# vfrantc/Bayesian-Enhancement-Model

Hardware: AMD Instinct MI355X
Metric: images/sec (whole node) CG_UNet N=8 Bayesian eval @256x256 (higher is better)
Workload: dtype f32

## Files before the change

### bayesian-enhancement-model_amd/bem/archs.py

```python
from __future__ import annotations

import math
import os

import torch
import torch.nn as nn

from . import autograd as ag
from . import ops
from .modules import (Conv2dK, ConvT2x2, LayerNorm2d, PwConv2d, VSSBlock, _Cache, _need_cuda, grad_mode, make_vss_level,
                      set_module_paths)
from .native import BemNativeError

_QD_DIR = os.path.join(os.path.dirname(os.path.dirname(os.path.abspath(__file__))), "basicsr", "QD", "checkpoints")


def _trunc_normal_(t, std=0.02):
    return nn.init.trunc_normal_(t, mean=0.0, std=std, a=-2.0, b=2.0)


def _init_weights(m):
    if isinstance(m, nn.Linear):
        _trunc_normal_(m.weight, std=0.02)
        if m.bias is not None:
# ... 1 lines not shown
    elif isinstance(m, nn.LayerNorm):
        nn.init.constant_(m.weight, 1.0)
        nn.init.constant_(m.bias, 0)


def conv_down(c):
    return Conv2dK(c, c * 2, 4, 2, 1, bias=False)


class _CrossAttnParams(nn.Module):

    def __init__(self, dim):
        super().__init__()
        for n in ("q1_proj", "k2_proj", "v2_proj", "q2_proj", "k1_proj", "v1_proj", "out1", "out2"):
            setattr(self, n, nn.Conv2d(dim, dim, 1))


class Decomp(nn.Module):

    def __init__(self, model="model4", wavelet_out=True, num_filters=32):
        super().__init__()
        if model not in ("model1", "model2", "model3", "model4"):
            raise ValueError(f"Unknown decomp_model: {model}")
        self.model, self.wavelet_out = model, wavelet_out
        nf = num_filters
        self.conv_in = Conv2dK(32, nf, 3, padding=1)
        if model == "model3":
            self.down_conv = Conv2dK(nf, nf, 3, stride=2, padding=1)
            self.mid_conv = Conv2dK(nf, nf, 3, padding=1)
            self.up_conv = ConvT2x2(nf, nf)
        d = 2 if model == "model2" else 1
        self.branch_q1 = nn.Sequential(Conv2dK(nf, nf, 3, padding=1), nn.ReLU(inplace=True), Conv2dK(nf, nf, 3, padding=d, dilation=d))
        self.branch_q2 = nn.Sequential(Conv2dK(nf, nf, 3, padding=1), nn.ReLU(inplace=True), Conv2dK(nf, nf, 3, padding=d, dilation=d))
        self.cross_attn = _CrossAttnParams(nf)
        self.fuse = nn.Conv2d(nf * 2, nf, 1)
        self.conv_out = Conv2dK(nf, 32, 3, padding=1)
        self.sharpening = Conv2dK(32, 32, 3, padding=1, bias=True)
        if model == "model4" and not wavelet_out:
            self.smooth_q1 = nn.Module(); self.smooth_q1.conv = nn.Conv2d(4, 4, 3, padding=1, groups=4, bias=True)
            self.smooth_q2 = nn.Module(); self.smooth_q2.conv = nn.Conv2d(4, 4, 3, padding=1, groups=4, bias=True)
        self._cache = _Cache()

    @classmethod
    def from_shipped(cls, model, wavelet_out):
        from safetensors.torch import load_file
        m = cls(model, wavelet_out)
        sd = load_file(os.path.join(_QD_DIR, f"{model}_999.safetensors"))
        res = m.load_state_dict(sd, strict=False)
        bad = [k for k in res.unexpected_keys if not k.startswith(("smooth_q1.", "smooth_q2."))]
        if res.missing_keys or bad:
            raise RuntimeError(f"frozen decomposition weights {model}_999: missing {res.missing_keys}, unexpected {bad}")
        m.eval()
        for p in m.parameters():
            p.requires_grad = False
        return m

    def _perm(self, dev):
        if self.wavelet_out:
            idx = [b * 8 + 2 * j for b in range(4) for j in range(4)] + [b * 8 + 2 * j + 1 for b in range(4) for j in range(4)]
        else:
            idx = [b * 8 + q for b in range(4) for q in (0, 2, 4, 6, 1, 3, 5, 7)]
        return torch.tensor(idx, device=dev, dtype=torch.long)

    def _prepared(self):
        srcs = [self.conv_out.weight, self.conv_out.bias, self.sharpening.weight, self.sharpening.bias, self.fuse.weight]

        def prep():
            dev = self.conv_out.weight.device
            p = self._perm(dev)
            ca = self.cross_attn
            aw = torch.cat([torch.cat([getattr(ca, n).weight.detach().reshape(-1), getattr(ca, n).bias.detach().reshape(-1)])
                            for n in ("q1_proj", "k2_proj", "v2_proj", "q2_proj", "k1_proj", "v1_proj", "out1", "out2")]).contiguous()
            d = dict(co_w=self.conv_out.weight.detach()[p].contiguous(), co_b=self.conv_out.bias.detach()[p].contiguous(),
                     sh_w=self.sharpening.weight.detach()[p][:, p].contiguous(), sh_b=self.sharpening.bias.detach()[p].contiguous(),
                     aw=aw, fw=self.fuse.weight.detach().reshape(32, 64).contiguous(), fb=self.fuse.bias.detach().contiguous())
            if hasattr(self, "smooth_q1"):
                d["sm_w"] = torch.cat([self.smooth_q1.conv.weight.detach(), self.smooth_q2.conv.weight.detach()], 0).contiguous()
                d["sm_b"] = torch.cat([self.smooth_q1.conv.bias.detach(), self.smooth_q2.conv.bias.detach()], 0).contiguous()
            return d
        return self._cache.get("prep", srcs, prep)

    def forward(self, x, c0=0):
        _need_cuda(x)
        P = self._prepared()
        d = ops.quat_dwt(x, c0)
        feat = self.conv_in(d)
        if self.model == "model3" and not self.wavelet_out:
            if self.training and torch.is_grad_enabled():
                raise BemNativeError("Decomp model3: its attention dropout is active in train() mode (QD/model3.py:98,127); only the eval-mode "
                                     "(identity) form is on the HIP path")
            mid = self.mid_conv(self.down_conv(feat, relu=True), relu=True)
            feat = ops.add(feat, self.up_conv._forward_nograd(mid))
        dil = self.branch_q1[2].dilation[0]
        b1, b2 = self.branch_q1[2], self.branch_q2[2]
        f1 = ops.conv2d(self.branch_q1[0](feat, relu=True), b1.weight.detach(), b1.bias.detach(), pad=dil, dilation=dil, res1=feat)
        f2 = ops.conv2d(self.branch_q2[0](feat, relu=True), b2.weight.detach(), b2.bias.detach(), pad=dil, dilation=dil, res1=feat)
        Wp, bias = ops.attn_fold(f1, f2, P["aw"], P["fw"], P["fb"])
        fused = ops.pw_gemm(f1, Wp, 32, x2=f2, in_mode=2, bias=bias)
        out = ops.conv2d(fused, P["co_w"], P["co_b"], pad=1)
        out = ops.conv2d(out, P["sh_w"], P["sh_b"], pad=1, res1=out)
        if self.wavelet_out:
            return out
        q = ops.iwt(out)
        if "sm_w" in P:
            q = ops.dwconv3x3(q, P["sm_w"], P["sm_b"], mode=3)
        return q


class _Dec(nn.ModuleDict):
    pass


def _check_last_act(last_act):
    if last_act is not None:
        raise NotImplementedError("last_act: only None occurs in the shipped option files")
    return nn.Identity()


def _first_conv(cin, n_feat):
    fc = Conv2dK(cin, n_feat, 3, 1, 1, bias=True)
    nn.init.kaiming_normal_(fc.weight, mode="fan_out", nonlinearity="linear")
    nn.init.zeros_(fc.bias)
    return fc


def _hamilton(o1, o2, train):
    if train:
        return ag.HamiltonFn.apply(o1, o2)
    B, _, H, W = o1.shape
    out8 = torch.empty(B, 8, H, W, device=o1.device, dtype=o1.dtype)
    ops.copy_channels(o1, out8, 0)
    ops.copy_channels(o2, out8, 4)
    return ops.hamilton(out8)


class _Stage2(nn.Module):

    def _setup(self, stage, num_blocks, d_state, ssm_ratio, mlp_ratio, mlp_type, decomp_model, wavelet_out):
        self.stage, self.num_levels = stage, len(num_blocks)
        if isinstance(d_state, int):
            d_state = [d_state] * self.num_levels
        if decomp_model is not None:
            self.decomp = Decomp.from_shipped(decomp_model, wavelet_out=wavelet_out)
        return lambda dim, i: make_vss_level(dim, num_blocks[i], d_state[i], ssm_ratio, mlp_ratio, mlp_type)

    def _add_encoder(self, sfx, cin, n_feat, level):
        setattr(self, "first_conv" + sfx, _first_conv(cin, n_feat))
        enc, cur = nn.ModuleList(), n_feat
        for i in range(self.num_levels - 1):
            enc.append(level(cur, i))
            cur *= 2
        setattr(self, "encoders" + sfx, enc)
        return cur

    def _add_down_layers(self, sfx, n_feat):
        setattr(self, "down_layers" + sfx, nn.ModuleList([conv_down(n_feat * (2 ** i)) for i in range(self.num_levels - 1)]))

    def _add_decoder(self, sfx, cur, n_feat, out_ch, level):
        decs = nn.ModuleList()
        for i in range(self.num_levels - 2, -1, -1):
            decs.append(_Dec({"up": ConvT2x2(cur, cur // 2), "fuse": PwConv2d(cur, cur // 2, bias=False), "block": level(cur // 2, i)}))
            cur //= 2
        setattr(self, "decoders" + sfx, decs)
        pj = Conv2dK(n_feat, out_ch, 3, 1, 1, bias=True)
        nn.init.zeros_(pj.bias)
        setattr(self, "proj" + sfx, pj)

    def _encode(self, sfx, x, **first_kw):
        f = getattr(self, "first_conv" + sfx)(x, **first_kw)
        skips = []
        for enc, down in zip(getattr(self, "encoders" + sfx), getattr(self, "down_layers" + sfx)):
            f, s = ag.fork(enc(f))
            skips.append(s)
            f = down(f)
        return f, skips

    def _decode(self, sfx, f, skips):
        for dec, skip in zip(getattr(self, "decoders" + sfx), reversed(skips)):
            f = dec["block"](dec["fuse"](dec["up"](f), x2=skip, in_mode=2))
        return getattr(self, "proj" + sfx)(f)

    def _cross_fuse(self, f1, f2):
        fa, fb = ag.fork(f1)
        f2 = self.cross_fusion_12(fa, f2)
        f2a, f2b = ag.fork(f2)
        return self.cross_fusion_21(f2a, fb), f2b

    def _attn_bottleneck(self, sfx, f, train):
        f = getattr(self, "bottleneck" + sfx)(f)
        se, sa = getattr(self, "bottleneck_se" + sfx), getattr(self, "spatial_attention" + sfx)
        return sa(se(f)) if train else sa(f, chan_scale=se.gate(f))


class _DualBranch(_Stage2):
    _wavelet, _in_ch, _out_ch = False, 4, 4

    def __init__(self, in_channels=3, out_channels=3, n_feat=40, stage=1, num_blocks=[2, 2, 2], d_state=1, ssm_ratio=1,
                 mlp_ratio=4, mlp_type="gdmlp", use_pixelshuffle=False, drop_path=0.0, use_illu=False, sam=False,
                 last_act=None, decomp_model="model1"):
        super().__init__()
        level = self._setup(stage, num_blocks, d_state, ssm_ratio, mlp_ratio, mlp_type, decomp_model, self._wavelet)
        for br in ("_Q1", "_Q2"):
            cur = self._add_encoder(br, self._in_ch, n_feat, level)
            self._add_down_layers(br, n_feat)
        self.bottleneck_fuse = PwConv2d(cur * 2, cur, bias=False)
        self.bottleneck_block = level(cur, -1)
        self.bottleneck_to_Q1 = PwConv2d(cur, cur, bias=False)
        self.bottleneck_to_Q2 = PwConv2d(cur, cur, bias=False)
        for br in ("_Q1", "_Q2"):
            self._add_decoder(br, cur, n_feat, self._out_ch, level)
        self.last_act = _check_last_act(last_act)
        self.apply(_init_weights)

    def _dual_unet(self, qs):
        feats, skips = [], []
        for br, q in zip(("_Q1", "_Q2"), qs):
            f, sk = self._encode(br, q)
            feats.append(f)
            skips.append(sk)
        fused = self.bottleneck_block(self.bottleneck_fuse(feats[0], x2=feats[1], in_mode=2))
        return [self._decode(br, getattr(self, "bottleneck_to" + br)(fz), sk) for br, fz, sk in zip(("_Q1", "_Q2"), ag.fork(fused), skips)]

    def _full_res(self, qs):
        train = grad_mode(self)
        with torch.enable_grad() if train else torch.no_grad():
            return _hamilton(*self._dual_unet(qs), train)


class DecompDualBranchDDWavelet(_DualBranch):
    _wavelet, _in_ch, _out_ch = True, 32, 16

    def decompose(self, x, c0):
        return self.decomp(x, c0)

    def forward_decomposed(self, d_img, d_cond, img_index=None):
        B, _, h, w = d_cond.shape
        spi = 1 if img_index is None else int(img_index)
        if d_img.shape[0] * spi != B:
            raise ValueError("forward_decomposed: image / sample batch mismatch")

        def branch_input(bi):
            q = torch.empty(B, 32, h, w, device=d_cond.device, dtype=d_cond.dtype)
            if spi == 1:
                ops.copy_channels(d_img, q, 0, src_c0=16 * bi, C=16)
            else:
                ops.copy_channels_rep(d_img, q, 0, spi, src_c0=16 * bi, C=16)
            ops.copy_channels(d_cond, q, 16, src_c0=16 * bi, C=16)
            return q
        o1, o2 = self._dual_unet(branch_input(bi) for bi in range(2))
        if o1.requires_grad or o2.requires_grad:
            return ag.IwtHamiltonFn.apply(o1, o2)
        return ops.iwt_hamilton(o1, o2)

    def forward(self, x, mask=None):
        _need_cuda(x)
        train = grad_mode(self)
        with torch.no_grad():
            x = x.contiguous()
            if x.shape[1] != 6:
                raise ValueError("DecompDualBranchDDWavelet expects 6 input channels (image || condition)")
            d_img, d_cond = self.decomp(x, 0), self.decomp(x, 3)
        with torch.enable_grad() if train else torch.no_grad():
            out = self.forward_decomposed(d_img, d_cond)
        return [x, out]


class DecompDualBranch2DD(_DualBranch):
    _in_ch = 8

    def forward(self, x, mask=None):
        _need_cuda(x)
        with torch.no_grad():
            x = x.contiguous()
            B, _, H, W = x.shape
            qi, qc = self.decomp(x, 0), self.decomp(x, 3)
            qs = []
            for bi in range(2):
                q = torch.empty(B, 8, H, W, device=x.device, dtype=x.dtype)
                ops.copy_channels(qi, q, 0, src_c0=4 * bi, C=4)
                ops.copy_channels(qc, q, 4, src_c0=4 * bi, C=4)
                qs.append(q)
        return [x, self._full_res(qs)]


class DecompDualBranch2(_DualBranch):

    def forward(self, x, mask=None):
        _need_cuda(x)
        with torch.no_grad():
            x = x.contiguous()
            B, _, H, W = x.shape
            qi = self.decomp(x, 0)
            qs = []
            for bi in range(2):
                q = torch.empty(B, 4, H, W, device=x.device, dtype=x.dtype)
                ops.copy_channels(qi, q, 0, src_c0=4 * bi, C=4)
                ops.add_channels(x, q, 0, src_c0=3, C=3)
                qs.append(q)
        return [x[:, 0:3], self._full_res(qs)]


class CrossFusionBlock(nn.Module):

    def __init__(self, ch):
        super().__init__()
        self.transform = PwConv2d(ch, ch, bias=True)
        self.gate = nn.Parameter(torch.ones(1, ch, 1, 1))
        self._cache = _Cache()

    def forward(self, x_src, x_tgt):
        _need_cuda(x_src)
        if grad_mode(self):
            return ag.GateAddFn.apply(self.transform(x_src), self.gate, x_tgt)
        t, C = self.transform, self.transform.out_channels
        Wp, b = self._cache.get("gated", [t.weight, t.bias, self.gate], lambda: (
            ops.pack_pw_weight(ops.row_scale(t.weight.detach().reshape(C, C).contiguous(), self.gate.detach().reshape(C).contiguous())),
            ops.row_scale(t.bias.detach().contiguous(), self.gate.detach().reshape(C).contiguous())))
        return ops.pw_gemm(x_src, Wp, C, bias=b, res=x_tgt)


class SEBlock(nn.Module):

# ... 430 lines not shown
```

### bayesian-enhancement-model_amd/bem/modules.py

```python
from __future__ import annotations

import math
import os
from typing import Dict, List, Optional

import torch
import torch.nn as nn

from . import autograd as ag
from . import ops
from .native import BemNativeError


class _Cache:

    def __init__(self):
        self._d = {}

    def get(self, key, srcs, fn):
        sig = (ops.WEIGHT_EPOCH[0],) + tuple((t.data_ptr(), ops.tensor_version(t), t.device) for t in srcs)
        hit = self._d.get(key)
        if hit is not None and hit[0] == sig:
            return hit[1]
        with torch.no_grad():
# ... 47 lines not shown
class sampling:

    def __init__(self, ctx: Optional[SampleCtx]):
        self.ctx = ctx

    def __enter__(self):
        self.prev = _SAMPLE_CTX[0]
        _SAMPLE_CTX[0] = self.ctx
        return self.ctx

    def __exit__(self, *a):
        _SAMPLE_CTX[0] = self.prev


class LayerNorm2d(nn.LayerNorm):

    def forward(self, x):
        raise BemNativeError("LayerNorm2d is fused into its consumer GEMM; it has no standalone forward here")


class Linear2d(nn.Linear):

    def __init__(self, *a, **k):
        super().__init__(*a, **k)
        self._cache = _Cache()
        self.module_path = ""

    def _load_from_state_dict(self, state_dict, prefix, *args):
        if prefix + "weight" in state_dict:
            state_dict[prefix + "weight"] = state_dict[prefix + "weight"].view(self.weight.shape)
        return super()._load_from_state_dict(state_dict, prefix, *args)

    def gemm_weights(self, B):
        Wp = self._cache.get("p", [self.weight], lambda: ops.pack_pw_weight(self.weight.detach().contiguous()))
        return Wp, (self.bias.detach() if self.bias is not None else None)

    def forward(self, x, **kw):
        _need_cuda(x)
        if grad_mode(self):
            return _pw_train(self, x, kw)
        Wp, b = self.gemm_weights(x.shape[0])
        return ops.pw_gemm(x, Wp, self.out_features, bias=b, **kw)


def _pw_train(m, x, kw):
    extra = set(kw) - {"x2", "in_mode"}
    if extra or (("x2" in kw) != (kw.get("in_mode", 0) == 2)):
        raise BemNativeError(f"1x1 layer: the training path covers plain and concat-input forms only (got {sorted(kw)})")
    return ag.PwFn.apply(x, kw.get("x2"), m.weight, m.bias, m)


class PwConv2d(nn.Conv2d):

    def __init__(self, cin, cout, bias=True):
        super().__init__(cin, cout, 1, 1, 0, bias=bias)
        self._cache = _Cache()
        self.module_path = ""

    def gemm_weights(self, B):
        Wp = self._cache.get("p", [self.weight], lambda: ops.pack_pw_weight(
            self.weight.detach().reshape(self.out_channels, self.in_channels).contiguous()))
        return Wp, (self.bias.detach() if self.bias is not None else None)

    def forward(self, x, **kw):
        _need_cuda(x)
        if grad_mode(self):
            return _pw_train(self, x, kw)
        Wp, b = self.gemm_weights(x.shape[0])
        return ops.pw_gemm(x, Wp, self.out_channels, bias=b, **kw)


class DwConv2d(nn.Conv2d):

    def __init__(self, ch, bias=True):
        super().__init__(ch, ch, 3, 1, 1, groups=ch, bias=bias)
        self.module_path = ""

    def dw_weights(self, B):
        return self.weight.detach(), (self.bias.detach() if self.bias is not None else None)


class Conv2dK(nn.Conv2d):

    def forward(self, x, relu=False, res1=None, res2=None, cin_slice=None):
        _need_cuda(x)
        if grad_mode(self) and self.weight.requires_grad:
            if relu or res1 is not None or res2 is not None:
                raise BemNativeError("Conv2dK: the training path covers the plain convolution (+ bias) only")
            return ag.Conv2dFn.apply(x, self.weight, self.bias, self, cin_slice)
        return ops.conv2d(x, self.weight.detach(), None if self.bias is None else self.bias.detach(),
                          stride=self.stride[0], pad=self.padding[0], relu=relu, res1=res1, res2=res2, cin_slice=cin_slice, dilation=self.dilation[0])


class ConvT2x2(nn.ConvTranspose2d):

    def __init__(self, cin, cout):
        super().__init__(cin, cout, kernel_size=2, stride=2, padding=0, output_padding=0)
        self._cache = _Cache()

    def forward(self, x):
        _need_cuda(x)
        if grad_mode(self):
            return ag.ConvT2x2Fn.apply(x, self.weight, self.bias, self)
        return self._forward_nograd(x)

    def _forward_nograd(self, x):
        co = self.out_channels

        def prep():
            w = self.weight.detach()
            w4 = w.permute(2, 3, 1, 0).reshape(4 * co, self.in_channels).contiguous()
            return ops.pack_pw_weight(w4), self.bias.detach().repeat(4).contiguous()
        Wp, b4 = self._cache.get("p", [self.weight, self.bias], prep)
        return ops.pw_gemm(x, Wp, 4 * co, bias=b4, convT_Win=x.shape[3])


class _BayesBase(nn.Module):
    def _init_common(self, sigma_init, decay, bias):
        self.deterministic = False
        self.decay, self.sigma_init, self.step = decay, sigma_init, 0
        self.bias = bias
        self.module_path = ""
        self._cache = _Cache()

    def _rho_init(self):
        return math.log(math.expm1(abs(self.sigma_init)) + 1e-20)

    def _register_priors(self):
        for kind in ("weight", "bias") if self.bias else ("weight",):
            self.register_buffer(f"prior_mu_{kind}", getattr(self, f"mu_{kind}").detach().clone(), persistent=False)
            self.register_buffer(f"prior_rho_{kind}", getattr(self, f"rho_{kind}").detach().clone(), persistent=False)
        self._ws = self._bs = self._eps_w = self._eps_b = self._sample_owner = None

    def _train_sample(self):
        step = _TRAIN_STEP[0]
        if step is None:
            raise BemNativeError("Bayesian leaves: a training-mode forward runs under Network.forward, which scopes the weight sample")
        if self._sample_owner is step:
            return
        ctx = _SAMPLE_CTX[0]
        from .train import STEP_STATE
        st = STEP_STATE[0]
        decay = lambda: min(self.decay, (1 + self.step) / (10 + self.step))
        d, d_dev = decay(), (st.slot(decay) if st is not None else None)
        for kind in ("weight", "bias") if self.bias else ("weight",):
            mu, rho = getattr(self, f"mu_{kind}"), getattr(self, f"rho_{kind}")
            ops.bnn_prior_ema_(getattr(self, f"prior_mu_{kind}"), getattr(self, f"prior_rho_{kind}"), mu.detach(), rho.detach(), d, d_dev)
            if ctx.eps is not None:
                e = ctx.eps[f"{self.module_path}.{kind}"].reshape((1,) + tuple(mu.shape)).contiguous()
            else:
                e = ops.randn((1,) + tuple(mu.shape), mu.device, ctx.seed, ctx.next_stream(), ctx.epoch_dev)
                self.__dict__.setdefault("_draw_order", {})[kind] = ctx.counter - getattr(step, "counter0", 0)
            w = ops.bnn_sample(mu.detach(), rho.detach(), 1, e)[0]
            if kind == "weight":
                self._ws, self._eps_w = w, e
            else:
                self._bs, self._eps_b = w, e
        if st is None:
            self.step += 1
        else:
            st.on_advance(self._count_step)
        self._sample_owner = step
        step.leaves.append(self)

    def _count_step(self):
        self.step += 1

    def fold_sample_grads(self):
        for w, e, kind in ((self._ws, self._eps_w, "weight"), (self._bs, self._eps_b, "bias")):
            if w is not None and w.grad is not None:
                mu, rho = getattr(self, f"mu_{kind}"), getattr(self, f"rho_{kind}")
                ops.bnn_reparam_bwd_(w.grad, e, rho.detach(), ag.grad_of(mu), ag.grad_of(rho))
        self._ws = self._bs = self._eps_w = self._eps_b = self._sample_owner = None

# ... 471 lines not shown
```

### bayesian-enhancement-model_amd/bem/native.py

```python
from __future__ import annotations

import ctypes
import os
from ctypes import c_double, c_float, c_int, c_int64, c_uint64, c_void_p

_HERE = os.path.dirname(os.path.abspath(__file__))
LIB_PATH = os.environ.get("BEM_HIP_LIB", os.path.join(os.path.dirname(_HERE), "lib", "libbem_hip.so"))
CSRC = os.path.join(os.path.dirname(_HERE), "csrc")


class BemNativeError(RuntimeError):
    pass


class PwArgs(ctypes.Structure):
    _fields_ = [
        ("x1", c_void_p), ("x2", c_void_p), ("C1", c_int), ("C2", c_int), ("in_mode", c_int),
        ("ln_w", c_void_p), ("ln_b", c_void_p), ("ln_eps", c_float),
        ("Wp", c_void_p), ("w_bstride", c_int64),
        ("bias", c_void_p), ("bias_bstride", c_int64),
        ("res", c_void_p),
        ("prelu", c_void_p), ("act", c_int),
        ("out", c_void_p), ("out_mode", c_int), ("Win", c_int),
        ("B", c_int), ("M", c_int), ("K", c_int), ("L", c_int),
    ]


class WgradArgs(ctypes.Structure):
    _fields_ = [
        ("dy", c_void_p), ("dy_bstride", c_int64), ("M", c_int),
        ("x1", c_void_p), ("x1_bstride", c_int64), ("C1", c_int),
        ("x2", c_void_p), ("x2_bstride", c_int64), ("C2", c_int),
        ("dw", c_void_p), ("ldw", c_int64), ("blk_rows", c_int), ("perm", c_int * 4),
        ("dbias", c_void_p),
        ("B", c_int), ("L", c_int),
    ]


P, I, I64, U64, F = c_void_p, c_int, c_int64, c_uint64, c_float

SIGNATURES = {
    "bem_selective_scan_fwd_f32": [P, P, P, P, P, P, P, P, I, I, I, I, I, I, P],
    "bem_selective_scan_fwd_in16": [P, P, P, P, P, P, P, P, I, I, I, I, I, I, I, P],
    "bem_cast16_to_f32": [P, P, ctypes.c_int64, I, P],
    "bem_cast_f32_to16": [P, P, ctypes.c_int64, I, P],
    "bem_selective_scan_bwd_ws_elems": [I, I, I, I],
    "bem_selective_scan_bwd_f32": [P] * 16 + [I, I, I, I, I, I, P],
    "bem_cross_scan_f32": [P, P, I, I, I, I, P],
    "bem_cross_merge_f32": [P, P, I, I, I, I, P],
    "bem_ss2d_scan_strided_f32": [P, P, P, P, P, P, P, P, P, P, I, I, I, I, I64, I64, P],
    "bem_ss2d_scan_rm_supported": [I, I, I],
    "bem_ss2d_scan_rm_f32": [P, P, P, P, P, P, P, P, P, I, I, I, I, I, I64, I64, P],
    "bem_pack_pw_weight_f32": [P, P, I, I, I, P],
    "bem_pw_packed_elems": [I, I],
    "bem_pw_gemm_x6_f32": [ctypes.POINTER(PwArgs), P],
    "bem_pack_pw_weight_x6": [P, P, I, I, I, P],
    "bem_pack_pw_weight_x6_strided": [P, P, I, I, I, I64, I64, I64, P],
    "bem_pack_pw_weight_x6_jobs": [P, P, I, P, P],
    "bem_pw_x6_packed_elems": [I, I],
    "bem_bnn_sample_pack_x6": [P, P, P, P, I, I, I, U64, U64, P, I, P],
    "bem_store_words": [P, P, I, P],
    "bem_bnn_ebank_sample_f32": [P, P, I, P, U64, U64, P],
    "bem_bnn_bank_sample_f32": [P, P, I, P, P, P, P, P, F, P, U64, U64, P, P],
    "bem_bnn_bank_kl_f32": [P, P, I, P, P, P, P],
    "bem_bnn_bank_kl_bwd_f32": [P, P, I, P, P, P, P],
    "bem_bnn_bank_reparam_bwd_f32": [P, P, I, P, P, P],
    "bem_row_scale_f32": [P, P, P, I, I, P],
    "bem_se_gate_f32": [P, P, P, P, I, I, I, P],
    "bem_spatial_attention_f32": [P, P, P, P, P, I, I, I, I, I, P],
    "bem_hamilton_bwd_f32": [P, P, P, I, I, I, P],
    "bem_chan_scale_f32": [P, P, I64, P, P, F, P, I, I, I64, P],
    "bem_chan_dot_f32": [P, P, P, I, I, I64, I, P],
    "bem_se_gate_bwd_f32": [P, P, P, P, P, P, P, P, I, I, I, P],
    "bem_spatial_attention_bwd_f32": [P, P, P, P, P, P, P, I, I, I, I, I, P],
    "bem_bnn_prior_ema_f32": [P, P, P, P, F, P, I64, P],
    "bem_bnn_kl_f32": [P, P, P, P, I64, P, P],
    "bem_bnn_kl_bwd_f32": [P, P, P, P, I64, P, P, P, P],
    "bem_bnn_reparam_bwd_f32": [P, P, P, P, P, I64, P],
    "bem_mask_token_f32": [P, P, P, P, I, I, I, I, P],
    "bem_mask_token_bwd_f32": [P, P, P, P, I, I, I, I, P],
    "bem_depth_to_space_f32": [P, P, I, I, I, I, P],
    "bem_prelu_f32": [P, P, P, I64, P],
    "bem_prelu_bwd_f32": [P, P, P, P, P, I64, P],
    "bem_bilinear_up_bwd_f32": [P, P, I, I, I, I, I, P],
    "bem_gdmlp_x6_f32": [P, P, P, F, P, P, P, P, P, P, I, I, I, I, I, P],
    "bem_conv3x3_x6_f32": [P, I64, P, P, P, P, P, I, I, I, I, I, I, P],
    "bem_conv4x4s2_x6_f32": [P, I64, P, P, P, P, P, I, I, I, I, I, I, P],
    "bem_conv4x4s2_fast_supported": [I, I, I],
    "bem_conv3x3_rows_supported": [I, I, I],
    "bem_ss2d_front_x6_f32": [P, P, P, F, P, P, P, P, P, P, P, I, I, I, I, I, P],
    "bem_conv_taps_x6_f32": [P, I64, P, P, P, P, P, I, I, I, I, I, I, I, I, I, P],
    "bem_dwconv3x3_f32": [P, P, I64, P, I64, P, I, I, I, I, I, P],
    "bem_conv2d_f32": [P, I64, P, P, P, P, P, I, I, I, I, I, I, I, I, I, I, P],
    "bem_conv2d_mfma_f32": [P, I64, P, P, P, P, P, I, I, I, I, I, I, I, I, I, I, P],
    "bem_quat_dwt_f32": [P, I64, P, I, I, I, P],
    "bem_dwt_f32": [P, P, I, I, I, I, P],
    "bem_iwt_f32": [P, P, I, I, I, I, P],
    "bem_iwt_hamilton_f32": [P, P, P, I, I, I, P],
    "bem_hamilton_f32": [P, P, I, I, I, P],
    "bem_hamilton_full_f32": [P, P, P, I, I, I, P],
    "bem_attn_stats_f64": [P, P, P, I, I, P],
    "bem_attn_fold_f32": [P, P, P, P, P, P, I, I, P],
    "bem_transpose_planes_f32": [P, I64, P, I64, I, I, I, I, P],
    "bem_copy_channels_f32": [P, I64, P, I64, I, I, I, P],
    "bem_copy_channels_rep_f32": [P, I64, P, I64, I, I, I, I, P],
    "bem_add_channels_f32": [P, I64, P, I64, I, I, I, P],
    "bem_bilinear_up_f32": [P, I64, P, I64, I, I, I, I, I, P],
    "bem_space_to_depth_f32": [P, P, I, I, I, I, P],
    "bem_pixel_shuffle2_f32": [P, P, I, I, I, I, P],
    "bem_bnn_sample_f32": [P, P, P, P, I, I64, U64, U64, P, P],
    "bem_select_best_f32": [P, P, P, P, P, I, I, I64, P],
    "bem_ssim_f32": [P, P, P, P, I, I, I, I, P],
    "bem_select_scores_f32": [P, P, P, F, I, P, P, P, P, I, I, I64, P],
    "bem_niqe_f32": [P, P, P, P, P, I, P, P, I, P, P, I, P, P, I64, I, I, I, P],
    "bem_niqe_ws_bytes": [I, I, I],
    "bem_uiqm_uciqe_f32": [P, P, P, P, I, P, P, I, P, P, P, I64, I, I, I, I, P],
    "bem_uiqm_ws_bytes": [I, I, I, I],
    "bem_mc_mean_f32": [P, P, P, P, I, I, I, I, I, I, I, P],
    "bem_pad_reflect_f32": [P, P, I, I, I, I, I, P],
    "bem_resize_down_f32": [P, P, I, I, I, I, P],
    "bem_randn_f32": [P, I64, U64, U64, P, P],
    "bem_cond_postproc_f32": [P, P, P, P, I, I, I, I, F, P],
    "bem_plane_mean_f32": [P, P, I, I, I, I, I, P],
    "bem_candidate_finalize_f32": [P, P, P, P, P, I, I, I, I, I, I, I, P],
    "bem_l1_loss_f32": [P, P, P, P, P, I64, F, P, P],
    "bem_iwt_hamilton_bwd_f32": [P, P, P, P, P, I, I, I, P],
    "bem_pixel_unshuffle2_f32": [P, P, I, I, I, I, P],
    "bem_channel_sum_f32": [P, P, I, I, I64, P],
    "bem_add_f32": [P, P, P, I64, F, P],
    "bem_ln_bwd_f32": [P, P, P, P, P, F, P, P, P, P, P, I, I, I64, P],
    "bem_ln_fwd_f32": [P, P, P, P, F, P, I, I, I64, P],
    "bem_dwact_bwd_f32": [P, P, P, P, P, P, P, I, I, I, I, I, P],
    "bem_pw_wgrad_f32": [ctypes.POINTER(WgradArgs), P],
    "bem_pw_wgrad_x6_f32": [ctypes.POINTER(WgradArgs), P, I64, P],
    "bem_pw_wgrad_x6_ws_elems": [I, I, I, I],
    "bem_conv_wgrad_f32": [P, P, I64, P, P, I, I, I, I, I, I, I, I, I, P],
    "bem_ss2d_scan_bwd_f32": [P] * 18 + [I, I, I, I, I64, I64, P],
    "bem_ss2d_scan_n_supported": [I],
    "bem_ss2d_scan_n_f32": [P] * 10 + [I, I, I, I, I, I64, I64, P],
    "bem_ss2d_scan_n_bwd_ws_elems": [I, I, I, I],
    "bem_ss2d_scan_n_bwd_f32": [P] * 19 + [I64, I, I, I, I, I, I64, I64, P],
    "bem_fusion_head_f32": [P, I64, P, I64, P, P, P, P, P, I, I, I, I, I, I, P],
    "bem_fusion_head_bwd_ws_elems": [I, I, I],
    "bem_fusion_head_bwd_f32": [P, I64, P, I64] + [P] * 11 + [I64, I, I, I, I, I, I, P],
    "bem_grad_sumsq_f32": [P, I64, P, P],
    "bem_adamw_step_f32": [P, P, P, P, I64, F, F, F, F, F, I, F, P, P, P, P],
    "bem_last_error": [],
    "bem_abi_version": [],
}
_RESTYPE = {"bem_last_error": ctypes.c_char_p, "bem_pw_packed_elems": c_int64, "bem_pw_x6_packed_elems": c_int64, "bem_selective_scan_bwd_ws_elems": c_int64,
            "bem_pw_wgrad_x6_ws_elems": c_int64, "bem_niqe_ws_bytes": c_int64, "bem_uiqm_ws_bytes": c_int64,
            "bem_ss2d_scan_n_bwd_ws_elems": c_int64, "bem_fusion_head_bwd_ws_elems": c_int64}

_lib = None


def build(verbose: bool = False) -> str:
    import subprocess
    r = subprocess.run(["make", "-j8", "-C", CSRC], capture_output=True, text=True)
    if r.returncode != 0:
        raise BemNativeError(f"building libbem_hip.so failed:\n{r.stdout}\n{r.stderr}")
    if verbose:
        print(r.stdout)
    return LIB_PATH


def lib():
    global _lib
    if _lib is None:
        if not os.path.exists(LIB_PATH):
            raise BemNativeError(
                f"{LIB_PATH} not found: the HIP library is required (no CPU fallback). "
                f"Build it with `make -C {CSRC}` or __graft_entry__.build().")
        L = ctypes.CDLL(LIB_PATH)
        for name, argtypes in SIGNATURES.items():
            fn = getattr(L, name)
            fn.argtypes = argtypes
            fn.restype = _RESTYPE.get(name, c_int)
# ... 9 lines not shown
```

### bayesian-enhancement-model_amd/bem/ops.py

```python
from __future__ import annotations

import ctypes
import os
from typing import Optional

import torch

from . import native
from .native import PwArgs, check, lib


def _stream():
    return ctypes.c_void_p(torch.cuda.current_stream().cuda_stream)


def _p(t: Optional[torch.Tensor]):
    return ctypes.c_void_p(0 if t is None else t.data_ptr())


def _chk(t: Optional[torch.Tensor], name: str, dtype=torch.float32, optional=False):
    if t is None:
        if optional:
            return
        raise ValueError(f"{name} is required")
# ... 296 lines not shown
def gdmlp_x6_supported(C, Hd):
    return GDMLP_X6 and C <= GDMLP_X6_MAXC and Hd % 16 == 0


def dw_gate_params10(dww, dwb, Hd):
    w = dww.reshape(2, Hd, 9).permute(1, 2, 0)
    b = torch.zeros(Hd, 1, 2, device=dww.device, dtype=dww.dtype) if dwb is None else dwb.reshape(2, Hd).t().reshape(Hd, 1, 2)
    return torch.cat([w, b], 1).contiguous()


def gdmlp_x6(x, ln_w, ln_b, ln_eps, Wp_gate, bias_gate, dw10, Wp_out, bias_out, Hd):
    for n_, t in (("x", x), ("ln_w", ln_w), ("ln_b", ln_b), ("Wp_gate", Wp_gate), ("bias_gate", bias_gate), ("dw10", dw10), ("Wp_out", Wp_out)):
        _chk(t, n_)
    _chk(bias_out, "bias_out", optional=True)
    B, C, H, W = x.shape
    if not (C <= 80 and Hd % 16 == 0):
        raise ValueError(f"gdmlp_x6: C = {C} (<= 80) / Hd = {Hd} (% 16) not supported")
    if tuple(dw10.shape) != (Hd, 10, 2):
        raise ValueError("gdmlp_x6: depthwise parameters must come from dw_gate_params10")
    if ln_w.numel() != C or ln_b.numel() != C or bias_gate.numel() != 2 * Hd or (bias_out is not None and bias_out.numel() != C):
        raise ValueError("gdmlp_x6: parameter shapes")
    _chk_packed1("gdmlp_x6", (("Wp_gate", Wp_gate, 2 * Hd, C), ("Wp_out", Wp_out, C, Hd)))
    out = torch.empty_like(x)
    s = _timed("gdmlp_x6", 8.0 * x.numel(), 6.0 * 2.0 * B * H * W * (2 * Hd * C + Hd * C)) if _PROF is not None and _PROF["kernel"] == "gdmlp_x6" and _PROF["pred"](C) else None
    check(lib().bem_gdmlp_x6_f32(_p(x), _p(ln_w), _p(ln_b), float(ln_eps), _p(Wp_gate), _p(bias_gate), _p(dw10), _p(Wp_out),
                                 _p(bias_out), _p(out), B, C, Hd, H, W, _stream()), "gdmlp_x6")
    _timed_end(s)
    return out


def dwconv3x3(x, w, bias=None, mode=0):
    _chk(x, "x"); _chk(w, "w"); _chk(bias, "bias", optional=True)
    B, Cin, H, W = x.shape
    Cout = Cin // 2 if mode == 2 else Cin
    per_b = w.dim() == 5
    Cw = w.shape[1] if per_b else w.shape[0]
    if Cw != Cin or tuple(w.shape[-3:]) != (1, 3, 3) or (per_b and w.shape[0] != B):
        raise ValueError(f"dwconv3x3: weight {tuple(w.shape)} vs input channels {Cin}")
    bb = 0
    if bias is not None:
        if bias.shape[-1] != Cin:
            raise ValueError("dwconv3x3: bias shape")
        bb = Cin if (bias.dim() == 2 and bias.shape[0] == B and B > 1) else 0
        if bias.dim() == 2 and bias.shape[0] not in (1, B):
            raise ValueError("dwconv3x3: bias batch")
    out = torch.empty(B, Cout, H, W, device=x.device, dtype=x.dtype)
    check(lib().bem_dwconv3x3_f32(_p(x), _p(w), (Cin * 9 if per_b else 0), _p(bias), bb, _p(out), B, Cout, H, W, mode,
                                  _stream()), "dwconv3x3")
    return out


_CONV_PACK = {}
USE_CONV_MFMA = __import__("os").environ.get("BEM_CONV_MFMA", "1") != "0"


def _packed_conv_weight(w):
    key = (w.data_ptr(), tensor_version(w), tuple(w.shape), WEIGHT_EPOCH[0])
    hit = _CONV_PACK.get(key)
    if hit is None:
        if len(_CONV_PACK) > 256:
            _CONV_PACK.clear()
        hit = (w, pack_pw_weight(w.reshape(w.shape[0], -1).contiguous(), x6=False))
        _CONV_PACK[key] = hit
    return hit[1]


_CONV_PACK_X6 = {}
USE_CONV_X6 = __import__("os").environ.get("BEM_CONV_X6", "1") != "0"
CONV4_FAST = __import__("os").environ.get("BEM_CONV4_FAST", "1") != "0"


def _packed_conv_weight_x6(w):
    key = (w.data_ptr(), tensor_version(w), tuple(w.shape), WEIGHT_EPOCH[0])
    hit = _CONV_PACK_X6.get(key)
    if hit is None:
        if len(_CONV_PACK_X6) > 256:
            _CONV_PACK_X6.clear()
        taps = w.permute(2, 3, 0, 1).reshape(w.shape[2] * w.shape[3], w.shape[0], w.shape[1]).contiguous()
        hit = (w, pack_pw_weight(taps, x6=True))
        _CONV_PACK_X6[key] = hit
    return hit[1]


def conv2d(x, w, bias=None, stride=1, pad=1, relu=False, res1=None, res2=None, cin_slice=None, dilation=1):
    _chk(x, "x"); _chk(w, "w"); _chk(bias, "bias", optional=True)
    _chk(res1, "res1", optional=True); _chk(res2, "res2", optional=True)
    B, Ct, H, W = x.shape
    Cout, Cin, KH, KW = w.shape
    c0 = 0
    if cin_slice is not None:
        c0, cs = cin_slice
        if cs != Cin or c0 + Cin > Ct:
            raise ValueError("conv2d: channel slice out of range")
    elif Ct != Cin:
        raise ValueError(f"conv2d: input has {Ct} channels, weight expects {Cin}")
    Ho, Wo = (H + 2 * pad - dilation * (KH - 1) - 1) // stride + 1, (W + 2 * pad - dilation * (KW - 1) - 1) // stride + 1
    out = torch.empty(B, Cout, Ho, Wo, device=x.device, dtype=x.dtype)
    if dilation != 1 or (KH, KW, stride) == (3, 3, 2):
        if (KH, KW) != (3, 3) or pad != dilation or Wo % 2 or Cin % 8 or (c0 * H * W) % 2:
            raise ValueError("conv2d: dilated / strided 3x3 convolutions run in the tap form only (pad = dilation, even output width, Cin % 8 == 0)")
        for n, r in (("res1", res1), ("res2", res2)):
            if r is not None and r.shape != out.shape:
                raise ValueError(f"conv2d: {n} shape")
        xp_ = ctypes.c_void_p(x.data_ptr() + 4 * c0 * H * W)
        check(lib().bem_conv_taps_x6_f32(xp_, Ct * H * W, _p(_packed_conv_weight_x6(w)), _p(bias), _p(res1), _p(res2), _p(out), B, Cin, H, W, Cout, 3, stride,
                                         dilation, int(relu), _stream()), "conv_taps_x6")
        return out
    for n, r in (("res1", res1), ("res2", res2)):
        if r is not None and r.shape != out.shape:
            raise ValueError(f"conv2d: {n} shape")
    if bias is not None and bias.shape != (Cout,):
        raise ValueError("conv2d: bias shape")
    xp = ctypes.c_void_p(x.data_ptr() + 4 * c0 * H * W)
    if USE_CONV_X6 and (KH, KW, stride, pad) == (3, 3, 1, 1) and W % 2 == 0 and Cin % 8 == 0 and (c0 * H * W) % 2 == 0:
        check(lib().bem_conv3x3_x6_f32(xp, Ct * H * W, _p(_packed_conv_weight_x6(w)), _p(bias), _p(res1), _p(res2), _p(out), B, Cin, H, W,
                                       Cout, int(relu), _stream()), "conv3x3_x6")
        return out
    conv4_fast = CONV4_FAST and (KH, KW, stride, pad) == (4, 4, 2, 1) and res1 is None and res2 is None and (c0 * H * W) % 4 == 0 \
        and (Ct * H * W) % 4 == 0 and x.data_ptr() % 16 == 0 and lib().bem_conv4x4s2_fast_supported(Cin, H, W) == 1
    if conv4_fast:
        check(lib().bem_conv4x4s2_x6_f32(xp, Ct * H * W, _p(_packed_conv_weight_x6(w)), _p(bias), _p(res1), _p(res2), _p(out), B, Cin, H, W,
                                         Cout, int(relu), _stream()), "conv4x4s2_x6")
        return out
    if USE_CONV_MFMA and Cout <= 160 and ((KH, KW, stride) in ((3, 3, 1), (4, 4, 2))):
        check(lib().bem_conv2d_mfma_f32(xp, Ct * H * W, _p(_packed_conv_weight(w)), _p(bias), _p(res1), _p(res2), _p(out), B, Cin, H, W,
                                        Cout, KH, KW, stride, pad, int(relu), _stream()), "conv2d_mfma")
        return out
    check(lib().bem_conv2d_f32(xp, Ct * H * W, _p(w), _p(bias), _p(res1), _p(res2), _p(out), B, Cin, H, W, Cout, KH, KW,
                               stride, pad, int(relu), _stream()), "conv2d")
    return out


def quat_dwt(x, c0=0):
    _chk(x, "x")
    B, Ct, H, W = x.shape
    if c0 + 3 > Ct or H % 2 or W % 2:
        raise ValueError("quat_dwt: needs 3 channels and even H, W")
    out = torch.empty(B, 32, H // 2, W // 2, device=x.device, dtype=x.dtype)
    check(lib().bem_quat_dwt_f32(ctypes.c_void_p(x.data_ptr() + 4 * c0 * H * W), Ct * H * W, _p(out), B, H, W, _stream()), "quat_dwt")
    return out


def dwt(x):
    _chk(x, "x")
    B, C, H, W = x.shape
    if H % 2 or W % 2:
        raise ValueError("dwt: even H, W required")
    out = torch.empty(B, 4 * C, H // 2, W // 2, device=x.device, dtype=x.dtype)
    check(lib().bem_dwt_f32(_p(x), _p(out), B, C, H, W, _stream()), "dwt")
    return out


def iwt(x):
    _chk(x, "x")
    B, C4, H, W = x.shape
    if C4 % 4:
        raise ValueError("iwt: channels must be a multiple of 4")
    out = torch.empty(B, C4 // 4, 2 * H, 2 * W, device=x.device, dtype=x.dtype)
    check(lib().bem_iwt_f32(_p(x), _p(out), B, C4, H, W, _stream()), "iwt")
    return out


def iwt_hamilton(q1w, q2w):
    _chk(q1w, "q1w"); _chk(q2w, "q2w")
    B, C, h, w = q1w.shape
    if C != 16 or q2w.shape != q1w.shape:
        raise ValueError("iwt_hamilton: expects two (B,16,h,w) tensors")
    out = torch.empty(B, 3, 2 * h, 2 * w, device=q1w.device, dtype=q1w.dtype)
    check(lib().bem_iwt_hamilton_f32(_p(q1w), _p(q2w), _p(out), B, h, w, _stream()), "iwt_hamilton")
    return out


def hamilton(q):
    _chk(q, "q")
    B, C, H, W = q.shape
    if C != 8:
        raise ValueError("hamilton: expects (B,8,H,W)")
    out = torch.empty(B, 3, H, W, device=q.device, dtype=q.dtype)
    check(lib().bem_hamilton_f32(_p(q), _p(out), B, H, W, _stream()), "hamilton")
    return out


def hamilton_bwd(q8, dout):
    _chk(q8, "q8"); _chk(dout, "dout")
    B, C, H, W = q8.shape
    if C != 8 or tuple(dout.shape) != (B, 3, H, W):
        raise ValueError("hamilton_bwd: shapes")
    d = torch.empty_like(q8)
    check(lib().bem_hamilton_bwd_f32(_p(q8), _p(dout), _p(d), B, H, W, _stream()), "hamilton_bwd")
    return d


def hamilton_full(q1, q2):
    _chk(q1, "q1"); _chk(q2, "q2")
    B, C, H, W = q1.shape
    if C != 4 or q2.shape != q1.shape:
        raise ValueError("hamilton_full: expects two (B,4,H,W) tensors")
    out = torch.empty_like(q1)
    check(lib().bem_hamilton_full_f32(_p(q1), _p(q2), _p(out), B, H, W, _stream()), "hamilton_full")
    return out


def attn_fold(f1, f2, attn_w, fuse_w, fuse_b):
    for n, t in (("f1", f1), ("f2", f2), ("attn_w", attn_w), ("fuse_w", fuse_w), ("fuse_b", fuse_b)):
        _chk(t, n)
    B, C, H, W = f1.shape
    if C != 32 or f2.shape != f1.shape or attn_w.numel() != 8 * (32 * 32 + 32) or fuse_w.numel() != 32 * 64 or fuse_b.numel() != 32:
        raise ValueError("attn_fold: shapes")
    L = H * W
    stats = torch.empty(B, 32 * 32 + 64, device=f1.device, dtype=torch.float64)
    check(lib().bem_attn_stats_f64(_p(f1), _p(f2), _p(stats), B, L, _stream()), "attn_stats")
    Wn = torch.empty(B, 32, 64, device=f1.device, dtype=torch.float32)
    bias = torch.empty(B, 32, device=f1.device, dtype=torch.float32)
    check(lib().bem_attn_fold_f32(_p(stats), _p(attn_w), _p(fuse_w), _p(fuse_b), _p(Wn), _p(bias), B, L, _stream()), "attn_fold")
    return pack_pw_weight(Wn, x6=True), bias


def transpose_planes(x):
    _chk(x, "x")
    B, C, H, W = x.shape
    out = torch.empty(B, C, W, H, device=x.device, dtype=x.dtype)
    n = B * C
# ... 1089 lines not shown
```

### bayesian-enhancement-model_amd/bem/pipeline.py

```python
from __future__ import annotations

import os
from typing import Dict, List, Optional

import torch

from . import ops
from .modules import SampleCtx, sampling


class BEMPipeline:

    def __init__(self, net1, net2, scale_down: int = 16, noise_level: float = 0.1):
        self.net1, self.net2 = net1, net2
        self.scale, self.noise_level = scale_down, noise_level
        self._side = None

    @torch.no_grad()
    def candidates(self, imgs, targets, num_samples: int, gt_mean: bool, deterministic: bool = False,
                   eps: Optional[Dict[str, torch.Tensor]] = None, noise: Optional[torch.Tensor] = None,
                   img_down: Optional[torch.Tensor] = None, seed: int = 0, rank: int = 0, sample_offset: int = 0,
                   total_samples: Optional[int] = None):
        from basicsr.bayesian import set_prediction_type
        B, _, h, w = imgs.shape
        N = 1 if deterministic else num_samples
        NT = total_samples or N
        if not deterministic and (eps is not None or noise is not None) and NT != N:
            rows = (torch.arange(B)[:, None] * NT + sample_offset + torch.arange(N)[None, :]).reshape(-1).to(imgs.device)
            if eps is not None:
                eps = {k_: v.index_select(0, rows) for k_, v in eps.items()}
            if noise is not None:
                noise = noise.index_select(0, rows)
        f = 4 * self.scale
        Hp = (((h + f) // f) * f) if h % f else h
        Wp = (((w + f) // f) * f) if w % f else w
        pad = ops.pad_reflect(imgs.contiguous(), Hp, Wp)
        if img_down is None:
            img_down = ops.resize_down(pad, self.scale)
        hd, wd = img_down.shape[-2:]
        x1 = img_down[:, None].expand(B, N, 3, hd, wd).reshape(B * N, 3, hd, wd)
        hoist = hasattr(self.net2, "forward_decomposed")
        d_img, main = None, torch.cuda.current_stream()
        if hoist and os.environ.get("BEM_DECOMP_OVERLAP", "1") != "0":
            if self._side is None or self._side.device != pad.device:
                self._side = torch.cuda.Stream(device=pad.device)
            self._side.wait_stream(main)
            with torch.cuda.stream(self._side):
                d_img = self.net2.decompose(pad, 0)
            pad.record_stream(self._side)
        set_prediction_type(self.net1, deterministic)
        with sampling(None if deterministic else SampleCtx(B * N, eps, seed, rank=rank)) as ctx:
            pred = self.net1(x1)[-1]
        tmean = ops.plane_mean(targets.contiguous()) if (gt_mean and targets is not None) else None
        if noise is None and self.noise_level:
            noise = ops.randn(tuple(pred.shape), pred.device, seed, (1 << 62) | (rank << 44) | SampleCtx._epoch)
        conds = ops.cond_postproc(pred, tmean, noise if self.noise_level else None, N, self.noise_level)
        cond_up = ops.bilinear_up(conds, self.scale)
        if hoist:
            if d_img is None:
                d_img = self.net2.decompose(pad, 0)
            else:
                main.wait_stream(self._side)
                d_img.record_stream(main)
            d_cond = self.net2.decompose(cond_up, 0)
            raw = self.net2.forward_decomposed(d_img, d_cond, None if N == 1 else N)
        else:
            x2 = torch.empty(B * N, 6, Hp, Wp, device=pad.device, dtype=pad.dtype)
            ops.copy_channels(pad[:, None].expand(B, N, 3, Hp, Wp).reshape(B * N, 3, Hp, Wp).contiguous(), x2, 0)
            ops.copy_channels(cond_up, x2, 3)
            raw = self.net2(x2)[-1]
        final, psnr = ops.candidate_finalize(raw, None if targets is None else targets.contiguous(), N, h, w,
                                             bool(gt_mean and targets is not None))
        return dict(conds=conds, raw=raw, final=final, psnr=psnr, N=N)

    @staticmethod
    def select(psnr_rows: List[float]) -> int:
        m = max(psnr_rows)
        if m == 0:
            return 0
        rel = [p / m for p in psnr_rows]
        return rel.index(max(rel))

    @torch.no_grad()
    def enhance(self, imgs, targets, num_samples, gt_mean=True, deterministic=False, sync=True, scorer=None, monte_carlo=False, shard=None, **kw):
        if shard is not None and shard[1] > 1 and not deterministic:
            from . import dist as bdist
            rank, world = shard
            kw.pop("rank", None)
            lo, hi = bdist.shard_samples(num_samples, rank, world)
            B = imgs.shape[0]
            r = self.candidates(imgs, targets, max(hi - lo, 1), gt_mean, False, rank=rank, sample_offset=lo, total_samples=num_samples, **kw)
            for k_ in ("final", "psnr", "conds") + (("raw",) if monte_carlo else ()):
                t = r[k_] if hi > lo else r[k_][:0]
                r[k_] = bdist.gather_samples(t.contiguous(), B, num_samples, rank, world)
            if not monte_carlo:
                r.pop("raw")
            r["N"] = num_samples
        else:
            r = self.candidates(imgs, targets, num_samples, gt_mean, deterministic, **kw)
        N = r["N"]
        h, w = imgs.shape[-2:]
        if scorer is not None:
            sel = scorer.select(r["final"], targets, N, psnr=r["psnr"])
            best, img = sel["best"], sel["best_images"]
            bp = ops.select_scores(None, r["psnr"], N, rule="max")[1] if targets is None else _gather(r["psnr"], best, N)
            r.update(scores=sel["s1"], scores2=sel["s2"])
        else:
            best, bp, img = ops.select_best(r["final"], r["psnr"], N)
            if targets is None:
                best = torch.zeros_like(best)
                img = r["final"][::N].contiguous()
        r.update(best=best, best_images=img, best_psnr=bp)
        if monte_carlo:
            mc = ops.mc_mean(r["raw"], None if targets is None else targets.contiguous(), N, h, w, bool(gt_mean and targets is not None))
            r["mc"] = mc
            if targets is not None:
                _, r["mc_psnr"] = ops.candidate_finalize(mc, targets.contiguous(), 1, h, w, False)
                r["mc_ssim"] = ops.ssim(mc, targets.contiguous(), 1) if min(h, w) > 10 else None
        if sync:
            r["best"], r["best_psnr"] = best.cpu().tolist(), bp.cpu().tolist()
        return r


def _gather(v, best, N):
    B = best.numel()
    return v.view(B, N).gather(1, best.long().view(B, 1)).view(B)


def synthetic_pair(shape, seed=287128, device="cpu"):
    g = torch.Generator().manual_seed(seed)
    lq = 0.25 * torch.rand(shape, generator=g)
    gt = (3.5 * lq + 0.05 * torch.randn(shape, generator=g)).clamp(0, 1)
    return lq.to(device), gt.to(device)


def build_nets(n_feat=40, num_blocks=(2, 2, 2), seed=100, device="cuda", stage2="DecompDualBranchDDWavelet", decomp="model4"):
    import inspect
    from basicsr.archs import build_network
    from basicsr.bayesian import convert2bnn_selective
    from basicsr.utils.registry import ARCH_REGISTRY
    torch.manual_seed(seed)
    common = dict(n_feat=n_feat, d_state=[1, 1, 1], ssm_ratio=1, mlp_ratio=4, mlp_type="gdmlp", use_pixelshuffle=True,
                  drop_path=0.0, sam=False, stage=1, num_blocks=list(num_blocks))
    net1 = build_network(dict(type="Network", in_channels=3, out_channels=3, **common))
    convert2bnn_selective(net1, {"sigma_init": 0.05, "decay": 0.998, "pretrain": False})
    opt2 = dict(type=stage2, in_channels=6, out_channels=3, **common)
    if "decomp_model" in inspect.signature(ARCH_REGISTRY.get(stage2)).parameters:
        opt2["decomp_model"] = decomp
    net2 = build_network(opt2)
# ... 2 lines not shown
```

### bayesian-enhancement-model_amd/csrc/conv.hip

```cpp
#include "bem_common.h"
#include <cstdlib>

namespace {

constexpr int RB = 4;

__device__ __forceinline__ void dw_block(const float* __restrict__ plane, int H, int W, int y0, int x0, bool vec,
                                         const float* __restrict__ w9, float (&acc)[RB][4]) {
    float wk[9];
#pragma unroll
    for (int i = 0; i < 9; ++i) wk[i] = w9[i];
#pragma unroll
    for (int ry = -1; ry <= RB; ++ry) {
        const int yy = y0 + ry;
        if (yy < 0 || yy >= H) continue;
        const float* r = plane + (int64_t)yy * W;
        float v[6];
        v[0] = x0 > 0 ? r[x0 - 1] : 0.f;
        if (vec) {
            const float4 c = *reinterpret_cast<const float4*>(r + x0);
            v[1] = c.x; v[2] = c.y; v[3] = c.z; v[4] = c.w;
        } else {
#pragma unroll
            for (int i = 0; i < 4; ++i) v[1 + i] = (x0 + i < W) ? r[x0 + i] : 0.f;
// ... 82 lines not shown
        const int yy = min(max(y0 + ry, 0), H - 1);
        const float* r = plane + (int64_t)yy * W;
        c[ry + 1] = *reinterpret_cast<const float4*>(r + x0);
        if (!DPPHALO) {
            hl[ry + 1] = r[max(x0 - 1, 0)];
            hr[ry + 1] = r[min(x0 + 4, W - 1)];
        }
    }
    float wk[9];
#pragma unroll
    for (int i = 0; i < 9; ++i) wk[i] = w9[i];
    const float mt = y0 > 0 ? 1.f : 0.f, mb = y0 + RB < H ? 1.f : 0.f;
    const float ml = x0 > 0 ? 1.f : 0.f, mr = x0 + 4 < W ? 1.f : 0.f;
#pragma unroll
    for (int ry = -1; ry <= RB; ++ry) {
        float4 q = c[ry + 1];
        if (ry == -1) { q.x *= mt; q.y *= mt; q.z *= mt; q.w *= mt; }
        if (ry == RB) { q.x *= mb; q.y *= mb; q.z *= mb; q.w *= mb; }
        const float v[6] = {(DPPHALO ? dpp_from_prev_lane(q.w) : hl[ry + 1] * ((ry == -1) ? mt : (ry == RB) ? mb : 1.f)) * ml, q.x, q.y, q.z, q.w,
                            (DPPHALO ? dpp_from_next_lane(q.x) : hr[ry + 1] * ((ry == -1) ? mt : (ry == RB) ? mb : 1.f)) * mr};
#pragma unroll
        for (int oy = 0; oy < RB; ++oy) {
            const int dy = ry - oy;
            if (dy < -1 || dy > 1) continue;
            const float w0 = wk[(dy + 1) * 3], w1 = wk[(dy + 1) * 3 + 1], w2 = wk[(dy + 1) * 3 + 2];
#pragma unroll
            for (int j = 0; j < 4; ++j) acc[oy][j] = fmaf(w0, v[j], fmaf(w1, v[j + 1], fmaf(w2, v[j + 2], acc[oy][j])));
        }
    }
}

template <int MODE, bool DPPHALO>
__global__ __launch_bounds__(256) void dwconv3x3_fast_kernel(const float* __restrict__ x, const float* __restrict__ w,
                                                             int64_t w_bs, const float* __restrict__ bias, int64_t b_bs,
                                                             float* __restrict__ out, int Cout, int H, int W) {
    const int W4 = W >> 2, HB = H / RB;
    const int i = blockIdx.x * blockDim.x + threadIdx.x;
    if (i >= HB * W4) return;
    const int yb = i / W4, y0 = yb * RB, x0 = (i - yb * W4) * 4;
    const int c = blockIdx.y, b = blockIdx.z;
    const int Cin = (MODE == 2) ? 2 * Cout : Cout;
    const int64_t HW = (int64_t)H * W;
    const float* wb = w + (int64_t)b * w_bs;
    const float* bb = bias ? bias + (int64_t)b * b_bs : wb;
    const float bm = bias ? 1.f : 0.f;
    const float b0 = bb[bias ? c : 0] * bm;
    const float b1 = (MODE == 2) ? bb[bias ? c + Cout : 0] * bm : 0.f;
    const float* pl = x + ((int64_t)b * Cin + c) * HW;
    float a0[RB][4], a1[RB][4];
#pragma unroll
    for (int r = 0; r < RB; ++r)
#pragma unroll
        for (int j = 0; j < 4; ++j) a0[r][j] = a1[r][j] = 0.f;
    dw_block_fast<DPPHALO>(pl, H, W, y0, x0, wb + (int64_t)c * 9, a0);
    if (MODE == 2) dw_block_fast<DPPHALO>(x + ((int64_t)b * Cin + c + Cout) * HW, H, W, y0, x0, wb + (int64_t)(c + Cout) * 9, a1);
    float4 self[RB];
    if (MODE == 3) {
#pragma unroll
        for (int r = 0; r < RB; ++r) self[r] = *reinterpret_cast<const float4*>(pl + (int64_t)(y0 + r) * W + x0);
    }
#pragma unroll
    for (int r = 0; r < RB; ++r) {
        float o[4];
        const float sv[4] = {MODE == 3 ? self[r].x : 0.f, MODE == 3 ? self[r].y : 0.f, MODE == 3 ? self[r].z : 0.f, MODE == 3 ? self[r].w : 0.f};
#pragma unroll
        for (int j = 0; j < 4; ++j) {
            const float v = a0[r][j] + b0;
            if (MODE == 2) o[j] = bem_gelu_fast(v) * (a1[r][j] + b1);
            else if (MODE == 1) o[j] = bem_silu(v);
            else if (MODE == 3) o[j] = sv[j] + fmaxf(v, 0.f);
            else o[j] = v;
        }
        *reinterpret_cast<float4*>(out + ((int64_t)b * Cout + c) * HW + (int64_t)(y0 + r) * W + x0) = make_float4(o[0], o[1], o[2], o[3]);
    }
}

constexpr int TH = 8, TW = 32, COB = 16, CIB = 8;

template <int KH, int KW, int S>
__global__ __launch_bounds__(256) void conv2d_kernel(const float* __restrict__ x, int64_t x_bs,
                                                     const float* __restrict__ w, const float* __restrict__ bias,
                                                     const float* __restrict__ res1, const float* __restrict__ res2,
                                                     float* __restrict__ out, int Cin, int H, int W, int Cout,
                                                     int Ho, int Wo, int pad, int relu, int tilesX) {
    constexpr int PH = (TH - 1) * S + KH, PW = (TW - 1) * S + KW;
    constexpr int PWP = PW + 1;
    __shared__ float patch[CIB][PH][PWP];
    __shared__ __attribute__((aligned(16))) float wl[CIB][KH * KW][COB];
    const int tile = blockIdx.x;
    const int ty0 = (tile / tilesX) * TH, tx0 = (tile % tilesX) * TW;
    const int co0 = blockIdx.y * COB;
    const int b = blockIdx.z;
    const int tx = threadIdx.x & 31, ty = threadIdx.x >> 5;
    const int oy = ty0 + ty, ox = tx0 + tx;
    const int iy0 = ty0 * S - pad, ix0 = tx0 * S - pad;
    const float* xb = x + (int64_t)b * x_bs;
    float acc[COB];
#pragma unroll
    for (int i = 0; i < COB; ++i) acc[i] = 0.f;
    for (int ci0 = 0; ci0 < Cin; ci0 += CIB) {
        __syncthreads();
        for (int i = threadIdx.x; i < CIB * PH * PW; i += 256) {
            const int cc = i / (PH * PW), rem = i - cc * (PH * PW);
            const int py = rem / PW, px = rem - py * PW;
            const int ci = ci0 + cc, iy = iy0 + py, ix = ix0 + px;
            float v = 0.f;
            if (ci < Cin && iy >= 0 && iy < H && ix >= 0 && ix < W) v = xb[((int64_t)ci * H + iy) * W + ix];
            patch[cc][py][px] = v;
        }
        for (int i = threadIdx.x; i < CIB * KH * KW * COB; i += 256) {
            const int o = i % COB, t = (i / COB) % (KH * KW), cc = i / (COB * KH * KW);
            const int ci = ci0 + cc, co = co0 + o;
            wl[cc][t][o] = (ci < Cin && co < Cout) ? w[(((int64_t)co * Cin + ci) * KH * KW) + t] : 0.f;
        }
        __syncthreads();
#pragma unroll 2
        for (int cc = 0; cc < CIB; ++cc) {
#pragma unroll
            for (int ky = 0; ky < KH; ++ky) {
#pragma unroll
                for (int kx = 0; kx < KW; ++kx) {
                    const float v = patch[cc][ty * S + ky][tx * S + kx];
                    const float4* wq = reinterpret_cast<const float4*>(&wl[cc][ky * KW + kx][0]);
#pragma unroll
                    for (int q = 0; q < COB / 4; ++q) {
                        const float4 ww = wq[q];
                        acc[4 * q] = fmaf(ww.x, v, acc[4 * q]);
                        acc[4 * q + 1] = fmaf(ww.y, v, acc[4 * q + 1]);
                        acc[4 * q + 2] = fmaf(ww.z, v, acc[4 * q + 2]);
                        acc[4 * q + 3] = fmaf(ww.w, v, acc[4 * q + 3]);
                    }
                }
            }
        }
    }
    if (oy >= Ho || ox >= Wo) return;
#pragma unroll
    for (int o = 0; o < COB; ++o) {
        const int co = co0 + o;
        if (co >= Cout) break;
        float v = acc[o] + (bias ? bias[co] : 0.f);
        if (relu) v = fmaxf(v, 0.f);
        const int64_t idx = (((int64_t)b * Cout + co) * Ho + oy) * Wo + ox;
        if (res1) v += res1[idx];
        if (res2) v += res2[idx];
        out[idx] = v;
    }
}


typedef float f32x16 __attribute__((ext_vector_type(16)));

template <int KH, int KW, int PH, int PWP>
__device__ __forceinline__ constexpr int patch_off(int k) {
    return (k / (KH * KW)) * PH * PWP + ((k % (KH * KW)) / KW) * PWP + (k % (KH * KW)) % KW;
}

template <int MTW>
__device__ __forceinline__ void conv_mfma_epilogue(f32x16 (&acc)[MTW][2], const float* __restrict__ Wp, const float* __restrict__ bias,
                                                   const float* __restrict__ res1, const float* __restrict__ res2,
                                                   float* __restrict__ out, int b, int Cout, int Ho, int Wo, int ty0, int tx0,
                                                   int wave, int half, int j, int relu) {
    const int ox = tx0 + j, oxc = min(ox, Wo - 1);
    const float* bp = bias ? bias : Wp;
    const float* p1 = res1 ? res1 : Wp;
    const float* p2 = res2 ? res2 : Wp;
    const float bmk = bias ? 1.f : 0.f, m1 = res1 ? 1.f : 0.f, m2 = res2 ? 1.f : 0.f;
    const int64_t k0 = bias ? -1 : 0, k1 = res1 ? -1 : 0, k2 = res2 ? -1 : 0;
    const float lo = relu ? 0.f : -3.402823466e38f;
#pragma unroll
    for (int t = 0; t < 2; ++t) {
        const int oy = ty0 + 2 * wave + t, oyc = min(oy, Ho - 1);
        const bool pix = oy < Ho && ox < Wo;
#pragma unroll
        for (int m = 0; m < MTW; ++m) {
            constexpr int RG = 8;
#pragma unroll
            for (int r0 = 0; r0 < 16; r0 += RG) {
                float r1[RG], r2[RG], bv[RG];
#pragma unroll
                for (int q = 0; q < RG; ++q) {
                    const int r = r0 + q;
                    const int co = min(m * 32 + (r & 3) + 8 * (r >> 2) + 4 * half, Cout - 1);
                    const int64_t idx = (((int64_t)b * Cout + co) * Ho + oyc) * Wo + oxc;
                    bv[q] = bp[co & k0] * bmk;
                    r1[q] = p1[idx & k1] * m1;
                    r2[q] = p2[idx & k2] * m2;
                }
#pragma unroll
                for (int q = 0; q < RG; ++q) {
                    const int r = r0 + q;
                    const int co = m * 32 + (r & 3) + 8 * (r >> 2) + 4 * half;
                    if (pix && co < Cout)
                        out[(((int64_t)b * Cout + co) * Ho + oy) * Wo + ox] = fmaxf(acc[m][t][r] + bv[q], lo) + r1[q] + r2[q];
                }
            }
        }
    }
}

template <int KH, int KW, int S, int MTW>
__global__ __launch_bounds__(256, MTW == 1 ? 4 : MTW == 2 ? 3 : MTW == 3 ? 2 : 1) void conv2d_mfma_kernel(const float* __restrict__ x, int64_t x_bs,
                                                          const float* __restrict__ Wp, const float* __restrict__ bias,
                                                          const float* __restrict__ res1, const float* __restrict__ res2,
                                                          float* __restrict__ out, int Cin, int H, int W, int Cout,
                                                          int Ho, int Wo, int pad, int relu, int tilesX, int KS) {
    constexpr int KK = KH * KW;
    constexpr int KC = CIB * KK;
    constexpr int PH = (TH - 1) * S + KH, PW = (TW - 1) * S + KW, PWP = PW + 1;
    __shared__ float patch[CIB * PH * PWP];
    const int lane = threadIdx.x & 63, wave = threadIdx.x >> 6, half = lane >> 5, j = lane & 31;
    const int tile = blockIdx.x, b = blockIdx.y;
    const int ty0 = (tile / tilesX) * TH, tx0 = (tile % tilesX) * TW;
    const int iy0 = ty0 * S - pad, ix0 = tx0 * S - pad;
    const float* xb = x + (int64_t)b * x_bs;
    f32x16 acc[MTW][2];
#pragma unroll
    for (int m = 0; m < MTW; ++m)
#pragma unroll
        for (int t = 0; t < 2; ++t)
#pragma unroll
            for (int r = 0; r < 16; ++r) acc[m][t][r] = 0.f;
    const float* wl = Wp + lane;
    const int64_t mts = (int64_t)KS * 64;
    const int rowoff0 = (2 * wave) * S * PWP + j * S, rowoff1 = rowoff0 + S * PWP;

    for (int ci0 = 0; ci0 < Cin; ci0 += CIB) {
        __syncthreads();
        {
            constexpr int UB = 8;
            constexpr int TOT = CIB * PH * PW;
            for (int base = 0; base < TOT; base += 256 * UB) {
                float v[UB];
#pragma unroll
                for (int u = 0; u < UB; ++u) {
                    const int i = base + u * 256 + threadIdx.x;
                    const int cc = i / (PH * PW), rem = i - cc * (PH * PW);
                    const int py = rem / PW, px = rem - py * PW;
                    const int ci = ci0 + cc, iy = iy0 + py, ix = ix0 + px;
                    v[u] = 0.f;
                    if (i < TOT && ci < Cin && iy >= 0 && iy < H && ix >= 0 && ix < W) v[u] = xb[((int64_t)ci * H + iy) * W + ix];
                }
#pragma unroll
                for (int u = 0; u < UB; ++u) {
                    const int i = base + u * 256 + threadIdx.x;
                    if (i < TOT) {
                        const int cc = i / (PH * PW), rem = i - cc * (PH * PW);
                        const int py = rem / PW, px = rem - py * PW;
                        patch[cc * PH * PWP + py * PWP + px] = v[u];
                    }
                }
            }
        }
        __syncthreads();
        const int sg0 = (ci0 * KK) >> 1;
        constexpr int NS = KC / 2;
        constexpr int PB = 4;
        static_assert(NS % PB == 0, "chunk k-steps must be a multiple of the operand batch");
        float an[MTW][PB];
#pragma unroll
        for (int m = 0; m < MTW; ++m)
#pragma unroll
            for (int u = 0; u < PB; ++u)
                an[m][u] = wl[m * mts + (int64_t)min(sg0 + u, KS - 1) * 64] * ((sg0 + u < KS) ? 1.f : 0.f);
        for (int s0 = 0; s0 < NS; s0 += PB) {
            float ac[MTW][PB];
#pragma unroll
            for (int m = 0; m < MTW; ++m)
#pragma unroll
                for (int u = 0; u < PB; ++u) {
                    ac[m][u] = an[m][u];
                    const int sn = sg0 + s0 + PB + u;
                    an[m][u] = wl[m * mts + (int64_t)min(sn, KS - 1) * 64] * ((s0 + PB + u < NS && sn < KS) ? 1.f : 0.f);
                }
#pragma unroll
            for (int u = 0; u < PB; ++u) {
                const int k = 2 * (s0 + u) + half, kc = k / KK, kt = k - kc * KK;
                const int o = kc * PH * PWP + (kt / KW) * PWP + (kt % KW);
                const float v0 = patch[o + rowoff0], v1 = patch[o + rowoff1];
#pragma unroll
                for (int m = 0; m < MTW; ++m) {
                    acc[m][0] = __builtin_amdgcn_mfma_f32_32x32x2f32(ac[m][u], v0, acc[m][0], 0, 0, 0);
                    acc[m][1] = __builtin_amdgcn_mfma_f32_32x32x2f32(ac[m][u], v1, acc[m][1], 0, 0, 0);
                }
            }
        }
    }
    conv_mfma_epilogue<MTW>(acc, Wp, bias, res1, res2, out, b, Cout, Ho, Wo, ty0, tx0, wave, half, j, relu);
}

template <int KH, int KW, int S, int MTW>
__global__ __launch_bounds__(256, MTW == 1 ? 3 : 2) void conv2d_mfma_pipe_kernel(const float* __restrict__ x, int64_t x_bs,
                                                               const float* __restrict__ Wp, const float* __restrict__ bias,
                                                               const float* __restrict__ res1, const float* __restrict__ res2,
                                                               float* __restrict__ out, int Cin, int H, int W, int Cout,
                                                               int Ho, int Wo, int pad, int relu, int tilesX, int KS) {
    constexpr int KK = KH * KW;
    constexpr int KC = CIB * KK;
    constexpr int NS = KC / 2;
    constexpr int PH = (TH - 1) * S + KH, PW = (TW - 1) * S + KW, PWP = PW + 1;
    constexpr int PSZ = CIB * PH * PWP;
    constexpr int TOT = CIB * PH * PW;
    constexpr int NU = (TOT + 255) / 256;
    constexpr int WSZ = NS * 64;
    static_assert(WSZ % 256 == 0, "weight slice must split evenly over the workgroup");
    constexpr int NWU = WSZ / 256;
    __shared__ float patch[2][PSZ + 1];
    __shared__ float wsm[2][MTW][WSZ];
    const int lane = threadIdx.x & 63, wave = threadIdx.x >> 6, half = lane >> 5, j = lane & 31;
    const int tile = blockIdx.x, b = blockIdx.y;
    const int ty0 = (tile / tilesX) * TH, tx0 = (tile % tilesX) * TW;
    const int iy0 = ty0 * S - pad, ix0 = tx0 * S - pad;
    const float* xb = x + (int64_t)b * x_bs;
    const int HW = H * W;
    int goff[NU], lofc[NU];
    float gm[NU];
#pragma unroll
    for (int u = 0; u < NU; ++u) {
        const int i = u * 256 + threadIdx.x;
        const int cc = i / (PH * PW), rem = i - cc * (PH * PW);
        const int py = rem / PW, px = rem - py * PW;
        const int iy = iy0 + py, ix = ix0 + px;
        const bool in = i < TOT && iy >= 0 && iy < H && ix >= 0 && ix < W;
        goff[u] = in ? iy * W + ix : 0;
        gm[u] = in ? 1.f : 0.f;
        lofc[u] = (i < TOT ? cc * PH * PWP + py * PWP + px : PSZ) | (min(cc, CIB - 1) << 20);
    }
    f32x16 acc[MTW][2];
#pragma unroll
    for (int m = 0; m < MTW; ++m)
#pragma unroll
        for (int t = 0; t < 2; ++t)
#pragma unroll
            for (int r = 0; r < 16; ++r) acc[m][t][r] = 0.f;
    const int64_t mts = (int64_t)KS * 64;
    const int wtot = KS * 64;
    const int rowoff0 = (2 * wave) * S * PWP + j * S, rowoff1 = rowoff0 + S * PWP;
    float v[NU], wv[MTW][NWU];
    auto fetch = [&](int ci0) {
#pragma unroll
        for (int u = 0; u < NU; ++u) {
            const float* p = xb + (int64_t)min(ci0 + (lofc[u] >> 20), Cin - 1) * HW + goff[u];
            asm volatile("global_load_dword %0, %1, off" : "=v"(v[u]) : "v"(p));
        }
        const int wbase = ((ci0 * KK) >> 1) * 64;
#pragma unroll
        for (int m = 0; m < MTW; ++m)
#pragma unroll
            for (int u = 0; u < NWU; ++u) {
                const float* p = Wp + m * mts + min(wbase + u * 256 + (int)threadIdx.x, wtot - 1);
                asm volatile("global_load_dword %0, %1, off" : "=v"(wv[m][u]) : "v"(p));
            }
    };
    auto arrive = [&]() {
        static_assert(NU == 11 && NWU == 9 && MTW <= 2, "operand lists below are written for the 3x3 stride-1 chunk");
        asm volatile("s_waitcnt vmcnt(0)"
                     : "+v"(v[0]), "+v"(v[1]), "+v"(v[2]), "+v"(v[3]), "+v"(v[4]), "+v"(v[5]), "+v"(v[6]), "+v"(v[7]), "+v"(v[8]),
                       "+v"(v[9]), "+v"(v[10]));
#pragma unroll
        for (int m = 0; m < MTW; ++m)
            asm volatile("" : "+v"(wv[m][0]), "+v"(wv[m][1]), "+v"(wv[m][2]), "+v"(wv[m][3]), "+v"(wv[m][4]), "+v"(wv[m][5]),
                              "+v"(wv[m][6]), "+v"(wv[m][7]), "+v"(wv[m][8]));
    };
    auto stash = [&](int bufi, int ci0) {
        const int wbase = ((ci0 * KK) >> 1) * 64;
#pragma unroll
        for (int u = 0; u < NU; ++u) patch[bufi][lofc[u] & 0xfffff] = v[u] * (ci0 + (lofc[u] >> 20) < Cin ? gm[u] : 0.f);
#pragma unroll
        for (int m = 0; m < MTW; ++m)
#pragma unroll
            for (int u = 0; u < NWU; ++u)
                wsm[bufi][m][u * 256 + threadIdx.x] = wv[m][u] * (wbase + u * 256 + (int)threadIdx.x < wtot ? 1.f : 0.f);
    };
    fetch(0);
    arrive();
    stash(0, 0);
    __syncthreads();
    int buf = 0;
    for (int ci0 = 0; ci0 < Cin; ci0 += CIB) {
        fetch(ci0 + CIB);
        __builtin_amdgcn_sched_barrier(0);
        const float* pb = patch[buf];
#pragma unroll
        for (int s = 0; s < NS; ++s) {
            const int o = half ? patch_off<KH, KW, PH, PWP>(2 * s + 1) : patch_off<KH, KW, PH, PWP>(2 * s);
            const float v0 = pb[o + rowoff0], v1 = pb[o + rowoff1];
#pragma unroll
            for (int m = 0; m < MTW; ++m) {
                const float a = wsm[buf][m][s * 64 + lane];
                acc[m][0] = __builtin_amdgcn_mfma_f32_32x32x2f32(a, v0, acc[m][0], 0, 0, 0);
                acc[m][1] = __builtin_amdgcn_mfma_f32_32x32x2f32(a, v1, acc[m][1], 0, 0, 0);
            }
        }
        __builtin_amdgcn_sched_barrier(0);
        arrive();
        stash(buf ^ 1, ci0 + CIB);
        __syncthreads();
        buf ^= 1;
    }
    conv_mfma_epilogue<MTW>(acc, Wp, bias, res1, res2, out, b, Cout, Ho, Wo, ty0, tx0, wave, half, j, relu);
}

}

extern "C" int bem_dwconv3x3_f32(const float* x, const float* w, int64_t w_bstride, const float* bias,
                                 int64_t bias_bstride, float* out, int B, int Cout, int H, int W, int mode,
                                 void* stream) {
    BEM_REQUIRE(x && w && out, "dwconv3x3: null tensor");
    BEM_REQUIRE(B >= 0 && B <= 65535 && Cout > 0 && Cout <= 65535 && H > 0 && W > 0, "dwconv3x3: bad shape");
    BEM_REQUIRE(mode >= 0 && mode <= 3, "dwconv3x3: mode %d", mode);
    if (B == 0) return BEM_OK;
    dim3 grid(cdiv(cdiv(H, RB) * ((W + 3) / 4), 256), Cout, B);
    hipStream_t s = (hipStream_t)stream;
    const bool fast = W % 4 == 0 && H % RB == 0 && (((uintptr_t)x | (uintptr_t)out) & 15) == 0;
    const bool dpp = fast && 64 % (W / 4) == 0;
#define BEM_DW(MODE) do { if (dpp) dwconv3x3_fast_kernel<MODE, true><<<grid, 256, 0, s>>>(x, w, w_bstride, bias, bias_bstride, out, Cout, H, W); \
                          else dwconv3x3_fast_kernel<MODE, false><<<grid, 256, 0, s>>>(x, w, w_bstride, bias, bias_bstride, out, Cout, H, W); } while (0)
    if (!fast) dwconv3x3_kernel<<<grid, 256, 0, s>>>(x, w, w_bstride, bias, bias_bstride, out, Cout, H, W, mode);
    else if (mode == 0) BEM_DW(0);
    else if (mode == 1) BEM_DW(1);
    else if (mode == 2) BEM_DW(2);
    else BEM_DW(3);
#undef BEM_DW
    return bem_check_launch("dwconv3x3");
}

extern "C" int bem_conv2d_f32(const float* x, int64_t x_bstride, const float* w, const float* bias,
                              const float* res1, const float* res2, float* out, int B, int Cin, int H, int W,
                              int Cout, int KH, int KW, int stride, int pad, int relu, void* stream) {
    BEM_REQUIRE(x && w && out, "conv2d: null tensor");
    BEM_REQUIRE(B >= 0 && B <= 65535 && Cin > 0 && Cout > 0 && H > 0 && W > 0, "conv2d: bad shape");
    const int Ho = (H + 2 * pad - KH) / stride + 1, Wo = (W + 2 * pad - KW) / stride + 1;
    BEM_REQUIRE(Ho > 0 && Wo > 0, "conv2d: empty output");
    if (B == 0) return BEM_OK;
    const int tilesX = cdiv(Wo, TW), tilesY = cdiv(Ho, TH);
    dim3 grid(tilesX * tilesY, cdiv(Cout, COB), B);
    hipStream_t s = (hipStream_t)stream;
    if (KH == 3 && KW == 3 && stride == 1)
        conv2d_kernel<3, 3, 1><<<grid, 256, 0, s>>>(x, x_bstride, w, bias, res1, res2, out, Cin, H, W, Cout, Ho, Wo, pad, relu, tilesX);
    else if (KH == 4 && KW == 4 && stride == 2)
        conv2d_kernel<4, 4, 2><<<grid, 256, 0, s>>>(x, x_bstride, w, bias, res1, res2, out, Cin, H, W, Cout, Ho, Wo, pad, relu, tilesX);
    else
        BEM_REQUIRE(false, "conv2d: unsupported kernel %dx%d stride %d (have 3x3 s1, 4x4 s2)", KH, KW, stride);
    return bem_check_launch("conv2d");
}

extern "C" int bem_conv2d_mfma_f32(const float* x, int64_t x_bstride, const float* Wp, const float* bias,
                                   const float* res1, const float* res2, float* out, int B, int Cin, int H, int W,
                                   int Cout, int KH, int KW, int stride, int pad, int relu, void* stream) {
    BEM_REQUIRE(x && Wp && out, "conv2d_mfma: null tensor");
    BEM_REQUIRE(B >= 0 && B <= 65535 && Cin > 0 && Cout > 0 && Cout <= 160 && H > 0 && W > 0, "conv2d_mfma: bad shape (Cout <= 160)");
    const int Ho = (H + 2 * pad - KH) / stride + 1, Wo = (W + 2 * pad - KW) / stride + 1;
    BEM_REQUIRE(Ho > 0 && Wo > 0, "conv2d_mfma: empty output");
    if (B == 0) return BEM_OK;
    const int tilesX = cdiv(Wo, TW), tilesY = cdiv(Ho, TH);
    const int KS = cdiv(Cin * KH * KW, 2), MT = cdiv(Cout, 32);
    dim3 grid(tilesX * tilesY, B);
    hipStream_t s = (hipStream_t)stream;
#define BEM_CONV_LAUNCH(KH_, KW_, S_, MTW_) \
    conv2d_mfma_kernel<KH_, KW_, S_, MTW_><<<grid, 256, 0, s>>>(x, x_bstride, Wp, bias, res1, res2, out, Cin, H, W, Cout, Ho, Wo, pad, relu, tilesX, KS)
    if (KH == 3 && KW == 3 && stride == 1) {
        static const bool pipe = !(getenv("BEM_CONV_PIPE") && getenv("BEM_CONV_PIPE")[0] == '0');
        if (MT <= 2 && pipe) {
            if (MT == 1) conv2d_mfma_pipe_kernel<3, 3, 1, 1><<<grid, 256, 0, s>>>(x, x_bstride, Wp, bias, res1, res2, out, Cin, H, W, Cout, Ho, Wo, pad, relu, tilesX, KS);
            else conv2d_mfma_pipe_kernel<3, 3, 1, 2><<<grid, 256, 0, s>>>(x, x_bstride, Wp, bias, res1, res2, out, Cin, H, W, Cout, Ho, Wo, pad, relu, tilesX, KS);
        }
        else if (MT == 1) BEM_CONV_LAUNCH(3, 3, 1, 1);
        else if (MT == 2) BEM_CONV_LAUNCH(3, 3, 1, 2);
        else if (MT == 3) BEM_CONV_LAUNCH(3, 3, 1, 3);
        else BEM_CONV_LAUNCH(3, 3, 1, 5);
    } else if (KH == 4 && KW == 4 && stride == 2) {
        if (MT == 1) BEM_CONV_LAUNCH(4, 4, 2, 1);
        else if (MT == 2) BEM_CONV_LAUNCH(4, 4, 2, 2);
        else if (MT == 3) BEM_CONV_LAUNCH(4, 4, 2, 3);
        else BEM_CONV_LAUNCH(4, 4, 2, 5);
    } else {
        BEM_REQUIRE(false, "conv2d_mfma: unsupported kernel %dx%d stride %d (have 3x3 s1, 4x4 s2)", KH, KW, stride);
    }
#undef BEM_CONV_LAUNCH
    return bem_check_launch("conv2d_mfma");
}
```

### bayesian-enhancement-model_amd/csrc/conv_rows_x6.hip

```cpp
#include "bem_common.h"
#include "scan_common.h"
#include "x6_common.h"

namespace {

struct CrX {
    const float* x; int64_t x_bs;
    const u32x4* Wp; const float* bias; const float* res1; const float* res2; float* out;
    int Cin, H, W, Ho, Wo, Cout, KB, MT, wo_shift, relu, mt_first;
};

typedef float f32x4v __attribute__((ext_vector_type(4)));

template <int MTW, int KS, int S>
__global__ __launch_bounds__(256, 2) void conv_rows_x6_kernel(CrX k) {
    constexpr int NPX = 4 / S;
    constexpr int NP = 3 * KS * MTW;
    __shared__ __attribute__((aligned(16))) u32x4 Ws[2][NP * 64];
    const int lane = threadIdx.x & 63, wave = __builtin_amdgcn_readfirstlane(threadIdx.x >> 6), kh = lane >> 5, n = lane & 31;
    const int b = blockIdx.z, mt0 = k.mt_first + blockIdx.y * MTW;
    const int Lo = k.Ho * k.Wo, Li = k.H * k.W;
    const int p0 = (xcd_tile(blockIdx.x, gridDim.x) * 4 + wave) * (32 * NPX);
    const int p = p0 + NPX * n;
    const bool live = p < Lo;
    const int pc = live ? p : 0;
    const int yo = pc >> k.wo_shift, xo = pc & (k.Wo - 1);
    const float lmask = xo == 0 ? 0.f : 1.f, rmask = xo == k.Wo - NPX ? 0.f : 1.f;
    const float* xb = k.x + (int64_t)b * k.x_bs;
    const uint32_t voff = 16 * lane, ws_lds = lds_addr(Ws);
    const int NS = KS * k.KB;

    auto dma_w = [&](int s, int buf) {
        const int kb = s / KS, r = s - kb * KS;
#pragma unroll
        for (int t = 0; t < (NP + 3) / 4; ++t) {
            const int pi = wave + 4 * t, kx = pi / (3 * MTW), m = (pi / 3) % MTW, li = pi % 3;
            if (pi < NP)
                glds16(k.Wp + ((((int64_t)(KS * r + kx) * k.MT + (mt0 + m)) * k.KB + kb) * 3 + li) * 64, voff, ws_lds + (buf * NP + pi) * 1024);
        }
    };
    auto load_x = [&](int s, f32x4v (&dst)[8], float& mk) {
        const int kb = min(s / KS, k.KB - 1), r = s - (s / KS) * KS;
        const int yi = S * yo - 1 + r;
        mk = (live && yi >= 0 && yi < k.H) ? 1.f : 0.f;
        const int off = min(max(yi, 0), k.H - 1) * k.W + S * xo;
#pragma unroll
        for (int e = 0; e < 8; ++e) {
            const int ch = min(16 * kb + 8 * kh + e, k.Cin - 1);
            dst[e] = *reinterpret_cast<const f32x4v*>(xb + (int64_t)ch * Li + off);
        }
    };

    f32x16 acc[MTW][NPX], alo[MTW][NPX];
#pragma unroll
    for (int m = 0; m < MTW; ++m)
#pragma unroll
        for (int t = 0; t < NPX; ++t)
#pragma unroll
            for (int r = 0; r < 16; ++r) acc[m][t][r] = alo[m][t][r] = 0.f;

    dma_w(0, 0);
    f32x4v xn[8];
    float mkn;
    load_x(0, xn, mkn);
    asm volatile("s_waitcnt vmcnt(0)" ::: "memory");
    __syncthreads();

    for (int s = 0; s < NS; ++s) {
        if (s + 1 < NS) dma_w(s + 1, (s + 1) & 1);
        float col[6][8];
#pragma unroll
        for (int e = 0; e < 8; ++e) {
            const f32x4v v = xn[e] * mkn;
            col[1][e] = v[0]; col[2][e] = v[1]; col[3][e] = v[2]; col[4][e] = v[3];
            col[0][e] = dpp_mov<0x138, 0xf>(0.f, v[3]) * lmask;
            col[5][e] = dpp_mov<0x130, 0xf>(0.f, v[0]) * rmask;
        }
        load_x(s + 1, xn, mkn);
        u32x4 xl[6][3];
#pragma unroll
        for (int c = 0; c < 6; ++c) split8(col[c], xl[c][0], xl[c][1], xl[c][2]);
        const u32x4* Wc = Ws[s & 1] + lane;
#pragma unroll
        for (int kx = 0; kx < KS; ++kx)
#pragma unroll
            for (int m = 0; m < MTW; ++m) {
                const u32x4* wp = Wc + (kx * MTW + m) * 192;
                const u32x4 wl[3] = {wp[0], wp[64], wp[128]};
#pragma unroll
                for (int j = 0; j < NPX; ++j) mac6(wl, xl[S * j + kx], acc[m][j], alo[m][j]);
            }
        asm volatile("s_waitcnt vmcnt(0)" ::: "memory");
        __syncthreads();
    }

    if (live) {
        typedef float fpx __attribute__((ext_vector_type(NPX)));
        const float lo = k.relu ? 0.f : -3.402823466e38f;
        const int64_t ob = (int64_t)b * k.Cout * Lo + pc;
#pragma unroll
        for (int m = 0; m < MTW; ++m)
#pragma unroll
            for (int r = 0; r < 16; ++r) {
                const int row = (mt0 + m) * 32 + (r & 3) + 8 * (r >> 2) + 4 * kh;
                if (row < k.Cout) {
                    const float bv = k.bias ? k.bias[row] : 0.f;
                    const int64_t o = ob + (int64_t)row * Lo;
                    fpx v;
#pragma unroll
                    for (int j = 0; j < NPX; ++j) v[j] = fmaxf(acc[m][j][r] + alo[m][j][r] + bv, lo);
                    if (k.res1) v += *reinterpret_cast<const fpx*>(k.res1 + o);
                    if (k.res2) v += *reinterpret_cast<const fpx*>(k.res2 + o);
                    *reinterpret_cast<fpx*>(k.out + o) = v;
                }
            }
    }
}

}

extern "C" int bem_conv4x4s2_fast_supported(int Cin, int H, int W) {
    const int Wo = W / 2;
    return Cin % 8 == 0 && H % 2 == 0 && W % 2 == 0 && Wo >= 2 && Wo <= 64 && (Wo & (Wo - 1)) == 0;
}
extern "C" int bem_conv3x3_rows_supported(int Cin, int H, int W) {
    return Cin % 8 == 0 && H > 0 && W >= 4 && W <= 128 && (W & (W - 1)) == 0;
}

int conv_rows_launch(int KS, const float* x, int64_t x_bstride, const float* Wp, const float* bias, const float* res1, const float* res2, float* out,
                     int B, int Cin, int H, int W, int Cout, int relu, void* stream) {
    const char* what = KS == 4 ? "conv4x4s2_x6" : "conv3x3_x6";
    BEM_REQUIRE(x && Wp && out, "%s: null tensor", what);
    BEM_REQUIRE(B >= 0 && B <= 65535 && Cin > 0 && Cout > 0 && (KS == 4 ? bem_conv4x4s2_fast_supported(Cin, H, W) : bem_conv3x3_rows_supported(Cin, H, W)),
                "%s: shape outside the row form", what);
    BEM_REQUIRE((((uintptr_t)Wp | (uintptr_t)x | (uintptr_t)out | (uintptr_t)(res1 ? res1 : out) | (uintptr_t)(res2 ? res2 : out)) & 15) == 0 && (x_bstride % 4) == 0,
                "%s: alignment (x, packed weights, out and residuals 16 bytes)", what);
    const int S = KS == 4 ? 2 : 1, Ho = H / S, Wo = W / S;
    BEM_REQUIRE((int64_t)Cout * Ho * Wo < (1ll << 30) && (int64_t)Cin * H * W < (1ll << 30), "%s: plane set too large for 32-bit lane offsets", what);
    if (B == 0) return BEM_OK;
    CrX k;
    k.x = x; k.x_bs = x_bstride; k.Wp = reinterpret_cast<const u32x4*>(Wp); k.bias = bias; k.res1 = res1; k.res2 = res2; k.out = out;
    k.Cin = Cin; k.H = H; k.W = W; k.Ho = Ho; k.Wo = Wo; k.Cout = Cout; k.KB = cdiv(Cin, 16); k.MT = cdiv(Cout, 32); k.relu = relu;
    k.wo_shift = __builtin_ctz(Wo);
    hipStream_t s = (hipStream_t)stream;
    if (KS == 4) {
        const int pairs = k.MT / 2, nx = cdiv(Ho * Wo, 256);
        if (pairs) {
            k.mt_first = 0;
            conv_rows_x6_kernel<2, 4, 2><<<dim3(nx, pairs, B), 256, 0, s>>>(k);
        }
        if (k.MT & 1) {
            k.mt_first = 2 * pairs;
            conv_rows_x6_kernel<1, 4, 2><<<dim3(nx, 1, B), 256, 0, s>>>(k);
        }
    } else {
        k.mt_first = 0;
        conv_rows_x6_kernel<1, 3, 1><<<dim3(cdiv(Ho * Wo, 512), k.MT, B), 256, 0, s>>>(k);
    }
    return bem_check_launch(what);
}
```

### bayesian-enhancement-model_amd/csrc/elementwise.hip

```cpp
#include "bem_common.h"
#include <algorithm>

thread_local char bem_err_buf[512] = "";
extern "C" const char* bem_last_error(void) { return bem_err_buf; }
extern "C" int bem_abi_version(void) { return 1; }

namespace {

#define GRID1D(n) dim3((unsigned)cdiv64((n), 256))

__global__ void quat_dwt_kernel(const float* __restrict__ rgb, int64_t x_bs, float* __restrict__ out, int H, int W,
                                int64_t total) {
    const int64_t i = (int64_t)blockIdx.x * blockDim.x + threadIdx.x;
    if (i >= total) return;
    const int h2 = H >> 1, w2 = W >> 1;
    const int x = (int)(i % w2), y = (int)((i / w2) % h2), b = (int)(i / ((int64_t)w2 * h2));
    const float* p = rgb + (int64_t)b * x_bs;
    const int64_t HW = (int64_t)H * W;
    float q[8][4];
#pragma unroll
    for (int s = 0; s < 4; ++s) {
        const int yy = 2 * y + (s & 1), xx = 2 * x + (s >> 1);
        const float r = p[(int64_t)yy * W + xx], g = p[HW + (int64_t)yy * W + xx], bl = p[2 * HW + (int64_t)yy * W + xx];
        const float den = fmaxf(fmaxf(r, g), bl) + 1e-7f;
        q[0][s] = 0.f; q[1][s] = 0.f;
        q[2][s] = r / den; q[3][s] = r;
        q[4][s] = g / den; q[5][s] = g;
        q[6][s] = bl / den; q[7][s] = bl;
    }
    const int64_t hw2 = (int64_t)h2 * w2;
    float* o = out + (int64_t)b * 32 * hw2 + (int64_t)y * w2 + x;
#pragma unroll
    for (int c = 0; c < 8; ++c) {
        const float a = q[c][0] / 2, bb = q[c][1] / 2, cc = q[c][2] / 2, d = q[c][3] / 2;
        o[(int64_t)(c) * hw2] = a + bb + cc + d;
        o[(int64_t)(8 + c) * hw2] = -a - bb + cc + d;
        o[(int64_t)(16 + c) * hw2] = -a + bb - cc + d;
        o[(int64_t)(24 + c) * hw2] = a - bb - cc + d;
    }
}

__global__ void dwt_kernel(const float* __restrict__ x, float* __restrict__ out, int C, int H, int W, int64_t total) {
    const int64_t i = (int64_t)blockIdx.x * blockDim.x + threadIdx.x;
    if (i >= total) return;
    const int h2 = H >> 1, w2 = W >> 1;
    const int xx = (int)(i % w2), y = (int)((i / w2) % h2);
    const int c = (int)((i / ((int64_t)w2 * h2)) % C), b = (int)(i / ((int64_t)w2 * h2 * C));
    const float* p = x + ((int64_t)b * C + c) * H * W;
    const float a = p[(int64_t)(2 * y) * W + 2 * xx] / 2, bb = p[(int64_t)(2 * y + 1) * W + 2 * xx] / 2;
    const float cc = p[(int64_t)(2 * y) * W + 2 * xx + 1] / 2, d = p[(int64_t)(2 * y + 1) * W + 2 * xx + 1] / 2;
    const int64_t hw2 = (int64_t)h2 * w2;
    float* o = out + ((int64_t)b * 4 * C + c) * hw2 + (int64_t)y * w2 + xx;
    o[0] = a + bb + cc + d;
    o[(int64_t)C * hw2] = -a - bb + cc + d;
    o[(int64_t)2 * C * hw2] = -a + bb - cc + d;
    o[(int64_t)3 * C * hw2] = a - bb - cc + d;
}

__device__ __forceinline__ void iwt4(float ll, float hl, float lh, float hh, float (&o)[4]) {
    ll /= 2; hl /= 2; lh /= 2; hh /= 2;
    o[0] = ll - hl - lh + hh;
    o[1] = ll - hl + lh - hh;
    o[2] = ll + hl - lh - hh;
    o[3] = ll + hl + lh + hh;
}

__global__ void iwt_kernel(const float* __restrict__ x, float* __restrict__ out, int C, int H, int W, int64_t total) {
    const int64_t i = (int64_t)blockIdx.x * blockDim.x + threadIdx.x;
    if (i >= total) return;
    const int xx = (int)(i % W), y = (int)((i / W) % H);
    const int c = (int)((i / ((int64_t)W * H)) % C), b = (int)(i / ((int64_t)W * H * C));
    const int64_t hw = (int64_t)H * W;
    const float* p = x + ((int64_t)b * 4 * C + c) * hw + (int64_t)y * W + xx;
    float o[4];
    iwt4(p[0], p[(int64_t)C * hw], p[(int64_t)2 * C * hw], p[(int64_t)3 * C * hw], o);
    float* q = out + ((int64_t)b * C + c) * 4 * hw + (int64_t)(2 * y) * (2 * W) + 2 * xx;
    *reinterpret_cast<float2*>(q) = make_float2(o[0], o[2]);
    *reinterpret_cast<float2*>(q + 2 * W) = make_float2(o[1], o[3]);
}

__device__ __forceinline__ void hamilton_ijk(const float (&p)[4], const float (&q)[4], float (&o)[3]) {
    o[0] = p[0] * q[1] + p[1] * q[0] + p[2] * q[3] - p[3] * q[2];
    o[1] = p[0] * q[2] - p[1] * q[3] + p[2] * q[0] + p[3] * q[1];
    o[2] = p[0] * q[3] + p[1] * q[2] - p[2] * q[1] + p[3] * q[0];
}

__global__ void iwt_hamilton_kernel(const float* __restrict__ q1w, const float* __restrict__ q2w,
                                    float* __restrict__ out, int h, int w, int64_t total) {
    const int64_t i = (int64_t)blockIdx.x * blockDim.x + threadIdx.x;
    if (i >= total) return;
    const int x = (int)(i % w), y = (int)((i / w) % h), b = (int)(i / ((int64_t)w * h));
    const int64_t hw = (int64_t)h * w;
    const float* a = q1w + (int64_t)b * 16 * hw + (int64_t)y * w + x;
    const float* c = q2w + (int64_t)b * 16 * hw + (int64_t)y * w + x;
    float P[4][4], Q[4][4];
#pragma unroll
    for (int k = 0; k < 4; ++k) {
        iwt4(a[(int64_t)k * hw], a[(int64_t)(4 + k) * hw], a[(int64_t)(8 + k) * hw], a[(int64_t)(12 + k) * hw], P[k]);
        iwt4(c[(int64_t)k * hw], c[(int64_t)(4 + k) * hw], c[(int64_t)(8 + k) * hw], c[(int64_t)(12 + k) * hw], Q[k]);
    }
    float res[3][4];
#pragma unroll
    for (int s = 0; s < 4; ++s) {
        const float pp[4] = {P[0][s], P[1][s], P[2][s], P[3][s]};
        const float qq[4] = {Q[0][s], Q[1][s], Q[2][s], Q[3][s]};
        float o[3];
        hamilton_ijk(pp, qq, o);
        res[0][s] = o[0]; res[1][s] = o[1]; res[2][s] = o[2];
    }
    const int W2 = 2 * w;
    float* op = out + (int64_t)b * 3 * 4 * hw + (int64_t)(2 * y) * W2 + 2 * x;
#pragma unroll
    for (int k = 0; k < 3; ++k) {
        float* o = op + (int64_t)k * 4 * hw;
        *reinterpret_cast<float2*>(o) = make_float2(res[k][0], res[k][2]);
        *reinterpret_cast<float2*>(o + W2) = make_float2(res[k][1], res[k][3]);
    }
}

__global__ void hamilton_kernel(const float* __restrict__ q, float* __restrict__ out, int64_t HW, int64_t total) {
    const int64_t i = (int64_t)blockIdx.x * blockDim.x + threadIdx.x;
// ... 133 lines not shown
        if (j == 0) {
            double s = 0;
            for (int k = 0; k < ATT_C; ++k) s += X[i][k] * Bv(mv, k);
            va[i] = s;
        }
        __syncthreads();
        Y[i][j] = pv;
        __syncthreads();
        const double mres = mm(Z, Y, i, j);
        if (j == 0) {
            double s = Bv(mo, i);
            for (int k = 0; k < ATT_C; ++k) s += Z[i][k] * va[k];
            (br ? c2 : c1)[i] = s;
        }
        (br ? M2 : M1)[i][j] = mres;
    }
    __syncthreads();
    X[i][j] = (double)fw[i * 64 + j];
    Y[i][j] = (double)fw[i * 64 + 32 + j];
    __syncthreads();
    const double left = X[i][j] + mm(Y, M2, i, j);
    const double right = mm(X, M1, i, j) + Y[i][j];
    float* wp = Wp + (int64_t)b * (32 * 64);
    wp[i * 64 + j] = (float)left;
    wp[i * 64 + 32 + j] = (float)right;
    if (j == 0) {
        double s = (double)fb[i];
        for (int k = 0; k < ATT_C; ++k) s += X[i][k] * c1[k] + Y[i][k] * c2[k];
        bias_out[(int64_t)b * 32 + i] = (float)s;
    }
}

__global__ __launch_bounds__(256) void transpose_planes_kernel(const float* __restrict__ src, int64_t src_bs,
                                                               float* __restrict__ dst, int64_t dst_bs, int ppb,
                                                               int H, int W) {
    __shared__ float t[32][33];
    const int plane = blockIdx.z;
    const int bq = plane / ppb, pq = plane - bq * ppb;
    const int64_t HW = (int64_t)H * W;
    const float* s = src + (int64_t)bq * src_bs + (int64_t)pq * HW;
    float* d = dst + (int64_t)bq * dst_bs + (int64_t)pq * HW;
    const int x0 = blockIdx.x * 32, y0 = blockIdx.y * 32;
    const int tx = threadIdx.x & 31, ty = threadIdx.x >> 5;
    float v[4];
#pragma unroll
    for (int k = 0; k < 4; ++k) {
        const int y = min(y0 + ty + 8 * k, H - 1), x = min(x0 + tx, W - 1);
        v[k] = s[(int64_t)y * W + x];
    }
#pragma unroll
    for (int k = 0; k < 4; ++k) t[ty + 8 * k][tx] = v[k];
    __syncthreads();
#pragma unroll
    for (int k = 0; k < 32; k += 8) {
        const int x = x0 + ty + k, y = y0 + tx;
        if (x < W && y < H) d[(int64_t)x * H + y] = t[tx][ty + k];
    }
}

__global__ void copy_channels_kernel(const float* __restrict__ src, int64_t src_bs, float* __restrict__ dst,
                                     int64_t dst_bs, int64_t CL, int64_t total) {
    const int64_t i = (int64_t)blockIdx.x * blockDim.x + threadIdx.x;
    if (i >= total) return;
    const int64_t b = i / CL, r = i - b * CL;
    dst[b * dst_bs + r] = src[b * src_bs + r];
}

__global__ void copy_channels_rep_kernel(const float* __restrict__ src, int64_t src_bs, float* __restrict__ dst,
                                         int64_t dst_bs, int64_t CL, int64_t total, int rep) {
    const int64_t i = (int64_t)blockIdx.x * blockDim.x + threadIdx.x;
    if (i >= total) return;
    const int64_t b = i / CL, r = i - b * CL;
    dst[b * dst_bs + r] = src[(b / rep) * src_bs + r];
}

__global__ void add_channels_kernel(const float* __restrict__ src, int64_t src_bs, float* __restrict__ dst,
                                    int64_t dst_bs, int64_t CL, int64_t total) {
    const int64_t i = (int64_t)blockIdx.x * blockDim.x + threadIdx.x;
    if (i >= total) return;
    const int64_t b = i / CL, r = i - b * CL;
    dst[b * dst_bs + r] += src[b * src_bs + r];
}

__global__ void bilinear_up_kernel(const float* __restrict__ src, int64_t src_bs, float* __restrict__ dst,
                                   int64_t dst_bs, int C, int H, int W, int s, int64_t total) {
    const int64_t i = (int64_t)blockIdx.x * blockDim.x + threadIdx.x;
    if (i >= total) return;
    const int Wo = W * s, Ho = H * s;
    const int xo = (int)(i % Wo), yo = (int)((i / Wo) % Ho);
    const int c = (int)((i / ((int64_t)Wo * Ho)) % C), b = (int)(i / ((int64_t)Wo * Ho * C));
    const float rs = 1.f / (float)s;
    float sy = ((float)yo + 0.5f) * rs - 0.5f; sy = sy < 0.f ? 0.f : sy;
    float sx = ((float)xo + 0.5f) * rs - 0.5f; sx = sx < 0.f ? 0.f : sx;
    const int y0 = (int)sy, x0 = (int)sx;
    const int y1 = y0 + (y0 < H - 1 ? 1 : 0), x1 = x0 + (x0 < W - 1 ? 1 : 0);
    const float ly = sy - (float)y0, lx = sx - (float)x0;
    const float hy = 1.f - ly, hx = 1.f - lx;
    const float* p = src + (int64_t)b * src_bs + (int64_t)c * H * W;
    const float v = hy * (hx * p[(int64_t)y0 * W + x0] + lx * p[(int64_t)y0 * W + x1]) +
                    ly * (hx * p[(int64_t)y1 * W + x0] + lx * p[(int64_t)y1 * W + x1]);
    dst[(int64_t)b * dst_bs + ((int64_t)c * Ho + yo) * Wo + xo] = v;
}

__global__ void space_to_depth_kernel(const float* __restrict__ x, float* __restrict__ out, int C, int H, int W,
                                      int64_t total) {
    const int64_t i = (int64_t)blockIdx.x * blockDim.x + threadIdx.x;
    if (i >= total) return;
    const int h2 = H >> 1, w2 = W >> 1;
    const int xx = (int)(i % w2), y = (int)((i / w2) % h2);
    const int cc = (int)((i / ((int64_t)w2 * h2)) % (4 * C)), b = (int)(i / ((int64_t)w2 * h2 * 4 * C));
    const int q = cc / C, c = cc - q * C;
    const int dy = q & 1, dx = q >> 1;
    out[i] = x[(((int64_t)b * C + c) * H + 2 * y + dy) * W + 2 * xx + dx];
}

__global__ void pixel_shuffle2_kernel(const float* __restrict__ x, float* __restrict__ out, int C, int H, int W,
                                      int64_t total) {
    const int64_t i = (int64_t)blockIdx.x * blockDim.x + threadIdx.x;
    if (i >= total) return;
    const int Wo = 2 * W, Ho = 2 * H;
    const int xo = (int)(i % Wo), yo = (int)((i / Wo) % Ho);
    const int c = (int)((i / ((int64_t)Wo * Ho)) % C), b = (int)(i / ((int64_t)Wo * Ho * C));
    const int ch = c * 4 + (yo & 1) * 2 + (xo & 1);
    out[i] = x[(((int64_t)b * 4 * C + ch) * H + (yo >> 1)) * W + (xo >> 1)];
}

__device__ __forceinline__ int reflect_idx(int i, int n) { return i < n ? i : 2 * (n - 1) - i; }

__global__ void pad_reflect_kernel(const float* __restrict__ x, float* __restrict__ out, int H, int W, int Hp, int Wp,
                                   int64_t total) {
    const int64_t i = (int64_t)blockIdx.x * blockDim.x + threadIdx.x;
    if (i >= total) return;
    const int xo = (int)(i % Wp), yo = (int)((i / Wp) % Hp);
    const int64_t plane = i / ((int64_t)Wp * Hp);
    out[i] = x[(plane * H + reflect_idx(yo, H)) * W + reflect_idx(xo, W)];
}

__global__ void resize_down_kernel(const float* __restrict__ x, float* __restrict__ out, int Hp, int Wp, int s,
                                   int64_t total) {
    const int64_t i = (int64_t)blockIdx.x * blockDim.x + threadIdx.x;
    if (i >= total) return;
    const int wd = Wp / s, hd = Hp / s;
    const int xo = (int)(i % wd), yo = (int)((i / wd) % hd);
    const int64_t plane = i / ((int64_t)wd * hd);
    const int a = s / 2 - 1;
    const float* p = x + (plane * Hp + (int64_t)yo * s + a) * Wp + (int64_t)xo * s + a;
    out[i] = 0.25f * (p[0] + p[Wp] + p[1] + p[Wp + 1]);
}

__global__ void randn_kernel(float* __restrict__ out, int64_t total, uint64_t seed, uint64_t stream_id, const uint64_t* __restrict__ stream_add) {
    const int64_t i = (int64_t)blockIdx.x * blockDim.x + threadIdx.x;
    if (stream_add) stream_id += stream_add[0];
    if (i < total) out[i] = philox_normal(i, seed, stream_id);
}

__global__ void bnn_sample_kernel(const float* __restrict__ mu, const float* __restrict__ rho,
                                  const float* __restrict__ eps_in, float* __restrict__ out, int64_t n, int64_t total,
                                  uint64_t seed, uint64_t stream_id, const uint64_t* __restrict__ stream_add) {
    const int64_t j = (int64_t)blockIdx.x * blockDim.x + threadIdx.x;
    const int64_t i0 = 4 * j;
    if (i0 >= total) return;
    if (stream_add) stream_id += stream_add[0];
    float z[4] = {0.f, 0.f, 0.f, 0.f};
    if (!eps_in) philox_normal4(j, seed, stream_id, z);
#pragma unroll
    for (int q = 0; q < 4; ++q) {
        const int64_t i = i0 + q;
        if (i < total) {
            const int64_t e = i % n;
            const float eps = eps_in ? eps_in[i] : z[q];
            out[i] = mu[e] + log1pf(expf(rho[e])) * eps;
        }
    }
}

__device__ __forceinline__ double block_sum(double v, double* sh) {
#pragma unroll
    for (int d = 32; d >= 1; d >>= 1) v += __shfl_down(v, d, 64);
    const int lane = threadIdx.x & 63, wave = threadIdx.x >> 6;
    __syncthreads();
    if (lane == 0) sh[wave] = v;
    __syncthreads();
    double s = 0;
    for (int w = 0; w < (int)(blockDim.x >> 6); ++w) s += sh[w];
// ... 174 lines not shown
    }
#pragma unroll
    for (int d = 32; d >= 1; d >>= 1) v += __shfl_xor(v, d, 64);
    if ((threadIdx.x & 63) == 0) red[threadIdx.x >> 6] = v;
    __syncthreads();
    if (threadIdx.x == 0) atomicAdd(acc + bn, red[0] + red[1] + red[2] + red[3]);
}
__global__ void ssim_final_kernel(const double* __restrict__ acc, float* __restrict__ out, int Bn, double inv) {
    const int i = blockIdx.x * blockDim.x + threadIdx.x;
    if (i < Bn) out[i] = (float)(acc[i] * inv);
}

__global__ void select_scores_kernel(const float* __restrict__ s1, const float* __restrict__ s2, double w, int rule, int* __restrict__ best,
                                     float* __restrict__ best_s1, float* __restrict__ best_s2, int B, int N) {
    const int b = blockIdx.x * blockDim.x + threadIdx.x;
    if (b >= B) return;
    const float* p = s1 + (int64_t)b * N;
    const float* q = s2 ? s2 + (int64_t)b * N : nullptr;
    int bi = 0;
    if (rule == 0) {
        double m1 = (double)p[0], m2 = q ? (double)q[0] : 1.0;
        for (int i = 1; i < N; ++i) { m1 = fmax(m1, (double)p[i]); if (q) m2 = fmax(m2, (double)q[i]); }
        double bs = -1e300;
        for (int i = 0; i < N; ++i) {
            const double sc = q ? w * (double)p[i] / m1 + (1.0 - w) * (double)q[i] / m2 : (double)p[i] / m1;
            if (sc > bs) { bs = sc; bi = i; }
        }
    } else {
        double bs = (double)p[0];
        for (int i = 1; i < N; ++i) {
            const double sc = (double)p[i];
            if (rule == 1 ? sc > bs : sc < bs) { bs = sc; bi = i; }
        }
    }
    best[b] = bi;
    if (best_s1) best_s1[b] = p[bi];
    if (best_s2 && q) best_s2[b] = q[bi];
}

__global__ __launch_bounds__(256) void mc_mean_kernel(const float* __restrict__ pred, float* __restrict__ out, double* __restrict__ gsum,
                                                     const float* __restrict__ target, int N, int Hp, int Wp, int h, int w) {
    __shared__ double sh[2][4];
    const int ch = blockIdx.y, b = blockIdx.z;
    const float gw = ch == 0 ? 0.114f : (ch == 1 ? 0.587f : 0.299f);
    double sm = 0.0, st = 0.0;
    const int64_t hw = (int64_t)h * w;
    for (int64_t i = (int64_t)blockIdx.x * 256 + threadIdx.x; i < hw; i += (int64_t)gridDim.x * 256) {
        const int y = (int)(i / w), x = (int)(i % w);
        float a = 0.f;
        for (int n = 0; n < N; ++n) a += fminf(fmaxf(pred[(((int64_t)b * N + n) * 3 + ch) * Hp * Wp + (int64_t)y * Wp + x], 0.f), 1.f);
        a = fminf(fmaxf(a / (float)N, 0.f), 1.f);
        out[((int64_t)b * 3 + ch) * hw + i] = a;
        sm += (double)(gw * a);
        if (target) st += (double)(gw * target[((int64_t)b * 3 + ch) * hw + i]);
    }
#pragma unroll
    for (int d = 32; d >= 1; d >>= 1) { sm += __shfl_xor(sm, d, 64); st += __shfl_xor(st, d, 64); }
    if ((threadIdx.x & 63) == 0) { sh[0][threadIdx.x >> 6] = sm; sh[1][threadIdx.x >> 6] = st; }
    __syncthreads();
    if (threadIdx.x == 0 && gsum) {
        atomicAdd(gsum + 2 * b, sh[0][0] + sh[0][1] + sh[0][2] + sh[0][3]);
        atomicAdd(gsum + 2 * b + 1, sh[1][0] + sh[1][1] + sh[1][2] + sh[1][3]);
    }
}
__global__ void mc_rescale_kernel(float* __restrict__ out, const double* __restrict__ gsum, int64_t chw, int64_t total) {
    const int64_t i = (int64_t)blockIdx.x * blockDim.x + threadIdx.x;
    if (i >= total) return;
    const int64_t b = i / chw;
    const float ratio = (float)(gsum[2 * b + 1] / gsum[2 * b]);
    out[i] = fminf(fmaxf(out[i] * ratio, 0.f), 1.f);
}

}

extern "C" int bem_quat_dwt_f32(const float* rgb, int64_t x_bstride, float* out, int B, int H, int W, void* stream) {
    BEM_REQUIRE(rgb && out, "quat_dwt: null tensor");
    BEM_REQUIRE(B >= 0 && H > 0 && W > 0 && H % 2 == 0 && W % 2 == 0, "quat_dwt: H, W must be even (got %d x %d)", H, W);
    if (B == 0) return BEM_OK;
    const int64_t total = (int64_t)B * (H / 2) * (W / 2);
    quat_dwt_kernel<<<GRID1D(total), 256, 0, (hipStream_t)stream>>>(rgb, x_bstride, out, H, W, total);
    return bem_check_launch("quat_dwt");
}

extern "C" int bem_dwt_f32(const float* x, float* out, int B, int C, int H, int W, void* stream) {
    BEM_REQUIRE(x && out, "dwt: null tensor");
    BEM_REQUIRE(B >= 0 && C > 0 && H > 0 && W > 0 && H % 2 == 0 && W % 2 == 0, "dwt: H, W must be even");
    if (B == 0) return BEM_OK;
    const int64_t total = (int64_t)B * C * (H / 2) * (W / 2);
    dwt_kernel<<<GRID1D(total), 256, 0, (hipStream_t)stream>>>(x, out, C, H, W, total);
    return bem_check_launch("dwt");
}

extern "C" int bem_iwt_f32(const float* x, float* out, int B, int C4, int H, int W, void* stream) {
    BEM_REQUIRE(x && out, "iwt: null tensor");
    BEM_REQUIRE(B >= 0 && C4 > 0 && C4 % 4 == 0 && H > 0 && W > 0, "iwt: channels %d must be a multiple of 4", C4);
    if (B == 0) return BEM_OK;
    const int64_t total = (int64_t)B * (C4 / 4) * H * W;
    iwt_kernel<<<GRID1D(total), 256, 0, (hipStream_t)stream>>>(x, out, C4 / 4, H, W, total);
    return bem_check_launch("iwt");
}

extern "C" int bem_iwt_hamilton_f32(const float* q1w, const float* q2w, float* out, int B, int h, int w, void* stream) {
    BEM_REQUIRE(q1w && q2w && out, "iwt_hamilton: null tensor");
    BEM_REQUIRE(B >= 0 && h > 0 && w > 0, "iwt_hamilton: bad shape");
    if (B == 0) return BEM_OK;
    const int64_t total = (int64_t)B * h * w;
    iwt_hamilton_kernel<<<GRID1D(total), 256, 0, (hipStream_t)stream>>>(q1w, q2w, out, h, w, total);
    return bem_check_launch("iwt_hamilton");
}

extern "C" int bem_hamilton_full_f32(const float* q1, const float* q2, float* out, int B, int H, int W, void* stream) {
    BEM_REQUIRE(q1 && q2 && out && B >= 0 && H > 0 && W > 0, "hamilton_full: bad arguments");
    if (B == 0) return BEM_OK;
    const int64_t total = (int64_t)B * H * W;
    hamilton_full_kernel<<<GRID1D(total), 256, 0, (hipStream_t)stream>>>(q1, q2, out, (int64_t)H * W, total);
    return bem_check_launch("hamilton_full");
}

extern "C" int bem_hamilton_f32(const float* q, float* out, int B, int H, int W, void* stream) {
    BEM_REQUIRE(q && out, "hamilton: null tensor");
    BEM_REQUIRE(B >= 0 && H > 0 && W > 0, "hamilton: bad shape");
    if (B == 0) return BEM_OK;
    const int64_t total = (int64_t)B * H * W;
    hamilton_kernel<<<GRID1D(total), 256, 0, (hipStream_t)stream>>>(q, out, (int64_t)H * W, total);
    return bem_check_launch("hamilton");
}

extern "C" int bem_attn_stats_f64(const float* f1, const float* f2, double* stats, int B, int L, void* stream) {
    BEM_REQUIRE(f1 && f2 && stats, "attn_stats: null tensor");
    BEM_REQUIRE(B >= 0 && B <= 65535 && L > 0, "attn_stats: bad shape");
    if (B == 0) return BEM_OK;
    hipStream_t s = (hipStream_t)stream;
    if (hipMemsetAsync(stats, 0, sizeof(double) * (size_t)B * (ATT_C * ATT_C + 2 * ATT_C), s) != hipSuccess)
        return bem_check_launch("attn_stats memset");
    dim3 grid(cdiv(L, ATT_CHUNK), B);
    attn_stats_kernel<<<grid, 256, 0, s>>>(f1, f2, stats, L);
    return bem_check_launch("attn_stats");
}

extern "C" int bem_attn_fold_f32(const double* stats, const float* attn_w, const float* fuse_w, const float* fuse_b,
                                 float* Wp_out, float* bias_out, int B, int L, void* stream) {
    BEM_REQUIRE(stats && attn_w && fuse_w && fuse_b && Wp_out && bias_out, "attn_fold: null tensor");
    BEM_REQUIRE(B >= 0 && L > 0, "attn_fold: bad shape");
    if (B == 0) return BEM_OK;
    attn_fold_kernel<<<B, 1024, 0, (hipStream_t)stream>>>(stats, attn_w, fuse_w, fuse_b, Wp_out, bias_out, L);
    return bem_check_launch("attn_fold");
}

extern "C" int bem_transpose_planes_f32(const float* src, int64_t src_bstride, float* dst, int64_t dst_bstride,
                                        int nbatch, int ppb, int H, int W, void* stream) {
    BEM_REQUIRE(src && dst, "transpose_planes: null tensor");
    BEM_REQUIRE(nbatch >= 0 && ppb > 0 && H > 0 && W > 0, "transpose_planes: bad shape");
    BEM_REQUIRE((int64_t)nbatch * ppb <= 65535 && cdiv(H, 32) <= 65535, "transpose_planes: too many planes (%lld)", (long long)nbatch * ppb);
    if (nbatch == 0) return BEM_OK;
    dim3 grid(cdiv(W, 32), cdiv(H, 32), nbatch * ppb);
    transpose_planes_kernel<<<grid, 256, 0, (hipStream_t)stream>>>(src, src_bstride, dst, dst_bstride, ppb, H, W);
    return bem_check_launch("transpose_planes");
}

extern "C" int bem_copy_channels_f32(const float* src, int64_t src_bstride, float* dst, int64_t dst_bstride, int B,
                                     int C, int L, void* stream) {
    BEM_REQUIRE(src && dst, "copy_channels: null tensor");
    BEM_REQUIRE(B >= 0 && C > 0 && L >= 0, "copy_channels: bad shape");
    const int64_t total = (int64_t)B * C * L;
    if (total == 0) return BEM_OK;
    copy_channels_kernel<<<GRID1D(total), 256, 0, (hipStream_t)stream>>>(src, src_bstride, dst, dst_bstride, (int64_t)C * L, total);
// ... 216 lines not shown
```

### bayesian-enhancement-model_amd/csrc/pw_gemm_x6.hip

```cpp
#include "bem_common.h"
#include "x6_common.h"
#include <stdlib.h>
#include <algorithm>

namespace {


struct PwX {
    const float* x1; const float* x2; int C1; int C2; int in_mode;
    const float* ln_w; const float* ln_b; float ln_eps;
    const u32x4* Wp; int64_t w_bstride;
    const float* bias; int64_t bias_bstride;
    const float* res; const float* prelu; int act;
    float* out; int out_mode; int Win;
    int M; int K; int L; int KB; int MT;
    int mtpb;
};


template <int NSUB, bool SUM, bool VEC>
__device__ __forceinline__ void ldx(const PwX& k, int b, int ch, int pc, const bool (&keep)[NSUB], float (&o)[NSUB]) {
    const int chc = min(ch, k.K - 1);
    const bool first = chc < k.C1;
    const float* r1 = k.x1 + ((int64_t)b * k.C1 + (first ? chc : 0)) * k.L;
// ... 693 lines not shown

extern "C" int bem_pw_gemm_x6_f32(const bem_pw_args* a, void* stream) {
    BEM_REQUIRE(a, "pw_gemm_x6: null args");
    BEM_REQUIRE(a->x1 && a->Wp && a->out, "pw_gemm_x6: null tensor");
    BEM_REQUIRE(a->B >= 0 && a->B <= 65535 && a->M > 0 && a->M <= BEM_X6_MAXM && a->K > 0 && a->L >= 0, "pw_gemm_x6: bad shape B=%d M=%d K=%d L=%d", a->B, a->M, a->K, a->L);
    BEM_REQUIRE(a->in_mode >= 0 && a->in_mode <= 2, "pw_gemm_x6: in_mode %d", a->in_mode);
    if (a->in_mode == 0) BEM_REQUIRE(a->K == a->C1, "pw_gemm_x6: K %d != C1 %d", a->K, a->C1);
    if (a->in_mode == 1) BEM_REQUIRE(a->x2 && a->K == a->C1 && a->C1 == a->C2, "pw_gemm_x6: sum mode needs x2 and K == C1 == C2");
    if (a->in_mode == 2) BEM_REQUIRE(a->x2 && a->K == a->C1 + a->C2, "pw_gemm_x6: cat mode needs x2 and K == C1 + C2");
    BEM_REQUIRE((a->ln_w == nullptr) == (a->ln_b == nullptr), "pw_gemm_x6: ln_w / ln_b must both be set or both NULL");
    BEM_REQUIRE(a->act == 0 || (a->act == 1 && a->prelu), "pw_gemm_x6: act %d", a->act);
    BEM_REQUIRE(a->out_mode == 0 || (a->out_mode == 1 && a->M % 4 == 0 && a->Win > 0 && a->L % a->Win == 0 && !a->res),
                "pw_gemm_x6: out_mode %d constraints", a->out_mode);
    BEM_REQUIRE(((uintptr_t)a->Wp & 15) == 0 && a->w_bstride % 4 == 0, "pw_gemm_x6: packed weights must be 16-byte aligned");
    BEM_REQUIRE((int64_t)a->M * a->L < (1ll << 30), "pw_gemm_x6: M * L = %lld exceeds the 32-bit lane offsets of the epilogue", (long long)a->M * a->L);
    const bool ln = a->ln_w != nullptr;
    BEM_REQUIRE(!ln || a->K <= BEM_X6_MAXK_LN, "pw_gemm_x6: LayerNorm prologue supports K <= %d (got %d)", BEM_X6_MAXK_LN, a->K);
    if (a->B == 0 || a->L == 0) return BEM_OK;
    PwX k;
    k.x1 = a->x1; k.x2 = a->x2 ? a->x2 : a->x1; k.C1 = a->C1; k.C2 = a->x2 ? a->C2 : a->C1; k.in_mode = a->in_mode;
    k.ln_w = a->ln_w; k.ln_b = a->ln_b; k.ln_eps = a->ln_eps;
    k.Wp = reinterpret_cast<const u32x4*>(a->Wp); k.w_bstride = a->w_bstride / 4; k.bias = a->bias; k.bias_bstride = a->bias_bstride;
    k.res = a->res; k.prelu = a->prelu; k.act = a->act; k.out = a->out; k.out_mode = a->out_mode; k.Win = a->Win;
    k.M = a->M; k.K = a->K; k.L = a->L; k.KB = cdiv(a->K, 16); k.MT = cdiv(a->M, 32); k.mtpb = k.MT;
    hipStream_t s = (hipStream_t)stream;
    const bool sum = a->in_mode == 1;
    const bool al = (((uintptr_t)a->x1 | (uintptr_t)(a->x2 ? a->x2 : a->x1) | (uintptr_t)a->out | (uintptr_t)(a->res ? a->res : a->out)) & 7) == 0;
    const bool vec = a->L % 2 == 0 && al;
#define BEM_X6_RES(KBM, NSUB, MTW)                                                                       \
    do {                                                                                                 \
        dim3 grid(cdiv(a->L, 128 * NSUB), 1, a->B);                                                      \
                    \
        const int64_t wv = (int64_t)a->B * cdiv(a->L, 32 * NSUB);                                        \
        const int groups = cdiv(k.MT, MTW);                                                              \
        const int ny = wv >= 2048 ? 1 : (int)std::min<int64_t>(groups, cdiv64(2048, wv));                \
        k.mtpb = cdiv(groups, ny) * MTW;                                                                 \
        grid.y = cdiv(k.MT, k.mtpb);                                                                     \
        if (NSUB == 2 && vec && !sum) pw_x6_res_kernel<KBM, NSUB, MTW, false, true><<<grid, 256, 0, s>>>(k);   \
        else if (NSUB == 2 && vec) pw_x6_res_kernel<KBM, NSUB, MTW, true, true><<<grid, 256, 0, s>>>(k);       \
        else if (!sum) pw_x6_res_kernel<KBM, NSUB, MTW, false, false><<<grid, 256, 0, s>>>(k);                 \
        else pw_x6_res_kernel<KBM, NSUB, MTW, true, false><<<grid, 256, 0, s>>>(k);                            \
        return bem_check_launch("pw_x6_res");                                                            \
    } while (0)
    if (k.KB <= 3) BEM_X6_RES(3, 2, 1);
    if (ln && k.KB <= 5) BEM_X6_RES(5, 2, 1);
    static const bool res10 = !(getenv("BEM_X6_RES10") && atoi(getenv("BEM_X6_RES10")) == 0);
    static const bool reslds = !(getenv("BEM_X6_RES_LDS") && atoi(getenv("BEM_X6_RES_LDS")) == 0);
    if (ln && k.KB == 10 && k.K == 160 && k.MT >= 8 && res10 && reslds && (int64_t)a->B * cdiv(a->L, 32) >= 2048) {
        dim3 grid(cdiv(a->L, 128), 1, a->B);
        k.mtpb = k.MT;
        if (!sum) pw_x6_res_lds_kernel<10, false, false><<<grid, 256, 0, s>>>(k);
        else pw_x6_res_lds_kernel<10, true, false><<<grid, 256, 0, s>>>(k);
        return bem_check_launch("pw_x6_res_lds");
    }
    if (ln && k.KB <= 10 && res10) { if (k.MT == 1) BEM_X6_RES(10, 1, 1); else BEM_X6_RES(10, 1, 2); }
#undef BEM_X6_RES
    {
        const bool three = false && k.MT == 3 && !ln;
        const int mtw = three ? 3 : (k.MT == 1 ? 1 : 2);
        dim3 grid(cdiv(a->L, three ? 128 : 256), cdiv(k.MT, mtw), a->B);
#define BEM_X6_STREAM(MTW, LN)                                                                \
    do {                                                                                      \
        if (vec && !sum) pw_x6_stream_kernel<MTW, 2, false, true, LN><<<grid, 256, 0, s>>>(k);   \
        else if (vec) pw_x6_stream_kernel<MTW, 2, true, true, LN><<<grid, 256, 0, s>>>(k);       \
        else if (!sum) pw_x6_stream_kernel<MTW, 2, false, false, LN><<<grid, 256, 0, s>>>(k);    \
        else pw_x6_stream_kernel<MTW, 2, true, false, LN><<<grid, 256, 0, s>>>(k);               \
    } while (0)
        if (three) {
            if (!sum) pw_x6_stream_kernel<3, 1, false, false, false><<<grid, 256, 0, s>>>(k);
            else pw_x6_stream_kernel<3, 1, true, false, false><<<grid, 256, 0, s>>>(k);
        }
        else if (ln) { if (mtw == 1) BEM_X6_STREAM(1, true); else BEM_X6_STREAM(2, true); }
        else { if (mtw == 1) BEM_X6_STREAM(1, false); else BEM_X6_STREAM(2, false); }
#undef BEM_X6_STREAM
    }
    return bem_check_launch("pw_x6_stream");
}

namespace {

struct CvX {
    const float* x; int64_t x_bs;
    const u32x4* Wp; const float* bias; const float* res1; const float* res2; float* out;
    int Cin, H, W, Ho, Wo, Cout, KB, MT, relu, pad, dil;
};

template <int MTW, int KH, int KW, int S>
__global__ __launch_bounds__(256, 2) void conv_taps_x6_kernel(CvX k) {
    constexpr int NSUB = 2, NTAP = KH * KW;
    const int lane = threadIdx.x & 63, wave = threadIdx.x >> 6, kh = lane >> 5, n = lane & 31;
    const int b = blockIdx.z, mt0 = blockIdx.y * MTW;
    const int Lo = k.Ho * k.Wo, Li = k.H * k.W;
    const int p0 = (xcd_tile(blockIdx.x, gridDim.x) * 4 + wave) * 64;
    if (p0 >= Lo) return;
    const int p = p0 + 2 * n;
    const bool live = p < Lo;
    const int pc = live ? p : 0;
    const int yo = pc / k.Wo, xo = pc - yo * k.Wo;
    const int yi0 = yo * S - k.pad, xi0 = xo * S - k.pad;
    const float* xb = k.x + (int64_t)b * k.x_bs;
    f32x16 acc[MTW][NSUB], alo[MTW][NSUB];
#pragma unroll
    for (int m = 0; m < MTW; ++m)
#pragma unroll
        for (int t = 0; t < NSUB; ++t)
#pragma unroll
            for (int r = 0; r < 16; ++r) acc[m][t][r] = alo[m][t][r] = 0.f;
    const u32x4* wbase = k.Wp + lane;
    const int64_t tap_stride = (int64_t)k.MT * k.KB * 3 * 64, mt_stride = (int64_t)k.KB * 3 * 64;
    const int nsteps = k.KB * NTAP;
    auto load_x = [&](int s, float (&dst)[8][NSUB], float (&mk)[NSUB]) {
        const int kb = min(s / NTAP, k.KB - 1), tap = s - (s / NTAP) * NTAP;
        const int ky = tap / KW, kx = tap - ky * KW;
        const int yy = yi0 + ky * k.dil, x0 = xi0 + kx * k.dil, x1 = x0 + S;
        const bool rowok = live && yy >= 0 && yy < k.H;
        mk[0] = (rowok && x0 >= 0 && x0 < k.W) ? 1.f : 0.f;
        mk[1] = (rowok && x1 >= 0 && x1 < k.W) ? 1.f : 0.f;
        const int q = yy * k.W + x0;
        const int c0 = 16 * kb, hoff = (c0 + 8 < k.Cin) ? 8 * kh : 0;
        if (S == 1) {
            const int qb = min(max(q, 0), Li - 2), d = q - qb;
#pragma unroll
            for (int e = 0; e < 8; ++e) {
                const float* pl = xb + (int64_t)(min(c0 + e, k.Cin - 1 - hoff) + hoff) * Li;
                float2 v;
                __builtin_memcpy(&v, pl + qb, sizeof(v));
                dst[e][0] = d > 0 ? v.y : v.x;
                dst[e][1] = d < 0 ? v.x : v.y;
            }
        } else {
            const int q0 = min(max(q, 0), Li - 1), q1 = min(max(q + S, 0), Li - 1);
#pragma unroll
            for (int e = 0; e < 8; ++e) {
                const float* pl = xb + (int64_t)(min(c0 + e, k.Cin - 1 - hoff) + hoff) * Li;
                dst[e][0] = pl[q0];
                dst[e][1] = pl[q1];
            }
        }
    };
    auto load_w = [&](int s, u32x4 (&dst)[MTW][3]) {
        const int sc = min(s, nsteps - 1), kb = sc / NTAP, tap = sc - kb * NTAP;
#pragma unroll
        for (int m = 0; m < MTW; ++m) {
            const bool ok = s < nsteps && mt0 + m < k.MT;
            const u32x4* wp = wbase + tap * tap_stride + (int64_t)(mt0 + m < k.MT ? mt0 + m : 0) * mt_stride + (int64_t)kb * 3 * 64;
            const uint32_t mk = ok ? 0xffffffffu : 0u;
#pragma unroll
            for (int li = 0; li < 3; ++li) {
                const u32x4 w = wp[li * 64];
                dst[m][li] = u32x4{w[0] & mk, w[1] & mk, w[2] & mk, w[3] & mk};
            }
        }
    };
    float xn[8][NSUB], mkn[NSUB];
    u32x4 wn[MTW][3];
    load_x(0, xn, mkn);
    load_w(0, wn);
    for (int s = 0; s < nsteps; ++s) {
        u32x4 xl[NSUB][3], wc[MTW][3];
#pragma unroll
        for (int t = 0; t < NSUB; ++t) {
            float v[8];
#pragma unroll
            for (int e = 0; e < 8; ++e) v[e] = xn[e][t] * mkn[t];
            split8(v, xl[t][0], xl[t][1], xl[t][2]);
        }
#pragma unroll
        for (int m = 0; m < MTW; ++m)
#pragma unroll
            for (int li = 0; li < 3; ++li) wc[m][li] = wn[m][li];
        load_x(s + 1, xn, mkn);
        load_w(s + 1, wn);
#pragma unroll
        for (int m = 0; m < MTW; ++m)
#pragma unroll
            for (int t = 0; t < NSUB; ++t) mac6(wc[m], xl[t], acc[m][t], alo[m][t]);
    }
    const float lo = k.relu ? 0.f : -3.402823466e38f;
    const uint32_t loff = (uint32_t)(4 * kh) * (uint32_t)Lo + (uint32_t)pc;
    float* outb = k.out + (int64_t)b * k.Cout * Lo;
    const float* r1b = k.res1 ? k.res1 + (int64_t)b * k.Cout * Lo : nullptr;
    const float* r2b = k.res2 ? k.res2 + (int64_t)b * k.Cout * Lo : nullptr;
#pragma unroll
    for (int m = 0; m < MTW; ++m) {
        if (mt0 + m >= k.MT) continue;
        const int rb = (mt0 + m) * 32;
#pragma unroll
        for (int g = 0; g < 4; ++g) {
            float bv[4], rv[4][NSUB];
#pragma unroll
            for (int i = 0; i < 4; ++i) {
                const int urow = rb + 8 * g + i;
                const int lrow = min(urow + 4 * kh, k.Cout - 1);
                bv[i] = k.bias ? k.bias[lrow] : 0.f;
                rv[i][0] = rv[i][1] = 0.f;
                const uint32_t ro = (uint32_t)lrow * (uint32_t)Lo + (uint32_t)pc;
                if (r1b) { const float2 q = *reinterpret_cast<const float2*>(r1b + ro); rv[i][0] += q.x; rv[i][1] += q.y; }
                if (r2b) { const float2 q = *reinterpret_cast<const float2*>(r2b + ro); rv[i][0] += q.x; rv[i][1] += q.y; }
            }
#pragma unroll
            for (int i = 0; i < 4; ++i) {
                const int r = 4 * g + i, urow = rb + 8 * g + i;
                const float o0 = fmaxf(acc[m][0][r] + alo[m][0][r] + bv[i], lo) + rv[i][0];
                const float o1 = fmaxf(acc[m][1][r] + alo[m][1][r] + bv[i], lo) + rv[i][1];
                if (live && urow + 4 * kh < k.Cout) *reinterpret_cast<float2*>(outb + (int64_t)urow * Lo + loff) = make_float2(o0, o1);
            }
        }
    }
}

}

static int conv_taps_launch(const float* x, int64_t x_bstride, const float* Wp, const float* bias, const float* res1, const float* res2,
                            float* out, int B, int Cin, int H, int W, int Cout, int KH, int stride, int dil, int relu, void* stream, const char* what) {
    BEM_REQUIRE(x && Wp && out, "%s: null tensor", what);
    BEM_REQUIRE(B >= 0 && B <= 65535 && Cin > 0 && Cout > 0 && H > 0 && W > 0, "%s: bad shape", what);
    BEM_REQUIRE((KH == 3 && stride == 1 && (dil == 1 || dil == 2)) || (KH == 3 && stride == 2 && dil == 1),
                "%s: supported forms are 3x3 s1 (dilation 1 / 2, padding = dilation) and 3x3 s2 p1", what);
    const int pad = dil;
    const int Ho = (H + 2 * pad - dil * (KH - 1) - 1) / stride + 1, Wo = (W + 2 * pad - dil * (KH - 1) - 1) / stride + 1;
    BEM_REQUIRE(Ho > 0 && Wo > 0 && Wo % 2 == 0 && Cin % 8 == 0 && H * W >= 2, "%s: needs an even output width and Cin %% 8 == 0 (got Wo=%d Cin=%d)", what, Wo, Cin);
    BEM_REQUIRE(((uintptr_t)Wp & 15) == 0 && (((uintptr_t)out | (uintptr_t)(res1 ? res1 : out) | (uintptr_t)(res2 ? res2 : out)) & 7) == 0,
                "%s: alignment (packed weights 16 bytes, out / residuals 8 bytes)", what);
    BEM_REQUIRE((int64_t)Cout * Ho * Wo < (1ll << 30) && (int64_t)Cin * H * W < (1ll << 30), "%s: plane set too large for 32-bit lane offsets", what);
    if (B == 0) return BEM_OK;
    CvX k;
    k.x = x; k.x_bs = x_bstride; k.Wp = reinterpret_cast<const u32x4*>(Wp); k.bias = bias; k.res1 = res1; k.res2 = res2; k.out = out;
    k.Cin = Cin; k.H = H; k.W = W; k.Ho = Ho; k.Wo = Wo; k.Cout = Cout; k.KB = cdiv(Cin, 16); k.MT = cdiv(Cout, 32); k.relu = relu; k.pad = pad; k.dil = dil;
    const int mtw = k.MT == 1 ? 1 : 2;
    dim3 grid(cdiv(Ho * Wo, 256), cdiv(k.MT, mtw), B);
    hipStream_t s = (hipStream_t)stream;
    if (KH == 3 && stride == 1) {
        if (mtw == 1) conv_taps_x6_kernel<1, 3, 3, 1><<<grid, 256, 0, s>>>(k);
        else conv_taps_x6_kernel<2, 3, 3, 1><<<grid, 256, 0, s>>>(k);
    } else {
        if (mtw == 1) conv_taps_x6_kernel<1, 3, 3, 2><<<grid, 256, 0, s>>>(k);
        else conv_taps_x6_kernel<2, 3, 3, 2><<<grid, 256, 0, s>>>(k);
    }
    return bem_check_launch(what);
}

extern "C" int bem_conv4x4s2_fast_supported(int Cin, int H, int W);
extern "C" int bem_conv3x3_rows_supported(int Cin, int H, int W);
int conv_rows_launch(int KS, const float* x, int64_t x_bstride, const float* Wp, const float* bias, const float* res1, const float* res2, float* out,
                     int B, int Cin, int H, int W, int Cout, int relu, void* stream);
static bool rows_aligned(const float* x, int64_t x_bstride, const float* out, const float* res1, const float* res2) {
    return x && out && (((uintptr_t)x | (uintptr_t)out | (uintptr_t)(res1 ? res1 : out) | (uintptr_t)(res2 ? res2 : out)) & 15) == 0 && x_bstride % 4 == 0;
}

extern "C" int bem_conv3x3_x6_f32(const float* x, int64_t x_bstride, const float* Wp, const float* bias, const float* res1,
                                  const float* res2, float* out, int B, int Cin, int H, int W, int Cout, int relu, void* stream) {
    static const bool rows = !(getenv("BEM_CONV3_ROWS") && atoi(getenv("BEM_CONV3_ROWS")) == 0);
    if (rows && Cin > 0 && bem_conv3x3_rows_supported(Cin, H, W) && rows_aligned(x, x_bstride, out, res1, res2))
        return conv_rows_launch(3, x, x_bstride, Wp, bias, res1, res2, out, B, Cin, H, W, Cout, relu, stream);
    return conv_taps_launch(x, x_bstride, Wp, bias, res1, res2, out, B, Cin, H, W, Cout, 3, 1, 1, relu, stream, "conv3x3_x6");
}


extern "C" int bem_conv4x4s2_x6_f32(const float* x, int64_t x_bstride, const float* Wp, const float* bias, const float* res1,
                                    const float* res2, float* out, int B, int Cin, int H, int W, int Cout, int relu, void* stream) {
    BEM_REQUIRE(Cin > 0 && bem_conv4x4s2_fast_supported(Cin, H, W) && rows_aligned(x, x_bstride, out, res1, res2),
                "conv4x4s2_x6: needs W = 2 Wo with Wo a power of two <= 64, even H, Cin %% 8 == 0 and 16-byte aligned tensors");
    return conv_rows_launch(4, x, x_bstride, Wp, bias, res1, res2, out, B, Cin, H, W, Cout, relu, stream);
}

extern "C" int bem_conv_taps_x6_f32(const float* x, int64_t x_bstride, const float* Wp, const float* bias, const float* res1, const float* res2,
                                    float* out, int B, int Cin, int H, int W, int Cout, int K, int stride, int dilation, int relu, void* stream) {
    return conv_taps_launch(x, x_bstride, Wp, bias, res1, res2, out, B, Cin, H, W, Cout, K, stride, dilation, relu, stream, "conv_taps_x6");
}
```

### include/bem_hip.h

```cpp
#ifndef BEM_HIP_H
#define BEM_HIP_H

#include <stdint.h>

#ifdef __cplusplus
extern "C" {
#endif

#define BEM_OK 0
#define BEM_ERR_INVALID 1
#define BEM_ERR_LAUNCH 2

const char* bem_last_error(void);
int bem_abi_version(void);


int bem_selective_scan_fwd_f32(const float* u, const float* delta, const float* A, const float* Bm,
                               const float* Cm, const float* D, const float* delta_bias, float* out,
                               int batch, int dim, int L, int dstate, int ngroups, int delta_softplus,
                               void* stream);

int bem_selective_scan_fwd_in16(const void* u, const void* delta, const float* A, const void* Bm, const void* Cm, const float* D,
                                const float* delta_bias, float* out, int in_dtype, int batch, int dim, int L, int dstate,
                                int ngroups, int delta_softplus, void* stream);

int bem_cast16_to_f32(const void* src, float* dst, int64_t n, int dtype, void* stream);
int bem_cast_f32_to16(const float* src, void* dst, int64_t n, int dtype, void* stream);

int64_t bem_selective_scan_bwd_ws_elems(int batch, int dim, int L, int dstate);
int bem_selective_scan_bwd_f32(const float* u, const float* delta, const float* A, const float* Bm, const float* Cm,
                               const float* D, const float* delta_bias, const float* dout, float* ws, float* du,
                               float* ddelta, float* dA, float* dB, float* dC, float* dD, float* ddelta_bias,
                               int batch, int dim, int L, int dstate, int ngroups, int delta_softplus, void* stream);

int bem_cross_scan_f32(const float* x, float* xs, int B, int C, int H, int W, void* stream);
int bem_cross_merge_f32(const float* ys, float* y, int B, int C, int H, int W, void* stream);

int bem_ss2d_scan_strided_f32(const float* x0, const float* x1, const float* xd0, const float* xd1,
                              const float* dtw, const float* dtb, const float* A, const float* Ds,
                              float* y0, float* y1, int B, int C, int L, int R, int64_t xd0_bstride, int64_t xd1_bstride,
                              void* stream);

int bem_ss2d_scan_rm_supported(int H, int W, int R);
int bem_ss2d_scan_rm_f32(const float* x, const float* xd0, const float* xd1, const float* dtw, const float* dtb,
                         const float* A, const float* Ds, float* y0, float* y1, int B, int C, int H, int W, int R,
                         int64_t xd0_bstride, int64_t xd1_bstride, void* stream);

int bem_ss2d_scan_n_supported(int N);
int bem_ss2d_scan_n_f32(const float* x0, const float* x1, const float* xd0, const float* xd1, const float* dtw, const float* dtb,
                        const float* A, const float* Ds, float* y0, float* y1, int B, int C, int L, int R, int N,
                        int64_t xd0_bstride, int64_t xd1_bstride, void* stream);

typedef struct {
    const float* x1; const float* x2; int C1; int C2; int in_mode;
    const float* ln_w; const float* ln_b; float ln_eps;
    const float* Wp; int64_t w_bstride;
    const float* bias; int64_t bias_bstride;
    const float* res;
    const float* prelu; int act;
    float* out; int out_mode; int Win;
    int B; int M; int K; int L;
} bem_pw_args;
int bem_pack_pw_weight_f32(const float* W, float* Wp, int nsets, int M, int K, void* stream);
int64_t bem_pw_packed_elems(int M, int K);

int bem_pw_gemm_x6_f32(const bem_pw_args* a, void* stream);
int bem_pack_pw_weight_x6(const float* W, float* Wp, int nsets, int M, int K, void* stream);
int bem_pack_pw_weight_x6_strided(const float* W, float* Wp, int nsets, int M, int K, int64_t set_stride, int64_t row_stride,
                                  int64_t col_stride, void* stream);
int bem_pack_pw_weight_x6_jobs(const void* jobs, const void* blks, int nblk, float* arena, void* stream);
int64_t bem_pw_x6_packed_elems(int M, int K);
int bem_bnn_sample_pack_x6(const float* mu, const float* rho, const float* eps, float* Wp, int nsets, int M, int K,
                           uint64_t seed, uint64_t stream_id, const uint64_t* stream_add, int sigma_given,
                           void* stream);

int bem_dwconv3x3_f32(const float* x, const float* w, int64_t w_bstride, const float* bias,
                      int64_t bias_bstride, float* out, int B, int Cout, int H, int W, int mode, void* stream);

int bem_conv2d_f32(const float* x, int64_t x_bstride, const float* w, const float* bias, const float* res1,
                   const float* res2, float* out, int B, int Cin, int H, int W, int Cout, int KH, int KW,
                   int stride, int pad, int relu, void* stream);

int bem_conv2d_mfma_f32(const float* x, int64_t x_bstride, const float* Wp, const float* bias, const float* res1,
                        const float* res2, float* out, int B, int Cin, int H, int W, int Cout, int KH, int KW,
                        int stride, int pad, int relu, void* stream);

int bem_conv3x3_x6_f32(const float* x, int64_t x_bstride, const float* Wp, const float* bias, const float* res1,
                       const float* res2, float* out, int B, int Cin, int H, int W, int Cout, int relu, void* stream);
int bem_conv4x4s2_fast_supported(int Cin, int H, int W);
int bem_conv3x3_rows_supported(int Cin, int H, int W);
int bem_conv4x4s2_x6_f32(const float* x, int64_t x_bstride, const float* Wp, const float* bias, const float* res1,
                         const float* res2, float* out, int B, int Cin, int H, int W, int Cout, int relu, void* stream);

int bem_conv_taps_x6_f32(const float* x, int64_t x_bstride, const float* Wp, const float* bias, const float* res1, const float* res2,
                         float* out, int B, int Cin, int H, int W, int Cout, int K, int stride, int dilation, int relu, void* stream);

int bem_quat_dwt_f32(const float* rgb, int64_t x_bstride, float* out, int B, int H, int W, void* stream);
int bem_dwt_f32(const float* x, float* out, int B, int C, int H, int W, void* stream);
int bem_iwt_f32(const float* x, float* out, int B, int C4, int H, int W, void* stream);
int bem_iwt_hamilton_f32(const float* q1w, const float* q2w, float* out, int B, int h, int w, void* stream);
int bem_hamilton_f32(const float* q, float* out, int B, int H, int W, void* stream);

int bem_hamilton_full_f32(const float* q1, const float* q2, float* out, int B, int H, int W, void* stream);

int bem_attn_stats_f64(const float* f1, const float* f2, double* stats, int B, int L, void* stream);
int bem_attn_fold_f32(const double* stats, const float* attn_w ,
                      const float* fuse_w , const float* fuse_b ,
                      float* W_out , float* bias_out , int B, int L,
                      void* stream);

int bem_transpose_planes_f32(const float* src, int64_t src_bstride, float* dst, int64_t dst_bstride,
                             int nbatch, int ppb, int H, int W, void* stream);
int bem_copy_channels_f32(const float* src, int64_t src_bstride, float* dst, int64_t dst_bstride,
                          int B, int C, int L, void* stream);
int bem_copy_channels_rep_f32(const float* src, int64_t src_bstride, float* dst, int64_t dst_bstride, int B, int C, int L, int rep,
                              void* stream);
int bem_add_channels_f32(const float* src, int64_t src_bstride, float* dst, int64_t dst_bstride,
                         int B, int C, int L, void* stream);
int bem_bilinear_up_f32(const float* src, int64_t src_bstride, float* dst, int64_t dst_bstride,
                        int B, int C, int H, int W, int s, void* stream);
int bem_space_to_depth_f32(const float* x, float* out, int B, int C, int H, int W, void* stream);
int bem_pixel_shuffle2_f32(const float* x, float* out, int B, int C, int H, int W, void* stream);

int bem_bnn_ebank_sample_f32(const void* segs, const void* blks, int nblk, float* arena, uint64_t seed, uint64_t stream_base, void* stream);

int bem_row_scale_f32(const float* w, const float* scale, float* out, int M, int K, void* stream);
int bem_se_gate_f32(const float* mean, const float* w1, const float* w2, float* y, int B, int C, int Cr, void* stream);
int bem_spatial_attention_f32(const float* x, const float* chan_scale, const float* w, float* map_ws, float* out, int B, int C, int H, int W,
                              int k, void* stream);

int bem_chan_scale_f32(const float* x, const float* scale, int64_t scale_bstride, const float* add, const float* add_bc, float add_bc_scale,
                       float* out, int B, int C, int64_t HW, void* stream);
int bem_chan_dot_f32(const float* a, const float* b, float* out, int B, int C, int64_t HW, int per_batch, void* stream);
int bem_se_gate_bwd_f32(const float* mean, const float* w1, const float* w2, const float* y, const float* dy, float* dmean, float* dw1,
                        float* dw2, int B, int C, int Cr, void* stream);
int bem_spatial_attention_bwd_f32(const float* x, const float* dout, const float* map, const float* w, float* dpre_ws, float* dx, float* dw,
                                  int B, int C, int H, int W, int k, void* stream);

int bem_bnn_sample_f32(const float* mu, const float* rho, const float* eps_in, float* out,
                       int nsets, int64_t n, uint64_t seed, uint64_t stream_id, const uint64_t* stream_add, void* stream);
int bem_pad_reflect_f32(const float* x, float* out, int P, int H, int W, int Hp, int Wp, void* stream);
int bem_resize_down_f32(const float* x, float* out, int P, int Hp, int Wp, int s, void* stream);
int bem_randn_f32(float* out, int64_t n, uint64_t seed, uint64_t stream_id, const uint64_t* stream_add, void* stream);
int bem_cond_postproc_f32(const float* pred, const float* target_mean, const float* noise, float* out,
                          int Bn, int h, int w, int samples_per_image, float noise_level, void* stream);
int bem_plane_mean_f32(const float* x, float* means, int P, int Hs, int Ws, int h, int w, void* stream);
int bem_candidate_finalize_f32(const float* pred, const float* target, float* final_out, float* psnr, double* ws,
                               int Bn, int samples_per_image, int Hp, int Wp, int h, int w, int gt_mean,
                               void* stream);

int bem_select_best_f32(const float* cand, const float* psnr, int* best, float* best_psnr, float* best_img, int B, int N,
                        int64_t chw, void* stream);

int bem_ssim_f32(const float* pred, const float* target, float* ssim, double* ws, int Bn, int samples_per_image, int h, int w, void* stream);

int bem_select_scores_f32(const float* cand, const float* s1, const float* s2, float weight, int rule, int* best, float* best_s1,
                          float* best_s2, float* best_img, int B, int N, int64_t chw, void* stream);

int bem_niqe_f32(const float* final, const double* mu_pris, const double* cov_pris, const double* window, const double* gam_tab, int ntab,
                 const float* rs_wh, const int* rs_ih, int kh, const float* rs_ww, const int* rs_iw, int kw, double* scores, void* ws,
                 int64_t ws_bytes, int Bn, int h, int w, void* stream);
int64_t bem_niqe_ws_bytes(int Bn, int h, int w);

int bem_uiqm_uciqe_f32(const float* final, const int* lab_tab, const int* rs_bh, const int* rs_kh, int kh, const int* rs_bv, const int* rs_kv,
                       int kv, double* uiqm, double* uciqe, void* ws, int64_t ws_bytes, int Bn, int h, int w, int Hr, void* stream);
int64_t bem_uiqm_ws_bytes(int Bn, int h, int w, int Hr);

int bem_mc_mean_f32(const float* pred, const float* target, float* out, double* ws, int B, int N, int Hp, int Wp, int h, int w,
                    int gt_mean, void* stream);

int bem_gdmlp_x6_f32(const float* x, const float* ln_w, const float* ln_b, float ln_eps, const float* Wp_gate,
                     const float* bias_gate, const float* dw_gate10, const float* Wp_out,
                     const float* bias_out, float* out, int B, int C, int Hd, int H, int W, void* stream);

int bem_ss2d_front_x6_f32(const float* x, const float* ln_w, const float* ln_b, float ln_eps, const float* Wp_in, const float* bias_in,
                          const float* dww, const float* dwb, const float* Wp_x, float* xc, float* xd, int B, int C, int Mx, int H, int W,
                          void* stream);


int bem_l1_loss_f32(const float* pred, const float* gt, float* dpred, float* loss, double* ws, int64_t n, float weight,
// ... 90 lines not shown
```

Before: 317.0.

## Split first conv by image/cond channels and fuse bilinear upsample into cond DWT

The first convolution of each branch is split into an image part and a condition part. The image part runs once per image on the side stream, and its result is broadcast across the N Bayesian samples through a new res1_rep residual index. A new cond_dwt kernel fuses the bilinear upsampling of the conditions into the quaternion DWT, and the per-branch 32-channel concatenation copies are dropped. The aim is to cut redundant image convolution work and intermediate memory traffic. The cost is extra kernel parameters and a broadcast residual index in every conv variant.

Result: faster. 321.2 (median of 6 runs) (+1.3%).

```diff
diff --git a/bayesian-enhancement-model_amd/bem/archs.py b/bayesian-enhancement-model_amd/bem/archs.py
--- a/bayesian-enhancement-model_amd/bem/archs.py
+++ b/bayesian-enhancement-model_amd/bem/archs.py
@@ -107,8 +107,11 @@
 
     def forward(self, x, c0=0):
         _need_cuda(x)
+        return self.forward_from_dwt(ops.quat_dwt(x, c0))
+
+    def forward_from_dwt(self, d):
+        _need_cuda(d)
         P = self._prepared()
-        d = ops.quat_dwt(x, c0)
         feat = self.conv_in(d)
         if self.model == "model3" and not self.wavelet_out:
             if self.training and torch.is_grad_enabled():
@@ -237,10 +240,10 @@
         self.last_act = _check_last_act(last_act)
         self.apply(_init_weights)
 
-    def _dual_unet(self, qs):
+    def _dual_unet(self, qs, first_kw=({}, {})):
         feats, skips = [], []
-        for br, q in zip(("_Q1", "_Q2"), qs):
-            f, sk = self._encode(br, q)
+        for br, q, kw in zip(("_Q1", "_Q2"), qs, first_kw):
+            f, sk = self._encode(br, q, **kw)
             feats.append(f)
             skips.append(sk)
         fused = self.bottleneck_block(self.bottleneck_fuse(feats[0], x2=feats[1], in_mode=2))
@@ -258,11 +261,24 @@
     def decompose(self, x, c0):
         return self.decomp(x, c0)
 
-    def forward_decomposed(self, d_img, d_cond, img_index=None):
+    def decompose_cond(self, conds, scale):
+        return self.decomp.forward_from_dwt(ops.cond_dwt(conds, scale))
+
+    def first_conv_image(self, d_img):
+        fcs = [getattr(self, "first_conv" + br) for br in ("_Q1", "_Q2")]
+        return [ops.conv2d(d_img, fc.weight_part(0, 16), fc.bias.detach(), pad=1, cin_slice=(16 * bi, 16)) for bi, fc in enumerate(fcs)]
+
+    def forward_decomposed(self, d_img, d_cond, img_index=None, p_img=None):
         B, _, h, w = d_cond.shape
         spi = 1 if img_index is None else int(img_index)
         if d_img.shape[0] * spi != B:
             raise ValueError("forward_decomposed: image / sample batch mismatch")
+        if not grad_mode(self):
+            if p_img is None:
+                p_img = self.first_conv_image(d_img)
+            o1, o2 = self._dual_unet((d_cond, d_cond), [dict(cin_slice=(16 * bi, 16), w_part=(16, 16), use_bias=False, res1=p_img[bi], res1_rep=spi)
+                                                        for bi in range(2)])
+            return ops.iwt_hamilton(o1, o2)
 
         def branch_input(bi):
             q = torch.empty(B, 32, h, w, device=d_cond.device, dtype=d_cond.dtype)
diff --git a/bayesian-enhancement-model_amd/bem/modules.py b/bayesian-enhancement-model_amd/bem/modules.py
--- a/bayesian-enhancement-model_amd/bem/modules.py
+++ b/bayesian-enhancement-model_amd/bem/modules.py
@@ -153,14 +153,23 @@
 
 class Conv2dK(nn.Conv2d):
 
-    def forward(self, x, relu=False, res1=None, res2=None, cin_slice=None):
+    def __init__(self, *a, **k):
+        super().__init__(*a, **k)
+        self._cache = _Cache()
+
+    def weight_part(self, c0, n):
+        return self._cache.get(("part", c0, n), [self.weight], lambda: self.weight.detach()[:, c0:c0 + n].contiguous())
+
+    def forward(self, x, relu=False, res1=None, res2=None, cin_slice=None, res1_rep=1, w_part=None, use_bias=True):
         _need_cuda(x)
         if grad_mode(self) and self.weight.requires_grad:
-            if relu or res1 is not None or res2 is not None:
+            if relu or res1 is not None or res2 is not None or w_part is not None or not use_bias:
                 raise BemNativeError("Conv2dK: the training path covers the plain convolution (+ bias) only")
             return ag.Conv2dFn.apply(x, self.weight, self.bias, self, cin_slice)
-        return ops.conv2d(x, self.weight.detach(), None if self.bias is None else self.bias.detach(),
-                          stride=self.stride[0], pad=self.padding[0], relu=relu, res1=res1, res2=res2, cin_slice=cin_slice, dilation=self.dilation[0])
+        w = self.weight.detach() if w_part is None else self.weight_part(*w_part)
+        return ops.conv2d(x, w, self.bias.detach() if (use_bias and self.bias is not None) else None,
+                          stride=self.stride[0], pad=self.padding[0], relu=relu, res1=res1, res2=res2, cin_slice=cin_slice, dilation=self.dilation[0],
+                          res1_rep=res1_rep)
 
 
 class ConvT2x2(nn.ConvTranspose2d):
diff --git a/bayesian-enhancement-model_amd/bem/native.py b/bayesian-enhancement-model_amd/bem/native.py
--- a/bayesian-enhancement-model_amd/bem/native.py
+++ b/bayesian-enhancement-model_amd/bem/native.py
@@ -84,16 +84,17 @@
     "bem_prelu_bwd_f32": [P, P, P, P, P, I64, P],
     "bem_bilinear_up_bwd_f32": [P, P, I, I, I, I, I, P],
     "bem_gdmlp_x6_f32": [P, P, P, F, P, P, P, P, P, P, I, I, I, I, I, P],
-    "bem_conv3x3_x6_f32": [P, I64, P, P, P, P, P, I, I, I, I, I, I, P],
+    "bem_conv3x3_x6_f32": [P, I64, P, P, P, P, P, I, I, I, I, I, I, I, P],
     "bem_conv4x4s2_x6_f32": [P, I64, P, P, P, P, P, I, I, I, I, I, I, P],
     "bem_conv4x4s2_fast_supported": [I, I, I],
     "bem_conv3x3_rows_supported": [I, I, I],
     "bem_ss2d_front_x6_f32": [P, P, P, F, P, P, P, P, P, P, P, I, I, I, I, I, P],
-    "bem_conv_taps_x6_f32": [P, I64, P, P, P, P, P, I, I, I, I, I, I, I, I, I, P],
+    "bem_conv_taps_x6_f32": [P, I64, P, P, P, P, P, I, I, I, I, I, I, I, I, I, I, P],
     "bem_dwconv3x3_f32": [P, P, I64, P, I64, P, I, I, I, I, I, P],
-    "bem_conv2d_f32": [P, I64, P, P, P, P, P, I, I, I, I, I, I, I, I, I, I, P],
-    "bem_conv2d_mfma_f32": [P, I64, P, P, P, P, P, I, I, I, I, I, I, I, I, I, I, P],
+    "bem_conv2d_f32": [P, I64, P, P, P, P, P, I, I, I, I, I, I, I, I, I, I, I, P],
+    "bem_conv2d_mfma_f32": [P, I64, P, P, P, P, P, I, I, I, I, I, I, I, I, I, I, I, P],
     "bem_quat_dwt_f32": [P, I64, P, I, I, I, P],
+    "bem_cond_dwt_f32": [P, P, I, I, I, I, P],
     "bem_dwt_f32": [P, P, I, I, I, I, P],
     "bem_iwt_f32": [P, P, I, I, I, I, P],
     "bem_iwt_hamilton_f32": [P, P, P, I, I, I, P],
diff --git a/bayesian-enhancement-model_amd/bem/ops.py b/bayesian-enhancement-model_amd/bem/ops.py
--- a/bayesian-enhancement-model_amd/bem/ops.py
+++ b/bayesian-enhancement-model_amd/bem/ops.py
@@ -402,7 +402,7 @@
     return hit[1]
 
 
-def conv2d(x, w, bias=None, stride=1, pad=1, relu=False, res1=None, res2=None, cin_slice=None, dilation=1):
+def conv2d(x, w, bias=None, stride=1, pad=1, relu=False, res1=None, res2=None, cin_slice=None, dilation=1, res1_rep=1):
     _chk(x, "x"); _chk(w, "w"); _chk(bias, "bias", optional=True)
     _chk(res1, "res1", optional=True); _chk(res2, "res2", optional=True)
     B, Ct, H, W = x.shape
@@ -416,25 +416,29 @@
         raise ValueError(f"conv2d: input has {Ct} channels, weight expects {Cin}")
     Ho, Wo = (H + 2 * pad - dilation * (KH - 1) - 1) // stride + 1, (W + 2 * pad - dilation * (KW - 1) - 1) // stride + 1
     out = torch.empty(B, Cout, Ho, Wo, device=x.device, dtype=x.dtype)
+    res1_rep = int(res1_rep)
+    if res1_rep < 1 or (res1_rep != 1 and res1 is None):
+        raise ValueError("conv2d: res1_rep must be >= 1 and needs res1")
+    res_shapes = (("res1", res1, (B // res1_rep if B % res1_rep == 0 else -1,) + tuple(out.shape[1:])), ("res2", res2, tuple(out.shape)))
     if dilation != 1 or (KH, KW, stride) == (3, 3, 2):
         if (KH, KW) != (3, 3) or pad != dilation or Wo % 2 or Cin % 8 or (c0 * H * W) % 2:
             raise ValueError("conv2d: dilated / strided 3x3 convolutions run in the tap form only (pad = dilation, even output width, Cin % 8 == 0)")
-        for n, r in (("res1", res1), ("res2", res2)):
-            if r is not None and r.shape != out.shape:
+        for n, r, shp in res_shapes:
+            if r is not None and tuple(r.shape) != shp:
                 raise ValueError(f"conv2d: {n} shape")
         xp_ = ctypes.c_void_p(x.data_ptr() + 4 * c0 * H * W)
         check(lib().bem_conv_taps_x6_f32(xp_, Ct * H * W, _p(_packed_conv_weight_x6(w)), _p(bias), _p(res1), _p(res2), _p(out), B, Cin, H, W, Cout, 3, stride,
-                                         dilation, int(relu), _stream()), "conv_taps_x6")
+                                         dilation, int(relu), res1_rep, _stream()), "conv_taps_x6")
         return out
-    for n, r in (("res1", res1), ("res2", res2)):
-        if r is not None and r.shape != out.shape:
+    for n, r, shp in res_shapes:
+        if r is not None and tuple(r.shape) != shp:
             raise ValueError(f"conv2d: {n} shape")
     if bias is not None and bias.shape != (Cout,):
         raise ValueError("conv2d: bias shape")
     xp = ctypes.c_void_p(x.data_ptr() + 4 * c0 * H * W)
     if USE_CONV_X6 and (KH, KW, stride, pad) == (3, 3, 1, 1) and W % 2 == 0 and Cin % 8 == 0 and (c0 * H * W) % 2 == 0:
         check(lib().bem_conv3x3_x6_f32(xp, Ct * H * W, _p(_packed_conv_weight_x6(w)), _p(bias), _p(res1), _p(res2), _p(out), B, Cin, H, W,
-                                       Cout, int(relu), _stream()), "conv3x3_x6")
+                                       Cout, int(relu), res1_rep, _stream()), "conv3x3_x6")
         return out
     conv4_fast = CONV4_FAST and (KH, KW, stride, pad) == (4, 4, 2, 1) and res1 is None and res2 is None and (c0 * H * W) % 4 == 0 \
         and (Ct * H * W) % 4 == 0 and x.data_ptr() % 16 == 0 and lib().bem_conv4x4s2_fast_supported(Cin, H, W) == 1
@@ -444,10 +448,10 @@
         return out
     if USE_CONV_MFMA and Cout <= 160 and ((KH, KW, stride) in ((3, 3, 1), (4, 4, 2))):
         check(lib().bem_conv2d_mfma_f32(xp, Ct * H * W, _p(_packed_conv_weight(w)), _p(bias), _p(res1), _p(res2), _p(out), B, Cin, H, W,
-                                        Cout, KH, KW, stride, pad, int(relu), _stream()), "conv2d_mfma")
+                                        Cout, KH, KW, stride, pad, int(relu), res1_rep, _stream()), "conv2d_mfma")
         return out
     check(lib().bem_conv2d_f32(xp, Ct * H * W, _p(w), _p(bias), _p(res1), _p(res2), _p(out), B, Cin, H, W, Cout, KH, KW,
-                               stride, pad, int(relu), _stream()), "conv2d")
+                               stride, pad, int(relu), res1_rep, _stream()), "conv2d")
     return out
 
 
@@ -458,6 +462,17 @@
         raise ValueError("quat_dwt: needs 3 channels and even H, W")
     out = torch.empty(B, 32, H // 2, W // 2, device=x.device, dtype=x.dtype)
     check(lib().bem_quat_dwt_f32(ctypes.c_void_p(x.data_ptr() + 4 * c0 * H * W), Ct * H * W, _p(out), B, H, W, _stream()), "quat_dwt")
+    return out
+
+
+def cond_dwt(conds, s):
+    _chk(conds, "conds")
+    s = int(s)
+    R, C, H, W = conds.shape
+    if C != 3 or s < 1 or (H * s) % 2 or (W * s) % 2:
+        raise ValueError("cond_dwt: needs 3 channels and even enlarged H, W")
+    out = torch.empty(R, 32, H * s // 2, W * s // 2, device=conds.device, dtype=conds.dtype)
+    check(lib().bem_cond_dwt_f32(_p(conds), _p(out), R, H, W, s, _stream()), "cond_dwt")
     return out
 
 
diff --git a/bayesian-enhancement-model_amd/bem/pipeline.py b/bayesian-enhancement-model_amd/bem/pipeline.py
--- a/bayesian-enhancement-model_amd/bem/pipeline.py
+++ b/bayesian-enhancement-model_amd/bem/pipeline.py
@@ -40,13 +40,14 @@
         hd, wd = img_down.shape[-2:]
         x1 = img_down[:, None].expand(B, N, 3, hd, wd).reshape(B * N, 3, hd, wd)
         hoist = hasattr(self.net2, "forward_decomposed")
-        d_img, main = None, torch.cuda.current_stream()
+        d_img, p_img, main = None, None, torch.cuda.current_stream()
         if hoist and os.environ.get("BEM_DECOMP_OVERLAP", "1") != "0":
             if self._side is None or self._side.device != pad.device:
                 self._side = torch.cuda.Stream(device=pad.device)
             self._side.wait_stream(main)
             with torch.cuda.stream(self._side):
                 d_img = self.net2.decompose(pad, 0)
+                p_img = self.net2.first_conv_image(d_img)
             pad.record_stream(self._side)
         set_prediction_type(self.net1, deterministic)
         with sampling(None if deterministic else SampleCtx(B * N, eps, seed, rank=rank)) as ctx:
@@ -55,16 +56,18 @@
         if noise is None and self.noise_level:
             noise = ops.randn(tuple(pred.shape), pred.device, seed, (1 << 62) | (rank << 44) | SampleCtx._epoch)
         conds = ops.cond_postproc(pred, tmean, noise if self.noise_level else None, N, self.noise_level)
-        cond_up = ops.bilinear_up(conds, self.scale)
         if hoist:
             if d_img is None:
                 d_img = self.net2.decompose(pad, 0)
+                p_img = self.net2.first_conv_image(d_img)
             else:
                 main.wait_stream(self._side)
-                d_img.record_stream(main)
-            d_cond = self.net2.decompose(cond_up, 0)
-            raw = self.net2.forward_decomposed(d_img, d_cond, None if N == 1 else N)
+                for t in [d_img] + p_img:
+                    t.record_stream(main)
+            d_cond = self.net2.decompose_cond(conds, self.scale)
+            raw = self.net2.forward_decomposed(d_img, d_cond, None if N == 1 else N, p_img=p_img)
         else:
+            cond_up = ops.bilinear_up(conds, self.scale)
             x2 = torch.empty(B * N, 6, Hp, Wp, device=pad.device, dtype=pad.dtype)
             ops.copy_channels(pad[:, None].expand(B, N, 3, Hp, Wp).reshape(B * N, 3, Hp, Wp).contiguous(), x2, 0)
             ops.copy_channels(cond_up, x2, 3)
diff --git a/bayesian-enhancement-model_amd/csrc/conv.hip b/bayesian-enhancement-model_amd/csrc/conv.hip
--- a/bayesian-enhancement-model_amd/csrc/conv.hip
+++ b/bayesian-enhancement-model_amd/csrc/conv.hip
@@ -188,7 +188,7 @@
                                                      const float* __restrict__ w, const float* __restrict__ bias,
                                                      const float* __restrict__ res1, const float* __restrict__ res2,
                                                      float* __restrict__ out, int Cin, int H, int W, int Cout,
-                                                     int Ho, int Wo, int pad, int relu, int tilesX) {
+                                                     int Ho, int Wo, int pad, int relu, int tilesX, int res1_rep) {
     constexpr int PH = (TH - 1) * S + KH, PW = (TW - 1) * S + KW;
     constexpr int PWP = PW + 1;
     __shared__ float patch[CIB][PH][PWP];
@@ -248,7 +248,7 @@
         float v = acc[o] + (bias ? bias[co] : 0.f);
         if (relu) v = fmaxf(v, 0.f);
         const int64_t idx = (((int64_t)b * Cout + co) * Ho + oy) * Wo + ox;
-        if (res1) v += res1[idx];
+        if (res1) v += res1[(((int64_t)(b / res1_rep) * Cout + co) * Ho + oy) * Wo + ox];
         if (res2) v += res2[idx];
         out[idx] = v;
     }
@@ -265,7 +265,7 @@
 template <int MTW>
 __device__ __forceinline__ void conv_mfma_epilogue(f32x16 (&acc)[MTW][2], const float* __restrict__ Wp, const float* __restrict__ bias,
                                                    const float* __restrict__ res1, const float* __restrict__ res2,
-                                                   float* __restrict__ out, int b, int Cout, int Ho, int Wo, int ty0, int tx0,
+                                                   float* __restrict__ out, int b, int b1, int Cout, int Ho, int Wo, int ty0, int tx0,
                                                    int wave, int half, int j, int relu) {
     const int ox = tx0 + j, oxc = min(ox, Wo - 1);
     const float* bp = bias ? bias : Wp;
@@ -274,6 +274,7 @@
     const float bmk = bias ? 1.f : 0.f, m1 = res1 ? 1.f : 0.f, m2 = res2 ? 1.f : 0.f;
     const int64_t k0 = bias ? -1 : 0, k1 = res1 ? -1 : 0, k2 = res2 ? -1 : 0;
     const float lo = relu ? 0.f : -3.402823466e38f;
+    const int64_t b1off = (int64_t)(b1 - b) * Cout * Ho * Wo;
 #pragma unroll
     for (int t = 0; t < 2; ++t) {
         const int oy = ty0 + 2 * wave + t, oyc = min(oy, Ho - 1);
@@ -290,7 +291,7 @@
                     const int co = min(m * 32 + (r & 3) + 8 * (r >> 2) + 4 * half, Cout - 1);
                     const int64_t idx = (((int64_t)b * Cout + co) * Ho + oyc) * Wo + oxc;
                     bv[q] = bp[co & k0] * bmk;
-                    r1[q] = p1[idx & k1] * m1;
+                    r1[q] = p1[(idx + b1off) & k1] * m1;
                     r2[q] = p2[idx & k2] * m2;
                 }
 #pragma unroll
@@ -310,7 +311,7 @@
                                                           const float* __restrict__ Wp, const float* __restrict__ bias,
                                                           const float* __restrict__ res1, const float* __restrict__ res2,
                                                           float* __restrict__ out, int Cin, int H, int W, int Cout,
-                                                          int Ho, int Wo, int pad, int relu, int tilesX, int KS) {
+                                                          int Ho, int Wo, int pad, int relu, int tilesX, int KS, int res1_rep) {
     constexpr int KK = KH * KW;
     constexpr int KC = CIB * KK;
     constexpr int PH = (TH - 1) * S + KH, PW = (TW - 1) * S + KW, PWP = PW + 1;
@@ -392,7 +393,7 @@
             }
         }
     }
-    conv_mfma_epilogue<MTW>(acc, Wp, bias, res1, res2, out, b, Cout, Ho, Wo, ty0, tx0, wave, half, j, relu);
+    conv_mfma_epilogue<MTW>(acc, Wp, bias, res1, res2, out, b, b / res1_rep, Cout, Ho, Wo, ty0, tx0, wave, half, j, relu);
 }
 
 template <int KH, int KW, int S, int MTW>
@@ -400,7 +401,7 @@
                                                                const float* __restrict__ Wp, const float* __restrict__ bias,
                                                                const float* __restrict__ res1, const float* __restrict__ res2,
                                                                float* __restrict__ out, int Cin, int H, int W, int Cout,
-                                                               int Ho, int Wo, int pad, int relu, int tilesX, int KS) {
+                                                               int Ho, int Wo, int pad, int relu, int tilesX, int KS, int res1_rep) {
     constexpr int KK = KH * KW;
     constexpr int KC = CIB * KK;
     constexpr int NS = KC / 2;
@@ -504,7 +505,7 @@
         __syncthreads();
         buf ^= 1;
     }
-    conv_mfma_epilogue<MTW>(acc, Wp, bias, res1, res2, out, b, Cout, Ho, Wo, ty0, tx0, wave, half, j, relu);
+    conv_mfma_epilogue<MTW>(acc, Wp, bias, res1, res2, out, b, b / res1_rep, Cout, Ho, Wo, ty0, tx0, wave, half, j, relu);
 }
 
 }
@@ -533,8 +534,8 @@
 
 extern "C" int bem_conv2d_f32(const float* x, int64_t x_bstride, const float* w, const float* bias,
                               const float* res1, const float* res2, float* out, int B, int Cin, int H, int W,
-                              int Cout, int KH, int KW, int stride, int pad, int relu, void* stream) {
-    BEM_REQUIRE(x && w && out, "conv2d: null tensor");
+                              int Cout, int KH, int KW, int stride, int pad, int relu, int res1_rep, void* stream) {
+    BEM_REQUIRE(x && w && out && res1_rep >= 1, "conv2d: null tensor or res1_rep < 1");
     BEM_REQUIRE(B >= 0 && B <= 65535 && Cin > 0 && Cout > 0 && H > 0 && W > 0, "conv2d: bad shape");
     const int Ho = (H + 2 * pad - KH) / stride + 1, Wo = (W + 2 * pad - KW) / stride + 1;
     BEM_REQUIRE(Ho > 0 && Wo > 0, "conv2d: empty output");
@@ -543,9 +544,9 @@
     dim3 grid(tilesX * tilesY, cdiv(Cout, COB), B);
     hipStream_t s = (hipStream_t)stream;
     if (KH == 3 && KW == 3 && stride == 1)
-        conv2d_kernel<3, 3, 1><<<grid, 256, 0, s>>>(x, x_bstride, w, bias, res1, res2, out, Cin, H, W, Cout, Ho, Wo, pad, relu, tilesX);
+        conv2d_kernel<3, 3, 1><<<grid, 256, 0, s>>>(x, x_bstride, w, bias, res1, res2, out, Cin, H, W, Cout, Ho, Wo, pad, relu, tilesX, res1_rep);
     else if (KH == 4 && KW == 4 && stride == 2)
-        conv2d_kernel<4, 4, 2><<<grid, 256, 0, s>>>(x, x_bstride, w, bias, res1, res2, out, Cin, H, W, Cout, Ho, Wo, pad, relu, tilesX);
+        conv2d_kernel<4, 4, 2><<<grid, 256, 0, s>>>(x, x_bstride, w, bias, res1, res2, out, Cin, H, W, Cout, Ho, Wo, pad, relu, tilesX, res1_rep);
     else
         BEM_REQUIRE(false, "conv2d: unsupported kernel %dx%d stride %d (have 3x3 s1, 4x4 s2)", KH, KW, stride);
     return bem_check_launch("conv2d");
@@ -553,8 +554,8 @@
 
 extern "C" int bem_conv2d_mfma_f32(const float* x, int64_t x_bstride, const float* Wp, const float* bias,
                                    const float* res1, const float* res2, float* out, int B, int Cin, int H, int W,
-                                   int Cout, int KH, int KW, int stride, int pad, int relu, void* stream) {
-    BEM_REQUIRE(x && Wp && out, "conv2d_mfma: null tensor");
+                                   int Cout, int KH, int KW, int stride, int pad, int relu, int res1_rep, void* stream) {
+    BEM_REQUIRE(x && Wp && out && res1_rep >= 1, "conv2d_mfma: null tensor or res1_rep < 1");
     BEM_REQUIRE(B >= 0 && B <= 65535 && Cin > 0 && Cout > 0 && Cout <= 160 && H > 0 && W > 0, "conv2d_mfma: bad shape (Cout <= 160)");
     const int Ho = (H + 2 * pad - KH) / stride + 1, Wo = (W + 2 * pad - KW) / stride + 1;
     BEM_REQUIRE(Ho > 0 && Wo > 0, "conv2d_mfma: empty output");
@@ -564,12 +565,12 @@
     dim3 grid(tilesX * tilesY, B);
     hipStream_t s = (hipStream_t)stream;
 #define BEM_CONV_LAUNCH(KH_, KW_, S_, MTW_) \
-    conv2d_mfma_kernel<KH_, KW_, S_, MTW_><<<grid, 256, 0, s>>>(x, x_bstride, Wp, bias, res1, res2, out, Cin, H, W, Cout, Ho, Wo, pad, relu, tilesX, KS)
+    conv2d_mfma_kernel<KH_, KW_, S_, MTW_><<<grid, 256, 0, s>>>(x, x_bstride, Wp, bias, res1, res2, out, Cin, H, W, Cout, Ho, Wo, pad, relu, tilesX, KS, res1_rep)
     if (KH == 3 && KW == 3 && stride == 1) {
         static const bool pipe = !(getenv("BEM_CONV_PIPE") && getenv("BEM_CONV_PIPE")[0] == '0');
         if (MT <= 2 && pipe) {
-            if (MT == 1) conv2d_mfma_pipe_kernel<3, 3, 1, 1><<<grid, 256, 0, s>>>(x, x_bstride, Wp, bias, res1, res2, out, Cin, H, W, Cout, Ho, Wo, pad, relu, tilesX, KS);
-            else conv2d_mfma_pipe_kernel<3, 3, 1, 2><<<grid, 256, 0, s>>>(x, x_bstride, Wp, bias, res1, res2, out, Cin, H, W, Cout, Ho, Wo, pad, relu, tilesX, KS);
+            if (MT == 1) conv2d_mfma_pipe_kernel<3, 3, 1, 1><<<grid, 256, 0, s>>>(x, x_bstride, Wp, bias, res1, res2, out, Cin, H, W, Cout, Ho, Wo, pad, relu, tilesX, KS, res1_rep);
+            else conv2d_mfma_pipe_kernel<3, 3, 1, 2><<<grid, 256, 0, s>>>(x, x_bstride, Wp, bias, res1, res2, out, Cin, H, W, Cout, Ho, Wo, pad, relu, tilesX, KS, res1_rep);
         }
         else if (MT == 1) BEM_CONV_LAUNCH(3, 3, 1, 1);
         else if (MT == 2) BEM_CONV_LAUNCH(3, 3, 1, 2);
diff --git a/bayesian-enhancement-model_amd/csrc/conv_rows_x6.hip b/bayesian-enhancement-model_amd/csrc/conv_rows_x6.hip
--- a/bayesian-enhancement-model_amd/csrc/conv_rows_x6.hip
+++ b/bayesian-enhancement-model_amd/csrc/conv_rows_x6.hip
@@ -7,7 +7,7 @@
 struct CrX {
     const float* x; int64_t x_bs;
     const u32x4* Wp; const float* bias; const float* res1; const float* res2; float* out;
-    int Cin, H, W, Ho, Wo, Cout, KB, MT, wo_shift, relu, mt_first;
+    int Cin, H, W, Ho, Wo, Cout, KB, MT, wo_shift, relu, mt_first, res1_rep;
 };
 
 typedef float f32x4v __attribute__((ext_vector_type(4)));
@@ -98,6 +98,7 @@
         typedef float fpx __attribute__((ext_vector_type(NPX)));
         const float lo = k.relu ? 0.f : -3.402823466e38f;
         const int64_t ob = (int64_t)b * k.Cout * Lo + pc;
+        const float* r1b = k.res1 + (int64_t)(b / k.res1_rep) * k.Cout * Lo + pc;
 #pragma unroll
         for (int m = 0; m < MTW; ++m)
 #pragma unroll
@@ -109,7 +110,7 @@
                     fpx v;
 #pragma unroll
                     for (int j = 0; j < NPX; ++j) v[j] = fmaxf(acc[m][j][r] + alo[m][j][r] + bv, lo);
-                    if (k.res1) v += *reinterpret_cast<const fpx*>(k.res1 + o);
+                    if (k.res1) v += *reinterpret_cast<const fpx*>(r1b + (int64_t)row * Lo);
                     if (k.res2) v += *reinterpret_cast<const fpx*>(k.res2 + o);
                     *reinterpret_cast<fpx*>(k.out + o) = v;
                 }
@@ -128,9 +129,10 @@
 }
 
 int conv_rows_launch(int KS, const float* x, int64_t x_bstride, const float* Wp, const float* bias, const float* res1, const float* res2, float* out,
-                     int B, int Cin, int H, int W, int Cout, int relu, void* stream) {
+                     int B, int Cin, int H, int W, int Cout, int relu, int res1_rep, void* stream) {
     const char* what = KS == 4 ? "conv4x4s2_x6" : "conv3x3_x6";
     BEM_REQUIRE(x && Wp && out, "%s: null tensor", what);
+    BEM_REQUIRE(res1_rep >= 1, "%s: res1_rep %d", what, res1_rep);
     BEM_REQUIRE(B >= 0 && B <= 65535 && Cin > 0 && Cout > 0 && (KS == 4 ? bem_conv4x4s2_fast_supported(Cin, H, W) : bem_conv3x3_rows_supported(Cin, H, W)),
                 "%s: shape outside the row form", what);
     BEM_REQUIRE((((uintptr_t)Wp | (uintptr_t)x | (uintptr_t)out | (uintptr_t)(res1 ? res1 : out) | (uintptr_t)(res2 ? res2 : out)) & 15) == 0 && (x_bstride % 4) == 0,
@@ -140,7 +142,7 @@
     if (B == 0) return BEM_OK;
     CrX k;
     k.x = x; k.x_bs = x_bstride; k.Wp = reinterpret_cast<const u32x4*>(Wp); k.bias = bias; k.res1 = res1; k.res2 = res2; k.out = out;
-    k.Cin = Cin; k.H = H; k.W = W; k.Ho = Ho; k.Wo = Wo; k.Cout = Cout; k.KB = cdiv(Cin, 16); k.MT = cdiv(Cout, 32); k.relu = relu;
+    k.Cin = Cin; k.H = H; k.W = W; k.Ho = Ho; k.Wo = Wo; k.Cout = Cout; k.KB = cdiv(Cin, 16); k.MT = cdiv(Cout, 32); k.relu = relu; k.res1_rep = res1_rep;
     k.wo_shift = __builtin_ctz(Wo);
     hipStream_t s = (hipStream_t)stream;
     if (KS == 4) {
diff --git a/bayesian-enhancement-model_amd/csrc/elementwise.hip b/bayesian-enhancement-model_amd/csrc/elementwise.hip
--- a/bayesian-enhancement-model_amd/csrc/elementwise.hip
+++ b/bayesian-enhancement-model_amd/csrc/elementwise.hip
@@ -8,6 +8,22 @@
 namespace {
 
 #define GRID1D(n) dim3((unsigned)cdiv64((n), 256))
+
+__device__ __forceinline__ void quat_stack(float r, float g, float bl, float (&q)[8][4], int s) {
+    const float den = fmaxf(fmaxf(r, g), bl) + 1e-7f;
+    q[0][s] = 0.f; q[1][s] = 0.f;
+    q[2][s] = r / den; q[3][s] = r;
+    q[4][s] = g / den; q[5][s] = g;
+    q[6][s] = bl / den; q[7][s] = bl;
+}
+
+__device__ __forceinline__ void haar_bands(const float (&q)[4], float (&o)[4]) {
+    const float a = q[0] / 2, bb = q[1] / 2, cc = q[2] / 2, d = q[3] / 2;
+    o[0] = a + bb + cc + d;
+    o[1] = -a - bb + cc + d;
+    o[2] = -a + bb - cc + d;
+    o[3] = a - bb - cc + d;
+}
 
 __global__ void quat_dwt_kernel(const float* __restrict__ rgb, int64_t x_bs, float* __restrict__ out, int H, int W,
                                 int64_t total) {
@@ -21,22 +37,16 @@
 #pragma unroll
     for (int s = 0; s < 4; ++s) {
         const int yy = 2 * y + (s & 1), xx = 2 * x + (s >> 1);
-        const float r = p[(int64_t)yy * W + xx], g = p[HW + (int64_t)yy * W + xx], bl = p[2 * HW + (int64_t)yy * W + xx];
-        const float den = fmaxf(fmaxf(r, g), bl) + 1e-7f;
-        q[0][s] = 0.f; q[1][s] = 0.f;
-        q[2][s] = r / den; q[3][s] = r;
-        q[4][s] = g / den; q[5][s] = g;
-        q[6][s] = bl / den; q[7][s] = bl;
+        quat_stack(p[(int64_t)yy * W + xx], p[HW + (int64_t)yy * W + xx], p[2 * HW + (int64_t)yy * W + xx], q, s);
     }
     const int64_t hw2 = (int64_t)h2 * w2;
     float* o = out + (int64_t)b * 32 * hw2 + (int64_t)y * w2 + x;
 #pragma unroll
     for (int c = 0; c < 8; ++c) {
-        const float a = q[c][0] / 2, bb = q[c][1] / 2, cc = q[c][2] / 2, d = q[c][3] / 2;
-        o[(int64_t)(c) * hw2] = a + bb + cc + d;
-        o[(int64_t)(8 + c) * hw2] = -a - bb + cc + d;
-        o[(int64_t)(16 + c) * hw2] = -a + bb - cc + d;
-        o[(int64_t)(24 + c) * hw2] = a - bb - cc + d;
+        float v[4];
+        haar_bands(q[c], v);
+#pragma unroll
+        for (int band = 0; band < 4; ++band) o[(int64_t)(8 * band + c) * hw2] = v[band];
     }
 }
 
@@ -336,6 +346,19 @@
     dst[b * dst_bs + r] += src[b * src_bs + r];
 }
 
+__device__ __forceinline__ float bilinear_at(const float* __restrict__ p, int H, int W, float rs, int yo, int xo) {
+#pragma clang fp contract(off)
+    float sy = __builtin_fmaf((float)yo + 0.5f, rs, -0.5f); sy = sy < 0.f ? 0.f : sy;
+    float sx = __builtin_fmaf((float)xo + 0.5f, rs, -0.5f); sx = sx < 0.f ? 0.f : sx;
+    const int y0 = (int)sy, x0 = (int)sx;
+    const int y1 = y0 + (y0 < H - 1 ? 1 : 0), x1 = x0 + (x0 < W - 1 ? 1 : 0);
+    const float ly = sy - (float)y0, lx = sx - (float)x0;
+    const float hy = 1.f - ly, hx = 1.f - lx;
+    const float t0 = __builtin_fmaf(lx, p[(int64_t)y0 * W + x1], hx * p[(int64_t)y0 * W + x0]);
+    const float t1 = __builtin_fmaf(hx, p[(int64_t)y1 * W + x0], lx * p[(int64_t)y1 * W + x1]);
+    return hy * t0 + ly * t1;
+}
+
 __global__ void bilinear_up_kernel(const float* __restrict__ src, int64_t src_bs, float* __restrict__ dst,
                                    int64_t dst_bs, int C, int H, int W, int s, int64_t total) {
     const int64_t i = (int64_t)blockIdx.x * blockDim.x + threadIdx.x;
@@ -344,16 +367,43 @@
     const int xo = (int)(i % Wo), yo = (int)((i / Wo) % Ho);
     const int c = (int)((i / ((int64_t)Wo * Ho)) % C), b = (int)(i / ((int64_t)Wo * Ho * C));
     const float rs = 1.f / (float)s;
-    float sy = ((float)yo + 0.5f) * rs - 0.5f; sy = sy < 0.f ? 0.f : sy;
-    float sx = ((float)xo + 0.5f) * rs - 0.5f; sx = sx < 0.f ? 0.f : sx;
-    const int y0 = (int)sy, x0 = (int)sx;
-    const int y1 = y0 + (y0 < H - 1 ? 1 : 0), x1 = x0 + (x0 < W - 1 ? 1 : 0);
-    const float ly = sy - (float)y0, lx = sx - (float)x0;
-    const float hy = 1.f - ly, hx = 1.f - lx;
     const float* p = src + (int64_t)b * src_bs + (int64_t)c * H * W;
-    const float v = hy * (hx * p[(int64_t)y0 * W + x0] + lx * p[(int64_t)y0 * W + x1]) +
-                    ly * (hx * p[(int64_t)y1 * W + x0] + lx * p[(int64_t)y1 * W + x1]);
-    dst[(int64_t)b * dst_bs + ((int64_t)c * Ho + yo) * Wo + xo] = v;
+    dst[(int64_t)b * dst_bs + ((int64_t)c * Ho + yo) * Wo + xo] = bilinear_at(p, H, W, rs, yo, xo);
+}
+
+template <int NPX>
+__global__ __launch_bounds__(256) void cond_dwt_kernel(const float* __restrict__ cond, float* __restrict__ out, int H, int W, int s, int64_t total) {
+    const int64_t i = (int64_t)blockIdx.x * blockDim.x + threadIdx.x;
+    if (i >= total) return;
+    const int h2 = (H * s) >> 1, w2 = (W * s) >> 1, wq = w2 / NPX;
+    const int x = (int)(i % wq) * NPX, y = (int)((i / wq) % h2), b = (int)(i / ((int64_t)wq * h2));
+    const float rs = 1.f / (float)s;
+    const float* p = cond + (int64_t)b * 3 * H * W;
+    const int HW = H * W;
+    float q[NPX][8][4];
+#pragma unroll
+    for (int j = 0; j < NPX; ++j)
+#pragma unroll
+        for (int t = 0; t < 4; ++t) {
+            const int yy = 2 * y + (t & 1), xx = 2 * (x + j) + (t >> 1);
+            quat_stack(bilinear_at(p, H, W, rs, yy, xx), bilinear_at(p + HW, H, W, rs, yy, xx), bilinear_at(p + 2 * HW, H, W, rs, yy, xx), q[j], t);
+        }
+    typedef float fpx __attribute__((ext_vector_type(NPX)));
+    const int64_t hw2 = (int64_t)h2 * w2;
+    float* o = out + (int64_t)b * 32 * hw2 + (int64_t)y * w2 + x;
+#pragma unroll
+    for (int c = 0; c < 8; ++c) {
+        float v[NPX][4];
+#pragma unroll
+        for (int j = 0; j < NPX; ++j) haar_bands(q[j][c], v[j]);
+#pragma unroll
+        for (int band = 0; band < 4; ++band) {
+            fpx w;
+#pragma unroll
+            for (int j = 0; j < NPX; ++j) w[j] = v[j][band];
+            *reinterpret_cast<fpx*>(o + (int64_t)(8 * band + c) * hw2) = w;
+        }
+    }
 }
 
 __global__ void space_to_depth_kernel(const float* __restrict__ x, float* __restrict__ out, int C, int H, int W,
@@ -694,6 +744,22 @@
     return bem_check_launch("quat_dwt");
 }
 
+extern "C" int bem_cond_dwt_f32(const float* cond, float* out, int R, int H, int W, int s, void* stream) {
+    BEM_REQUIRE(cond && out, "cond_dwt: null tensor");
+    BEM_REQUIRE(R >= 0 && H > 0 && W > 0 && s >= 1 && (int64_t)H * s < (1 << 24) && (int64_t)W * s < (1 << 24) && (H * s) % 2 == 0 && (W * s) % 2 == 0,
+                "cond_dwt: the enlarged image (%d x %d times %d) must have even sides", H, W, s);
+    if (R == 0) return BEM_OK;
+    const int h2 = H * s / 2, w2 = W * s / 2;
+    if (w2 % 4 == 0 && ((uintptr_t)out & 15) == 0) {
+        const int64_t total = (int64_t)R * h2 * (w2 / 4);
+        cond_dwt_kernel<4><<<GRID1D(total), 256, 0, (hipStream_t)stream>>>(cond, out, H, W, s, total);
+    } else {
+        const int64_t total = (int64_t)R * h2 * w2;
+        cond_dwt_kernel<1><<<GRID1D(total), 256, 0, (hipStream_t)stream>>>(cond, out, H, W, s, total);
+    }
+    return bem_check_launch("cond_dwt");
+}
+
 extern "C" int bem_dwt_f32(const float* x, float* out, int B, int C, int H, int W, void* stream) {
     BEM_REQUIRE(x && out, "dwt: null tensor");
     BEM_REQUIRE(B >= 0 && C > 0 && H > 0 && W > 0 && H % 2 == 0 && W % 2 == 0, "dwt: H, W must be even");
diff --git a/bayesian-enhancement-model_amd/csrc/pw_gemm_x6.hip b/bayesian-enhancement-model_amd/csrc/pw_gemm_x6.hip
--- a/bayesian-enhancement-model_amd/csrc/pw_gemm_x6.hip
+++ b/bayesian-enhancement-model_amd/csrc/pw_gemm_x6.hip
@@ -799,7 +799,7 @@
 struct CvX {
     const float* x; int64_t x_bs;
     const u32x4* Wp; const float* bias; const float* res1; const float* res2; float* out;
-    int Cin, H, W, Ho, Wo, Cout, KB, MT, relu, pad, dil;
+    int Cin, H, W, Ho, Wo, Cout, KB, MT, relu, pad, dil, res1_rep;
 };
 
 template <int MTW, int KH, int KW, int S>
@@ -896,7 +896,7 @@
     const float lo = k.relu ? 0.f : -3.402823466e38f;
     const uint32_t loff = (uint32_t)(4 * kh) * (uint32_t)Lo + (uint32_t)pc;
     float* outb = k.out + (int64_t)b * k.Cout * Lo;
-    const float* r1b = k.res1 ? k.res1 + (int64_t)b * k.Cout * Lo : nullptr;
+    const float* r1b = k.res1 ? k.res1 + (int64_t)(b / k.res1_rep) * k.Cout * Lo : nullptr;
     const float* r2b = k.res2 ? k.res2 + (int64_t)b * k.Cout * Lo : nullptr;
 #pragma unroll
     for (int m = 0; m < MTW; ++m) {
@@ -929,8 +929,9 @@
 }
 
 static int conv_taps_launch(const float* x, int64_t x_bstride, const float* Wp, const float* bias, const float* res1, const float* res2,
-                            float* out, int B, int Cin, int H, int W, int Cout, int KH, int stride, int dil, int relu, void* stream, const char* what) {
-    BEM_REQUIRE(x && Wp && out, "%s: null tensor", what);
+                            float* out, int B, int Cin, int H, int W, int Cout, int KH, int stride, int dil, int relu, int res1_rep, void* stream,
+                            const char* what) {
+    BEM_REQUIRE(x && Wp && out && res1_rep >= 1, "%s: null tensor or res1_rep < 1", what);
     BEM_REQUIRE(B >= 0 && B <= 65535 && Cin > 0 && Cout > 0 && H > 0 && W > 0, "%s: bad shape", what);
     BEM_REQUIRE((KH == 3 && stride == 1 && (dil == 1 || dil == 2)) || (KH == 3 && stride == 2 && dil == 1),
                 "%s: supported forms are 3x3 s1 (dilation 1 / 2, padding = dilation) and 3x3 s2 p1", what);
@@ -943,7 +944,7 @@
     if (B == 0) return BEM_OK;
     CvX k;
     k.x = x; k.x_bs = x_bstride; k.Wp = reinterpret_cast<const u32x4*>(Wp); k.bias = bias; k.res1 = res1; k.res2 = res2; k.out = out;
-    k.Cin = Cin; k.H = H; k.W = W; k.Ho = Ho; k.Wo = Wo; k.Cout = Cout; k.KB = cdiv(Cin, 16); k.MT = cdiv(Cout, 32); k.relu = relu; k.pad = pad; k.dil = dil;
+    k.Cin = Cin; k.H = H; k.W = W; k.Ho = Ho; k.Wo = Wo; k.Cout = Cout; k.KB = cdiv(Cin, 16); k.MT = cdiv(Cout, 32); k.relu = relu; k.pad = pad; k.dil = dil; k.res1_rep = res1_rep;
     const int mtw = k.MT == 1 ? 1 : 2;
     dim3 grid(cdiv(Ho * Wo, 256), cdiv(k.MT, mtw), B);
     hipStream_t s = (hipStream_t)stream;
@@ -960,17 +961,17 @@
 extern "C" int bem_conv4x4s2_fast_supported(int Cin, int H, int W);
 extern "C" int bem_conv3x3_rows_supported(int Cin, int H, int W);
 int conv_rows_launch(int KS, const float* x, int64_t x_bstride, const float* Wp, const float* bias, const float* res1, const float* res2, float* out,
-                     int B, int Cin, int H, int W, int Cout, int relu, void* stream);
+                     int B, int Cin, int H, int W, int Cout, int relu, int res1_rep, void* stream);
 static bool rows_aligned(const float* x, int64_t x_bstride, const float* out, const float* res1, const float* res2) {
     return x && out && (((uintptr_t)x | (uintptr_t)out | (uintptr_t)(res1 ? res1 : out) | (uintptr_t)(res2 ? res2 : out)) & 15) == 0 && x_bstride % 4 == 0;
 }
 
 extern "C" int bem_conv3x3_x6_f32(const float* x, int64_t x_bstride, const float* Wp, const float* bias, const float* res1,
-                                  const float* res2, float* out, int B, int Cin, int H, int W, int Cout, int relu, void* stream) {
+                                  const float* res2, float* out, int B, int Cin, int H, int W, int Cout, int relu, int res1_rep, void* stream) {
     static const bool rows = !(getenv("BEM_CONV3_ROWS") && atoi(getenv("BEM_CONV3_ROWS")) == 0);
     if (rows && Cin > 0 && bem_conv3x3_rows_supported(Cin, H, W) && rows_aligned(x, x_bstride, out, res1, res2))
-        return conv_rows_launch(3, x, x_bstride, Wp, bias, res1, res2, out, B, Cin, H, W, Cout, relu, stream);
-    return conv_taps_launch(x, x_bstride, Wp, bias, res1, res2, out, B, Cin, H, W, Cout, 3, 1, 1, relu, stream, "conv3x3_x6");
+        return conv_rows_launch(3, x, x_bstride, Wp, bias, res1, res2, out, B, Cin, H, W, Cout, relu, res1_rep, stream);
+    return conv_taps_launch(x, x_bstride, Wp, bias, res1, res2, out, B, Cin, H, W, Cout, 3, 1, 1, relu, res1_rep, stream, "conv3x3_x6");
 }
 
 
@@ -978,10 +979,11 @@
                                     const float* res2, float* out, int B, int Cin, int H, int W, int Cout, int relu, void* stream) {
     BEM_REQUIRE(Cin > 0 && bem_conv4x4s2_fast_supported(Cin, H, W) && rows_aligned(x, x_bstride, out, res1, res2),
                 "conv4x4s2_x6: needs W = 2 Wo with Wo a power of two <= 64, even H, Cin %% 8 == 0 and 16-byte aligned tensors");
-    return conv_rows_launch(4, x, x_bstride, Wp, bias, res1, res2, out, B, Cin, H, W, Cout, relu, stream);
+    return conv_rows_launch(4, x, x_bstride, Wp, bias, res1, res2, out, B, Cin, H, W, Cout, relu, 1, stream);
 }
 
 extern "C" int bem_conv_taps_x6_f32(const float* x, int64_t x_bstride, const float* Wp, const float* bias, const float* res1, const float* res2,
-                                    float* out, int B, int Cin, int H, int W, int Cout, int K, int stride, int dilation, int relu, void* stream) {
-    return conv_taps_launch(x, x_bstride, Wp, bias, res1, res2, out, B, Cin, H, W, Cout, K, stride, dilation, relu, stream, "conv_taps_x6");
-}
+                                    float* out, int B, int Cin, int H, int W, int Cout, int K, int stride, int dilation, int relu, int res1_rep,
+                                    void* stream) {
+    return conv_taps_launch(x, x_bstride, Wp, bias, res1, res2, out, B, Cin, H, W, Cout, K, stride, dilation, relu, res1_rep, stream, "conv_taps_x6");
+}
diff --git a/include/bem_hip.h b/include/bem_hip.h
--- a/include/bem_hip.h
+++ b/include/bem_hip.h
@@ -79,23 +79,25 @@
 
 int bem_conv2d_f32(const float* x, int64_t x_bstride, const float* w, const float* bias, const float* res1,
                    const float* res2, float* out, int B, int Cin, int H, int W, int Cout, int KH, int KW,
-                   int stride, int pad, int relu, void* stream);
+                   int stride, int pad, int relu, int res1_rep, void* stream);
 
 int bem_conv2d_mfma_f32(const float* x, int64_t x_bstride, const float* Wp, const float* bias, const float* res1,
                         const float* res2, float* out, int B, int Cin, int H, int W, int Cout, int KH, int KW,
-                        int stride, int pad, int relu, void* stream);
+                        int stride, int pad, int relu, int res1_rep, void* stream);
 
 int bem_conv3x3_x6_f32(const float* x, int64_t x_bstride, const float* Wp, const float* bias, const float* res1,
-                       const float* res2, float* out, int B, int Cin, int H, int W, int Cout, int relu, void* stream);
+                       const float* res2, float* out, int B, int Cin, int H, int W, int Cout, int relu, int res1_rep, void* stream);
 int bem_conv4x4s2_fast_supported(int Cin, int H, int W);
 int bem_conv3x3_rows_supported(int Cin, int H, int W);
 int bem_conv4x4s2_x6_f32(const float* x, int64_t x_bstride, const float* Wp, const float* bias, const float* res1,
                          const float* res2, float* out, int B, int Cin, int H, int W, int Cout, int relu, void* stream);
 
 int bem_conv_taps_x6_f32(const float* x, int64_t x_bstride, const float* Wp, const float* bias, const float* res1, const float* res2,
-                         float* out, int B, int Cin, int H, int W, int Cout, int K, int stride, int dilation, int relu, void* stream);
+                         float* out, int B, int Cin, int H, int W, int Cout, int K, int stride, int dilation, int relu, int res1_rep,
+                         void* stream);
 
 int bem_quat_dwt_f32(const float* rgb, int64_t x_bstride, float* out, int B, int H, int W, void* stream);
+int bem_cond_dwt_f32(const float* cond, float* out, int R, int H, int W, int s, void* stream);
 int bem_dwt_f32(const float* x, float* out, int B, int C, int H, int W, void* stream);
 int bem_iwt_f32(const float* x, float* out, int B, int C4, int H, int W, void* stream);
 int bem_iwt_hamilton_f32(const float* q1w, const float* q2w, float* out, int B, int h, int w, void* stream);
```
